# rubenwiersma/gravo_mg

Hardware: AMD Instinct MI355X
Metric: V-cycle wall time (ms per V-cycle incl. residual check) + solve-to-1e-4 iterations, 3M-vertex Poisson (lower is better)
Workload: dtype f64

## Files before the change

### gravo_mg_amd/cabi.py

```python
from __future__ import annotations

import ctypes as C
import os
from typing import List, Optional, Sequence, Tuple

import numpy as np
import scipy.sparse as sp

_HERE = os.path.dirname(os.path.abspath(__file__))
LIB_PATH = os.environ.get("GMG_LIB_PATH") or os.path.join(_HERE, "lib", "libgravomg_hip.so")

GMG_OK, GMG_ERR_INVALID, GMG_ERR_NO_DEVICE, GMG_ERR_HIP, GMG_ERR_STATE, GMG_ERR_NUMERIC, GMG_ERR_UNSUPPORTED = 0, -1, -2, -3, -4, -5, -6
DIVERGED = 1
SMOOTHER_MULTICOLOR_GS, SMOOTHER_JACOBI, SMOOTHER_CHEBYSHEV = 0, 1, 2
COARSE_HOST_LDLT, COARSE_DEVICE_INVERSE, COARSE_AUTO, COARSE_DEVICE_TRIANGLE = 0, 1, 2, 3

_STATUS_NAMES = {
    -1: "GMG_ERR_INVALID", -2: "GMG_ERR_NO_DEVICE", -3: "GMG_ERR_HIP", -4: "GMG_ERR_STATE",
    -5: "GMG_ERR_NUMERIC", -6: "GMG_ERR_UNSUPPORTED",
}


class GmgError(RuntimeError):
    def __init__(self, code: int, msg: str):
        super().__init__(f"{_STATUS_NAMES.get(code, code)}: {msg}")
        self.code = code


class GmgConfig(C.Structure):
    _fields_ = [
        ("device", C.c_int), ("smoother", C.c_int), ("jacobi_omega", C.c_double), ("pre_iters", C.c_int),
        ("post_iters", C.c_int), ("coarse_mode", C.c_int), ("use_graph", C.c_int), ("sigma", C.c_int),
        ("row_align", C.c_int), ("block_rows", C.c_int), ("block_lanes", C.c_int), ("block_from_level", C.c_int),
        ("device_setup", C.c_int), ("device_rap", C.c_int), ("reorder_fine", C.c_int), ("inner_precision", C.c_int), ("block_csr", C.c_int), ("host_threads", C.c_int),
        ("verbose", C.c_int), ("gs_omega", C.c_double), ("restrict_sigma", C.c_int), ("block_ep", C.c_int), ("dist_shard_levels", C.c_int), ("block_fine", C.c_int), ("fine_col16", C.c_int), ("stream_gate", C.c_int), ("dist_exchange", C.c_int), ("prepare_structure", C.c_int), ("fuse_restrict_sweep", C.c_int), ("speculate_head", C.c_int), ("uniform_slices", C.c_int), ("color_ahead", C.c_int),
        ("accelerate", C.c_int),
    ]


class GmgHierarchyOptions(C.Structure):
    _fields_ = [
        ("ratio", C.c_double), ("lower_bound", C.c_int), ("check_voronoi", C.c_int), ("nested", C.c_int),
        ("sampling", C.c_int), ("weighting", C.c_int), ("debug", C.c_int), ("full_clustering", C.c_int), ("use_device", C.c_int),
    ]


class GmgDeviceVectors(C.Structure):
    _fields_ = [
        ("rhs", C.c_void_p), ("rhs_row_stride", C.c_int64), ("rhs_col_stride", C.c_int64),
        ("x0", C.c_void_p), ("x0_row_stride", C.c_int64), ("x0_col_stride", C.c_int64),
        ("x", C.c_void_p), ("x_row_stride", C.c_int64), ("x_col_stride", C.c_int64),
    ]


_ip = C.POINTER(C.c_int)
_dp = C.POINTER(C.c_double)
_vp = C.c_void_p

SIGNATURES = {
    "gmg_config_default": (C.c_int, [C.POINTER(GmgConfig)]),
    "gmg_config_size": (C.c_int, []),
    "gmg_create": (C.c_int, [C.POINTER(GmgConfig), C.POINTER(_vp)]),
    "gmg_destroy": (None, [_vp]),
    "gmg_last_error": (C.c_char_p, [_vp]),
    "gmg_device_count": (C.c_int, []),
    "gmg_set_num_levels": (C.c_int, [_vp, C.c_int]),
    "gmg_set_prolongation": (C.c_int, [_vp, C.c_int, C.c_int, C.c_int, _ip, _ip, _dp]),
    "gmg_set_mass": (C.c_int, [_vp, C.c_int, _dp]),
    "gmg_set_system": (C.c_int, [_vp, C.c_int, _ip, _ip, _dp]),
    "gmg_num_levels": (C.c_int, [_vp]),
    "gmg_level_info": (C.c_int, [_vp, C.c_int, _ip, C.POINTER(C.c_int64), _ip, _ip]),
    "gmg_get_level_operator": (C.c_int, [_vp, C.c_int, _ip, _ip, _dp]),
    "gmg_get_level_ordering": (C.c_int, [_vp, C.c_int, _ip, _ip]),
    "gmg_get_level_blocks": (C.c_int, [_vp, C.c_int, _ip, _ip, C.POINTER(C.c_ubyte)]),
    "gmg_get_timing": (C.c_int, [_vp, C.c_char_p, _dp]),
    "gmg_smooth": (C.c_int, [_vp, C.c_int, _dp, _dp, C.c_int, C.c_int]),
    "gmg_residual": (C.c_int, [_vp, C.c_int, _dp, _dp, C.c_int, _dp]),
    "gmg_spmv": (C.c_int, [_vp, C.c_int, _dp, C.c_int, _dp]),
    "gmg_restrict": (C.c_int, [_vp, C.c_int, _dp, C.c_int, _dp]),
    "gmg_prolong_add": (C.c_int, [_vp, C.c_int, _dp, C.c_int, _dp]),
    "gmg_coarse_solve": (C.c_int, [_vp, _dp, C.c_int, _dp]),
    "gmg_residual_norm": (C.c_int, [_vp, _dp, _dp, C.c_int, C.c_int, _dp]),
    "gmg_vcycle": (C.c_int, [_vp, _dp, _dp, C.c_int]),
    "gmg_smooth_residual": (C.c_int, [_vp, C.c_int, _dp, _dp, C.c_int, C.c_int, C.c_int, _dp]),
    "gmg_solve": (C.c_int, [_vp, _dp, _dp, C.c_int, C.c_double, C.c_int, C.c_int, _ip, _dp, _dp]),
    "gmg_solve_x0_rhs": (C.c_int, [_vp, _dp, _dp, C.c_int, C.c_double, C.c_int, C.c_int, _ip, _dp, _dp]),
    "gmg_solve_device": (C.c_int, [_vp, C.POINTER(GmgDeviceVectors), C.c_int, C.c_double, C.c_int, C.c_int, _ip, _dp, _dp]),
    "gmg_set_system_values_device": (C.c_int, [_vp, C.c_void_p, C.c_int64]),
    "gmg_load_problem": (C.c_int, [_vp, _dp, _dp, C.c_int]),
    "gmg_run_cycles": (C.c_int, [_vp, C.c_int, C.c_int, _dp]),
    "gmg_fetch_solution": (C.c_int, [_vp, _dp]),
    "gmg_set_stream": (C.c_int, [_vp, _vp]),
    "gmg_dist_setup": (C.c_int, [_vp, C.c_int, C.c_int]),
    "gmg_dist_partition": (C.c_int, [_vp, C.c_int, C.c_int]),
    "gmg_dist_bind": (C.c_int, [_vp, _vp, _vp, _vp, C.c_int]),
    "gmg_dist_smooth_color": (C.c_int, [_vp, C.c_int]),
    "gmg_dist_residual_own": (C.c_int, [_vp]),
    "gmg_dist_coarse_cycle": (C.c_int, [_vp]),
    "gmg_dist_prolong_own": (C.c_int, [_vp]),
    "gmg_dist_norm_partial": (C.c_int, [_vp, C.c_int, _dp]),
    "gmg_dist_all_rows": (C.c_int, [_vp, C.c_int]),
    "gmg_dist_gather": (C.c_int, [_vp, C.c_void_p, C.c_void_p, C.c_int64, C.c_void_p]),
    "gmg_dist_scatter": (C.c_int, [_vp, C.c_void_p, C.c_void_p, C.c_void_p, C.c_int64, C.c_void_p]),
    "gmg_p2p_blob_bytes": (C.c_int, []),
    "gmg_p2p_prepare": (C.c_int, [_vp, C.c_int, C.c_int, C.c_int]),
    "gmg_p2p_export": (C.c_int, [_vp, C.c_void_p]),
    "gmg_p2p_connect": (C.c_int, [_vp, C.c_void_p]),
    "gmg_p2p_rccl_unique_id": (C.c_int, [C.c_void_p]),
    "gmg_p2p_connect_rccl": (C.c_int, [_vp, C.c_void_p]),
    "gmg_p2p_load": (C.c_int, [_vp, _dp, _dp]),
    "gmg_p2p_cycles": (C.c_int, [_vp, C.c_int, C.c_int, _dp]),
    "gmg_p2p_fetch": (C.c_int, [_vp, _dp]),
    "gmg_p2p_solve": (C.c_int, [_vp, _dp, _dp, C.c_double, C.c_int, C.c_int, C.POINTER(C.c_int), C.POINTER(C.c_double)]),
    "gmg_p2p_stat": (C.c_int, [_vp, C.c_char_p, _dp]),
    "gmg_p2p_set_smoother": (C.c_int, [_vp, C.c_int]),
    "gmg_p2p_set_fences": (C.c_int, [_vp, C.c_int]),
    "gmg_hierarchy_options_default": (C.c_int, [C.POINTER(GmgHierarchyOptions)]),
    "gmg_hierarchy_build": (C.c_int, [_dp, C.c_int, _ip, C.c_int, C.POINTER(GmgHierarchyOptions), C.POINTER(_vp)]),
    "gmg_hierarchy_destroy": (None, [_vp]),
    "gmg_hierarchy_num_levels": (C.c_int, [_vp]),
    "gmg_hierarchy_level_shape": (C.c_int, [_vp, C.c_int, _ip, _ip, _ip]),
    "gmg_hierarchy_get_prolongation": (C.c_int, [_vp, C.c_int, _ip, _ip, _dp]),
    "gmg_hierarchy_get_timing": (C.c_int, [_vp, C.c_char_p, _dp]),
    "gmg_hierarchy_get_samples": (C.c_int, [_vp, C.c_int, _ip]),
    "gmg_hierarchy_get_nearest": (C.c_int, [_vp, C.c_int, _ip]),
    "gmg_hierarchy_get_points": (C.c_int, [_vp, C.c_int, _dp]),
    "gmg_host_threads": (C.c_int, []),
    "gmg_hierarchy_get_triangles": (C.c_int, [_vp, C.c_int, _ip, _ip]),
    "gmg_hierarchy_get_fine_order": (C.c_int, [_vp, _ip, _ip]),
    "gmg_set_fine_order": (C.c_int, [_vp, C.c_int, _ip]),
    "gmg_set_fine_graph": (C.c_int, [_vp, C.c_int, C.c_int, _ip]),
    "gmg_use_hierarchy": (C.c_int, [_vp, _vp]),
    "gmg_finalize_hierarchy": (C.c_int, [_vp]),
    "gmg_host_ldlt_solve": (C.c_int, [C.c_int, _ip, _ip, _dp, _dp, C.c_int, _dp, C.POINTER(C.c_int64)]),
}

INTERNAL_SIGNATURES = {
    "gmg_debug_sell_info": (C.c_int, [_vp, C.c_int, C.c_int, C.POINTER(C.c_int64)]),
    "gmg_debug_sell_copy": (C.c_int, [_vp, C.c_int, C.c_int, C.POINTER(C.c_int64), _ip, _dp, _ip, _dp]),
    "gmg_debug_col16_copy": (C.c_int, [_vp, C.c_int, C.POINTER(C.c_int64), C.POINTER(C.c_uint), _ip]),
    "gmg_debug_select_parents": (C.c_int, [C.c_int, C.c_int, C.c_int, C.c_int, C.c_int, C.c_int, _dp, _dp, _ip, _ip, _ip, _ip, _ip, _ip, _ip, _ip, C.c_int,
                                           C.POINTER(C.c_ubyte), C.POINTER(C.c_ubyte), _ip, _dp]),
    "gmg_hierarchy_debug_row_kinds": (C.c_int, [_vp, C.c_int, _ip]),
    "gmg_host_galerkin": (C.c_int, [C.c_int, _ip, _ip, _dp, C.c_int, _ip, _ip, _dp, _ip, _ip, _dp]),
    "gmg_debug_device_galerkin": (C.c_int, [_vp, C.c_int, _ip, _ip, _dp, _dp, C.c_int, _ip, _ip, _dp, C.c_int64, _ip, _ip, _dp, _dp, _ip]),
    "gmg_host_plan_level": (C.c_int, [C.c_int, _ip, _ip, _dp, C.c_int, C.c_int, C.c_int, C.POINTER(C.c_int64), _ip, _ip, _ip,
                                      C.POINTER(C.c_ubyte)]),
    "gmg_host_fine_block_rule": (C.c_int, [C.c_int, _ip, _ip, _dp, _ip, _ip]),
    "gmg_debug_set": (C.c_int, [_vp, C.c_char_p, C.c_double]),
    "gmg_bench_kernel": (C.c_int, [_vp, C.c_int, C.c_int, C.c_int, C.c_int, _dp, _ip]),
    "gmg_profile_cycle": (C.c_int, [_vp, C.c_int, C.c_int, _dp, C.c_int]),
    "gmg_algorithmic_bytes": (C.c_int, [_vp, C.c_int, C.c_int, C.c_int, _dp]),
    "gmg_p2p_bench_kind": (C.c_int, [_vp, C.c_char_p, C.c_int, _dp]),
    "gmg_p2p_debug_collective_roundtrip": (C.c_int, [_vp, _dp, C.POINTER(C.c_longlong)]),
    "gmg_host_ldlt_probe": (C.c_int, [C.c_int, _ip, _ip, _dp, _dp, C.c_int, C.c_char_p, C.c_int]),
}

_lib = None


def _preload_torch_hip_runtime():
    import importlib.util
    try:
        spec = importlib.util.find_spec("torch")
    except (ImportError, ValueError):
        spec = None
    if spec is None or not spec.submodule_search_locations:
        return
    libdir = os.path.join(list(spec.submodule_search_locations)[0], "lib")
    for name in ("libhsa-runtime64.so", "libamdhip64.so"):
        path = os.path.join(libdir, name)
        if os.path.exists(path):
            try:
                C.CDLL(path, mode=C.RTLD_GLOBAL)
            except OSError:
                pass


def lib() -> C.CDLL:
    global _lib
    if _lib is None:
        if not os.path.exists(LIB_PATH):
            raise ImportError(
                f"{LIB_PATH} is missing: build it with gravo_mg_amd/csrc/build.sh (or __graft_entry__.build()). "
                "gravo_mg_amd has no CPU fallback for the device path.")
        _preload_torch_hip_runtime()
        l = C.CDLL(LIB_PATH)
        for name, (res, args) in list(SIGNATURES.items()) + list(INTERNAL_SIGNATURES.items()):
            fn = getattr(l, name)
            fn.restype = res
            fn.argtypes = args
        if l.gmg_config_size() != C.sizeof(GmgConfig):
            raise ImportError(f"{LIB_PATH} was built with a gmg_config of {l.gmg_config_size()} bytes, gravo_mg_amd/cabi.py mirrors one of {C.sizeof(GmgConfig)}: "
                              "rebuild the library (gravo_mg_amd/csrc/build.sh) or update the mirror")
        _lib = l
    return _lib


def device_count() -> int:
    return int(lib().gmg_device_count())


def _f64(a, shape2d: bool = True) -> np.ndarray:
    a = np.asarray(a, dtype=np.float64)
    if a.ndim == 1:
        a = a[:, None]
    return np.asfortranarray(a)


def _csc_layout(m) -> sp.csc_matrix:
    m = m if sp.isspmatrix_csc(m) else sp.csc_matrix(m)
    if m.indptr.dtype != np.int32 or m.indices.dtype != np.int32:
        if m.nnz >= 2**31:
            raise ValueError("matrix too large for int32 indices")
        m = sp.csc_matrix((m.data, m.indices.astype(np.int32), m.indptr.astype(np.int32)), shape=m.shape)
    if m.data.dtype != np.float64:
        m = m.astype(np.float64)
    return m


def _csc(m) -> sp.csc_matrix:
    m = sp.csc_matrix(m)
    if not m.has_sorted_indices:
        m = m.copy()
        m.sort_indices()
    m.sum_duplicates()
    if m.indptr.dtype != np.int32 or m.indices.dtype != np.int32:
        if m.nnz >= 2**31:
            raise ValueError("matrix too large for int32 indices")
        m = sp.csc_matrix((m.data, m.indices.astype(np.int32), m.indptr.astype(np.int32)), shape=m.shape)
# ... 7 lines not shown


def _pd(a: np.ndarray):
    return a.ctypes.data_as(_dp)


class Hierarchy:

    def __init__(self, pos, neigh, ratio=8.0, lower_bound=1000, check_voronoi=True, nested=False, sampling=0, weighting=0, debug=False, full_clustering=False, use_device=True):
        l = lib()
        pos = np.ascontiguousarray(pos, dtype=np.float64)
        neigh = np.ascontiguousarray(neigh, dtype=np.int32)
        if pos.ndim != 2 or pos.shape[1] != 3 or neigh.ndim != 2 or neigh.shape[0] != pos.shape[0]:
            raise ValueError("pos must be n x 3 and neigh n x K")
        opt = GmgHierarchyOptions()
        l.gmg_hierarchy_options_default(C.byref(opt))
        opt.ratio, opt.lower_bound, opt.check_voronoi, opt.nested = float(ratio), int(lower_bound), int(bool(check_voronoi)), int(bool(nested))
        opt.sampling, opt.weighting, opt.debug, opt.full_clustering = int(sampling), int(weighting), int(bool(debug)), int(bool(full_clustering))
        opt.use_device = int(use_device)
        self._h = _vp()
        rc = l.gmg_hierarchy_build(_pd(pos), pos.shape[0], _pi(neigh), neigh.shape[1], C.byref(opt), C.byref(self._h))
        if rc:
            raise GmgError(rc, "gmg_hierarchy_build failed (only Sampling.FASTDISK is supported)" if rc == GMG_ERR_UNSUPPORTED else "gmg_hierarchy_build failed")
        self.U: List[sp.csc_matrix] = []
        for k in range(l.gmg_hierarchy_num_levels(self._h)):
            nf, nc, nnz = C.c_int(), C.c_int(), C.c_int()
            l.gmg_hierarchy_level_shape(self._h, k, C.byref(nf), C.byref(nc), C.byref(nnz))
            colptr = np.empty(nc.value + 1, np.int32); rowidx = np.empty(nnz.value, np.int32); val = np.empty(nnz.value, np.float64)
            l.gmg_hierarchy_get_prolongation(self._h, k, _pi(colptr), _pi(rowidx), _pd(val))
            self.U.append(sp.csc_matrix((val, rowidx, colptr), shape=(nf.value, nc.value)))
        self.samples, self.nearest, self.points = [], [], []
        for k, u in enumerate(self.U):
            s_ = np.empty(u.shape[1], np.int32); n_ = np.empty(u.shape[0], np.int32); p_ = np.empty((u.shape[1], 3), np.float64)
            if l.gmg_hierarchy_get_samples(self._h, k, _pi(s_)) or l.gmg_hierarchy_get_nearest(self._h, k, _pi(n_)) or l.gmg_hierarchy_get_points(self._h, k, _pd(p_)):
                raise GmgError(GMG_ERR_INVALID, "hierarchy getters failed")
            self.samples.append(s_); self.nearest.append(n_); self.points.append(p_)
        self.triangles = []
        for k in range(len(self.U)):
            cnt = C.c_int()
            l.gmg_hierarchy_get_triangles(self._h, k, None, C.byref(cnt))
            t = np.empty((cnt.value, 3), np.int32)
            if cnt.value:
                l.gmg_hierarchy_get_triangles(self._h, k, _pi(t), C.byref(cnt))
            self.triangles.append(t)
        cnt = C.c_int()
        l.gmg_hierarchy_get_fine_order(self._h, None, C.byref(cnt))
        self.fine_order = None
        if cnt.value:
            self.fine_order = np.empty(cnt.value, np.int32)
            l.gmg_hierarchy_get_fine_order(self._h, _pi(self.fine_order), C.byref(cnt))

    def row_kinds(self, k: int) -> np.ndarray:
        out = np.zeros(4, np.int32)
        if lib().gmg_hierarchy_debug_row_kinds(self._h, int(k), _pi(out)):
            raise GmgError(GMG_ERR_INVALID, "gmg_hierarchy_debug_row_kinds failed")
        return out

    def timing(self, key: str) -> float:
        out = C.c_double()
        rc = lib().gmg_hierarchy_get_timing(self._h, key.encode(), C.byref(out))
        if rc:
            raise KeyError(key)
        return out.value

    TIMING_KEYS = ("n_vertices", "hierarchy", "sampling", "cluster", "next_neighborhood", "next_positions",
                   "triangle_finding", "triangle_selection", "PDS", "levels")

    def timings(self) -> dict:
        return {k: self.timing(k) for k in self.TIMING_KEYS}

    def __del__(self):
        try:
            if getattr(self, "_h", None):
                lib().gmg_hierarchy_destroy(self._h)
                self._h = None
        except Exception:
            pass


class Engine:

    def __init__(self, smoother=SMOOTHER_MULTICOLOR_GS, pre_iters=2, post_iters=2, jacobi_omega=0.67,
                 coarse_mode=COARSE_AUTO, use_graph=False, sigma=0, row_align=64, block_rows=64, block_from_level=1, block_lanes=0,
                 device_setup=True, device_rap=True, reorder_fine=2, inner_precision=0, block_csr=True, device=0, verbose=False, gs_omega=None, block_ep=None, restrict_sigma=None, dist_shard_levels=None, block_fine=None, fine_col16=None, stream_gate=None, prepare_structure=None, dist_exchange=None, fuse_restrict_sweep=None, speculate_head=None, uniform_slices=None, color_ahead=None, accelerate=0):
        l = lib()
        cfg = GmgConfig()
        l.gmg_config_default(C.byref(cfg))
        cfg.device, cfg.smoother, cfg.jacobi_omega = int(device), int(smoother), float(jacobi_omega)
        cfg.pre_iters, cfg.post_iters, cfg.coarse_mode = int(pre_iters), int(post_iters), int(coarse_mode)
        cfg.use_graph, cfg.sigma, cfg.row_align, cfg.verbose = int(bool(use_graph)), int(sigma), int(row_align), int(bool(verbose))
        cfg.block_rows, cfg.block_from_level, cfg.block_lanes = int(block_rows), int(block_from_level), int(block_lanes)
        cfg.device_setup, cfg.device_rap, cfg.reorder_fine = int(bool(device_setup)), int(bool(device_rap)), int(reorder_fine)
        cfg.inner_precision, cfg.block_csr = int(inner_precision), int(bool(block_csr))
        if gs_omega is not None:
            cfg.gs_omega = float(gs_omega)
        if block_ep is not None:
            cfg.block_ep = int(bool(block_ep))
        if restrict_sigma is not None:
            cfg.restrict_sigma = int(restrict_sigma)
        if dist_shard_levels is not None:
            cfg.dist_shard_levels = int(dist_shard_levels)
        if block_fine is not None:
            cfg.block_fine = int(bool(block_fine))
        if fine_col16 is not None:
            cfg.fine_col16 = int(bool(fine_col16))
        if stream_gate is not None:
            cfg.stream_gate = int(bool(stream_gate))
        if prepare_structure is not None:
            cfg.prepare_structure = int(bool(prepare_structure))
        if fuse_restrict_sweep is not None:
            cfg.fuse_restrict_sweep = int(bool(fuse_restrict_sweep))
        if speculate_head is not None:
            cfg.speculate_head = int(bool(speculate_head))
        if uniform_slices is not None:
            cfg.uniform_slices = int(bool(uniform_slices))
        if color_ahead is not None:
            cfg.color_ahead = int(bool(color_ahead))
        if dist_exchange is not None:
            cfg.dist_exchange = int(dist_exchange)
        cfg.accelerate = int(accelerate)
        self._h = _vp()
        rc = l.gmg_create(C.byref(cfg), C.byref(self._h))
        if rc:
            raise GmgError(rc, "gmg_create failed (invalid configuration)")
        self._n0 = None
        self._sizes: List[int] = []
        self.pre_iters, self.post_iters = int(pre_iters), int(post_iters)
        self.gs_omega = float(cfg.gs_omega)

    @classmethod
    def borrow(cls, handle: int) -> "Engine":
        self = cls.__new__(cls)
        self._h = _vp(int(handle))
        self._borrowed = True
        self._n0 = None
        self._sizes = []
        self.pre_iters = self.post_iters = None
        self.gs_omega = None
        return self

    def _chk(self, rc: int):
        if rc:
            raise GmgError(rc, lib().gmg_last_error(self._h).decode())

    def close(self):
        if getattr(self, "_h", None):
            if not getattr(self, "_borrowed", False):
                lib().gmg_destroy(self._h)
            self._h = None

    def __del__(self):
        try:
            self.close()
        except Exception:
            pass

    def set_prolongations(self, U: Sequence, finalize: bool = True, fine_order=None, fine_graph=None):
        l = lib()
        self._chk(l.gmg_set_num_levels(self._h, len(U)))
        self._sizes = []
        for k, u in enumerate(U):
            u = _csc(u)
            self._chk(l.gmg_set_prolongation(self._h, k, u.shape[0], u.shape[1], _pi(u.indptr), _pi(u.indices), _pd(u.data)))
            if k == 0:
                self._sizes.append(u.shape[0])
            self._sizes.append(u.shape[1])
        if fine_order is not None and len(U):
            fo = np.ascontiguousarray(fine_order, dtype=np.int32)
            self._chk(l.gmg_set_fine_order(self._h, fo.shape[0], _pi(fo)))
        if fine_graph is not None and len(U):
            fg = np.ascontiguousarray(fine_graph, dtype=np.int32)
            self._chk(l.gmg_set_fine_graph(self._h, fg.shape[0], fg.shape[1], _pi(fg)))
        if finalize and len(U):
            self._chk(l.gmg_finalize_hierarchy(self._h))

    def use_hierarchy(self, hier: Hierarchy):
        self._chk(lib().gmg_use_hierarchy(self._h, hier._h))
        self._sizes = [hier.U[0].shape[0]] + [u.shape[1] for u in hier.U] if hier.U else []

    def set_mass(self, mass_diag):
        m = np.ascontiguousarray(mass_diag, dtype=np.float64).ravel()
        self._chk(lib().gmg_set_mass(self._h, m.shape[0], _pd(m)))

    def set_system(self, lhs):
        a = _csc_layout(lhs)
        if a.shape[0] != a.shape[1]:
            raise ValueError("lhs must be square")
        self._chk(lib().gmg_set_system(self._h, a.shape[0], _pi(a.indptr), _pi(a.indices), _pd(a.data)))
        self._n0 = a.shape[0]

    @property
    def num_levels(self) -> int:
        return int(lib().gmg_num_levels(self._h))

    def level_info(self, k: int) -> dict:
        n, nnz, nc, npad = C.c_int(), C.c_int64(), C.c_int(), C.c_int()
        self._chk(lib().gmg_level_info(self._h, k, C.byref(n), C.byref(nnz), C.byref(nc), C.byref(npad)))
        return {"n": n.value, "nnz": nnz.value, "n_colors": nc.value, "n_pad": npad.value}

    def level_operator(self, k: int) -> sp.csc_matrix:
        info = self.level_info(k)
        colptr = np.empty(info["n"] + 1, np.int32); rowidx = np.empty(info["nnz"], np.int32); val = np.empty(info["nnz"], np.float64)
        self._chk(lib().gmg_get_level_operator(self._h, k, _pi(colptr), _pi(rowidx), _pd(val)))
# ... 317 lines not shown
    a, u = _csc_layout(A), _csc_layout(U)
    nc = u.shape[1]
    v2 = None if val2 is None else np.ascontiguousarray(val2, dtype=np.float64)
    if v2 is not None and v2.shape != a.data.shape:
        raise ValueError("val2 must have one value per stored entry of A")
    colptr, status = np.zeros(nc + 1, np.int32), C.c_int(-1)
    cap = a.nnz + nc
    for attempt in range(2):
        rowidx, val = np.empty(max(cap, 1), np.int32), np.empty(max(cap, 1), np.float64)
        out2 = np.empty(max(cap, 1), np.float64) if v2 is not None else None
        rc = lib().gmg_debug_device_galerkin(eng._h, a.shape[0], _pi(a.indptr), _pi(a.indices), _pd(a.data), _pd(v2) if v2 is not None else None, nc,
                                             _pi(u.indptr), _pi(u.indices), _pd(u.data), cap, _pi(colptr), _pi(rowidx), _pd(val),
                                             _pd(out2) if out2 is not None else None, C.byref(status))
        if rc == GMG_ERR_INVALID and attempt == 0 and int(colptr[nc]) > cap:
            cap = int(colptr[nc])
            continue
        eng._chk(rc)
        break
    if status.value != 0:
        return status.value, None, None
    nnz = int(colptr[nc])
    return 0, sp.csc_matrix((val[:nnz].copy(), rowidx[:nnz].copy(), colptr), shape=(nc, nc)), (out2[:nnz].copy() if out2 is not None else None)


def host_galerkin(A, U, as_stored: bool = False) -> sp.csc_matrix:
    a, u = (_csc_layout(A), _csc_layout(U)) if as_stored else (_csc(A), _csc(U))
    nc = u.shape[1]
    colptr = np.zeros(nc + 1, np.int32)
    rc = lib().gmg_host_galerkin(a.shape[0], _pi(a.indptr), _pi(a.indices), _pd(a.data), nc, _pi(u.indptr), _pi(u.indices), _pd(u.data),
                                 _pi(colptr), None, None)
    if rc:
        raise GmgError(rc, "gmg_host_galerkin")
    nnz = int(colptr[nc])
    rowidx = np.empty(nnz, np.int32); val = np.empty(nnz, np.float64)
    lib().gmg_host_galerkin(a.shape[0], _pi(a.indptr), _pi(a.indices), _pd(a.data), nc, _pi(u.indptr), _pi(u.indices), _pd(u.data),
                            _pi(colptr), _pi(rowidx), _pd(val))
    return sp.csc_matrix((val, rowidx, colptr), shape=(nc, nc))


def default_host_threads() -> int:
    return int(lib().gmg_host_threads())


def host_plan_level(A, mode: int = 0, block_rows: int = 256, sigma: int = 1024, row_align: int = 64) -> dict:
    a = _csc(A)
    n = a.shape[0]
    if mode != 1:
        block_rows = row_align
    info = (C.c_int64 * 6)()
    rc = lib().gmg_host_plan_level(n, _pi(a.indptr), _pi(a.indices), _pd(a.data), int(mode), int(block_rows), int(sigma), info, None, None, None, None)
    if rc:
        raise GmgError(rc, "gmg_host_plan_level")
    new2old = np.empty(int(info[0]), np.int32); color_begin = np.zeros(int(info[1]) + 1, np.int32)
    blk_begin = np.zeros(int(info[2]) + 1, np.int32); row_color = np.zeros(int(info[0]), np.uint8)
    rc = lib().gmg_host_plan_level(n, _pi(a.indptr), _pi(a.indices), _pd(a.data), int(mode), int(block_rows), int(sigma), info,
                                   _pi(new2old), _pi(color_begin), _pi(blk_begin), row_color.ctypes.data_as(C.POINTER(C.c_ubyte)))
    if rc:
        raise GmgError(rc, "gmg_host_plan_level")
    n_pad, n_colors, n_blocks = int(info[0]), int(info[1]), int(info[2])
    out = {"n_pad": n_pad, "n_colors": n_colors, "n_blocks": n_blocks, "sell_stored": int(info[3]), "offdiag_nnz": int(info[4]),
           "new2old": new2old[:n_pad].copy()}
    if mode == 1:
        out["blk_begin"] = blk_begin[: n_blocks + 1].copy()
        out["row_color"] = row_color[:n_pad].copy()
    else:
        out["color_begin"] = color_begin[: n_colors + 1].copy()
    return out


def host_plan_ahead(n, indptr, indices, row_align: int = 64, sigma: int = 1024) -> dict:
    indptr = np.ascontiguousarray(indptr, np.int32); indices = np.ascontiguousarray(indices, np.int32)
    vals = np.ones(max(len(indices), 1))
    info = (C.c_int64 * 6)()
    rc = lib().gmg_host_plan_level(int(n), _pi(indptr), _pi(indices), _pd(vals), 4, int(row_align), int(sigma), info, None, None, None, None)
    if rc:
        raise GmgError(rc, "gmg_host_plan_level")
    new2old = np.empty(int(info[0]), np.int32); color_begin = np.zeros(int(info[1]) + 1, np.int32)
    rc = lib().gmg_host_plan_level(int(n), _pi(indptr), _pi(indices), _pd(vals), 4, int(row_align), int(sigma), info, _pi(new2old), _pi(color_begin), None, None)
    if rc:
        raise GmgError(rc, "gmg_host_plan_level")
    return {"n_pad": int(info[0]), "n_colors": int(info[1]), "colored_ahead": bool(info[5]), "new2old": new2old, "color_begin": color_begin}


def host_fine_block_rule(A):
    a = _csc(A)
    blocked, reason = C.c_int(0), C.c_int(0)
    rc = lib().gmg_host_fine_block_rule(a.shape[0], _pi(a.indptr), _pi(a.indices), _pd(a.data), C.byref(blocked), C.byref(reason))
    if rc:
        raise GmgError(rc, "gmg_host_fine_block_rule")
    return bool(blocked.value), int(reason.value)


def host_ldlt_solve(A, b):
    a = _csc(A)
    B = _f64(b)
    X = np.empty_like(B, order="F")
    nnz = C.c_int64()
    rc = lib().gmg_host_ldlt_solve(a.shape[0], _pi(a.indptr), _pi(a.indices), _pd(a.data), _pd(B), B.shape[1], _pd(X), C.byref(nnz))
    if rc:
        raise GmgError(rc, "gmg_host_ldlt_solve (zero pivot?)")
    return (X[:, 0].copy() if np.asarray(b).ndim == 1 else X), nnz.value


def host_ldlt_probe(A, b, reps: int = 3) -> str:
    a = _csc(A)
    B = _f64(b)
    buf = C.create_string_buffer(1 << 16)
    rc = lib().gmg_host_ldlt_probe(a.shape[0], _pi(a.indptr), _pi(a.indices), _pd(a.data), _pd(B), int(reps), buf, len(buf))
    if rc:
        raise GmgError(rc, "gmg_host_ldlt_probe")
    return buf.value.decode()
```

### gravo_mg_amd/csrc/bindings.cpp

```cpp
#include <chrono>
#include <cstdio>
#include <cstdlib>
#include <pybind11/numpy.h>
#include <pybind11/pybind11.h>
#include <pybind11/stl.h>

#include <algorithm>
#include <atomic>
#include <cmath>
#include <cstdint>
#include <memory>
#include <stdexcept>
#include <string>
#include <thread>
#include <vector>

#include "multigrid_solver.h"

namespace py = pybind11;
using DenseIn = py::array_t<double, py::array::f_style | py::array::forcecast>;
using IntIn = py::array_t<int, py::array::c_style | py::array::forcecast>;

namespace {

// ... 202 lines not shown
        MGBS::MatrixXd x = b;
        solver->clearError();
        if (pardiso) throw std::runtime_error("direct_solve(pardiso=True): Pardiso (MKL) is not part of this build; use pardiso=False (sparse LDL^T)");
        solver->solve(A, b, x, 0);
        check();
        return from_dense(x);
    }

    py::list prolongation_matrices() {
        py::list out;
        for (const auto& u : solver->U) out.append(from_sparse(u));
        return out;
    }

    void set_prolongation_matrices(py::list U) {
        std::vector<MGBS::SparseMatrix> v;
        for (auto item : U) v.push_back(to_sparse(py::reinterpret_borrow<py::object>(item)));
        solver->U = v;
    }

    std::vector<std::vector<int>> sampling_indices() { return solver->samples; }
    std::vector<std::vector<size_t>> nearest_source() { return solver->nearestSource; }
    py::list level_points() {
        py::list out;
        for (const auto& P : solver->levelV) out.append(from_dense(P));
        return out;
    }
    py::list level_edges() { return py::list(); }
    std::vector<std::vector<int>> notrimap() { return solver->noTriFoundMap; }
    std::vector<std::vector<std::vector<int>>> all_triangles() { return solver->allTriangles; }
    py::list coarse_normals() { return py::list(); }

    void write_hierarchy_timing(std::string experiment, std::string file, bool write_headers) { MGBS::writeTiming(solver->hierarchyTiming, experiment, file, write_headers); }
    void write_solver_timing(std::string experiment, std::string file, bool write_headers) { MGBS::writeTiming(solver->solverTiming, experiment, file, write_headers); }
    void write_convergence(std::string file) { MGBS::writeConvergence(solver->convergence, file); }

    double residual(py::object lhs, DenseIn rhs, DenseIn solution, int type = 2) {
        MappedSparse mapped = map_system_matrix(lhs, symCache);
        MGBS::SparseMatrix& A = mapped.m;
        solver->clearError();
        double r = solver->residualCheck(A, to_dense(rhs), to_dense(solution), type);
        check();
        return r;
    }

    std::map<std::string, double> solver_timing() { return solver->solverTiming; }
    std::map<std::string, double> hierarchy_timing() { return solver->hierarchyTiming; }
    std::vector<std::tuple<double, double>> convergence() { return solver->convergence; }
    std::tuple<uintptr_t, long> prepare_system(py::object lhs) {
        MappedSparse mapped = map_system_matrix(lhs, symCache);
        gmg_handle h = nullptr;
        long gen = 0;
        solver->clearError();
        if (solver->prepareSystem(mapped.m, &h, &gen) != GMG_OK) { check(); throw std::runtime_error("prepare_system failed"); }
        return std::make_tuple((uintptr_t)h, gen);
    }
    uintptr_t engine_handle() { return (uintptr_t)solver->engineHandle(); }
    void invalidate_system() { solver->systemChangedExternally(); }
    void set_engine_option(const std::string& key, double value) {
        gmg_config& c = solver->engineConfig;
        if (key == "smoother") c.smoother = (int)value;
        else if (key == "jacobi_omega") c.jacobi_omega = value;
        else if (key == "gs_omega") c.gs_omega = value;
        else if (key == "coarse_mode") c.coarse_mode = (int)value;
        else if (key == "use_graph") c.use_graph = (int)value;
        else if (key == "block_rows") c.block_rows = (int)value;
        else if (key == "block_from_level") c.block_from_level = (int)value;
        else if (key == "device") c.device = (int)value;
        else if (key == "row_align") c.row_align = (int)value;
        else if (key == "block_lanes") c.block_lanes = (int)value;
        else if (key == "dist_shard_levels") c.dist_shard_levels = (int)value;
        else if (key == "block_fine") c.block_fine = (int)value;
        else if (key == "dist_rank") solver->distRank = (int)value;
        else if (key == "dist_world") solver->distWorld = (int)value;
        else if (key == "fine_col16") c.fine_col16 = (int)value;
        else if (key == "stream_gate") c.stream_gate = (int)value;
        else if (key == "fuse_restrict_sweep") c.fuse_restrict_sweep = (int)value;
        else if (key == "speculate_head") c.speculate_head = (int)value;
        else if (key == "uniform_slices") c.uniform_slices = (int)value;
        else if (key == "color_ahead") c.color_ahead = (int)value;
        else if (key == "dist_exchange") c.dist_exchange = (int)value;
        else if (key == "inner_precision") c.inner_precision = (int)value;
        else if (key == "accelerate") c.accelerate = (int)value;
        else throw std::invalid_argument("unknown engine option: " + key);
    }

#ifdef GMG_TESTING
    void test_report_diverged(int n) { solver->testReportDiverged = n; }
#endif

private:
    void check() {
        std::string now = solver->lastError();
        if (!now.empty()) throw std::runtime_error(now);
    }
    std::unique_ptr<MGBS::MultigridSolver> solver;
    SymmetryCache symCache;
};

PYBIND11_MODULE(gravomg_bindings, m) {
    m.doc() = "Multigrid solver bindings (MI355X-native V-cycle hot path)";

    py::enum_<Hierarchy>(m, "Hierarchy").value("OURS", OURS).value("SIG21", SIG21);
    py::enum_<Sampling>(m, "Sampling").value("FASTDISK", FASTDISK).value("POISSONDISK", POISSONDISK).value("FPS", FPS).value("RANDOM", RANDOM).value("MIS", MIS);
    py::enum_<Weighting>(m, "Weighting").value("BARYCENTRIC", BARYCENTRIC).value("UNIFORM", UNIFORM).value("INVDIST", INVDIST);

    py::class_<MultigridSolver>(m, "MultigridSolver")
        .def(py::init<DenseIn, IntIn, py::object, double, int, int, double, int, int, int, int, bool, bool, Sampling, Weighting, bool, DenseIn, bool, bool, bool, int, bool>())
        .def("construct_sig21_hierarchy", &MultigridSolver::construct_sig21_hierarchy, py::arg("F"))
        .def("toggle_hierarchy", &MultigridSolver::toggle_hierarchy, py::arg("hierarchy"))
        .def("solve", &MultigridSolver::solve, py::arg("lhs"), py::arg("rhs"))
        .def("direct_solve", &MultigridSolver::direct_solve, py::arg("lhs"), py::arg("rhs"), py::arg("pardiso"))
        .def("prolongation_matrices", &MultigridSolver::prolongation_matrices)
        .def("set_prolongation_matrices", &MultigridSolver::set_prolongation_matrices, py::arg("U"))
        .def("sampling_indices", &MultigridSolver::sampling_indices)
        .def("level_points", &MultigridSolver::level_points)
        .def("level_edges", &MultigridSolver::level_edges)
        .def("notrimap", &MultigridSolver::notrimap)
        .def("all_triangles", &MultigridSolver::all_triangles)
        .def("coarse_normals", &MultigridSolver::coarse_normals)
        .def("nearest_source", &MultigridSolver::nearest_source)
        .def("write_hierarchy_timing", &MultigridSolver::write_hierarchy_timing, py::arg("experiment"), py::arg("file"), py::arg("write_headers"))
        .def("write_solver_timing", &MultigridSolver::write_solver_timing, py::arg("experiment"), py::arg("file"), py::arg("write_headers"))
        .def("write_convergence", &MultigridSolver::write_convergence, py::arg("file"))
        .def("residual", &MultigridSolver::residual, py::arg("lhs"), py::arg("rhs"), py::arg("solution"), py::arg("type") = 2)
        .def("solver_timing", &MultigridSolver::solver_timing)
        .def("hierarchy_timing", &MultigridSolver::hierarchy_timing)
        .def("convergence", &MultigridSolver::convergence)
        .def("prepare_system", &MultigridSolver::prepare_system, py::arg("lhs"))
        .def("engine_handle", &MultigridSolver::engine_handle)
        .def("invalidate_system", &MultigridSolver::invalidate_system)
        .def("set_engine_option", &MultigridSolver::set_engine_option, py::arg("key"), py::arg("value"))
#ifdef GMG_TESTING
        .def("_test_report_diverged", &MultigridSolver::test_report_diverged, py::arg("n"))
#endif
        ;
}
```

### gravo_mg_amd/csrc/engine.hip

```cpp
#include <hip/hip_runtime.h>
#include <dlfcn.h>

#include <array>
#include <atomic>
#include <chrono>
#include <cmath>
#include <functional>
#include <future>
#include <cstdio>
#include <cstdlib>
#include <cstring>
#include <map>
#include <mutex>
#include <shared_mutex>
#include <string>
#include <vector>

#if !defined(__HIP_DEVICE_COMPILE__)
#include <execinfo.h>
#include <signal.h>
#include <unistd.h>
#endif

#include "../../include/gravomg_hip.h"
// ... 15 lines not shown

#if !defined(__HIP_DEVICE_COMPILE__)
namespace {
struct sigaction gmg_prev_action[32];
void gmg_fatal_signal(int sig) {
    void* frames[48];
    const int nf = backtrace(frames, 48);
    const char msg[] = "[gmg] fatal signal, native stack of the faulting thread:\n";
    (void)!write(2, msg, sizeof(msg) - 1);
    backtrace_symbols_fd(frames, nf, 2);
    if (sig > 0 && sig < 32) sigaction(sig, &gmg_prev_action[sig], nullptr); else signal(sig, SIG_DFL);
    raise(sig);
}
struct GmgSignalAid {
    GmgSignalAid() {
        if (!EnvSwitches::get().segv_backtrace) return;
        void* warm[4];
        (void)backtrace(warm, 4);
        struct sigaction sa;
        std::memset(&sa, 0, sizeof(sa));
        sa.sa_handler = gmg_fatal_signal;
        for (int sig : {SIGSEGV, SIGBUS, SIGABRT, SIGFPE}) sigaction(sig, &sa, &gmg_prev_action[sig]);
    }
} gmg_signal_aid;
}
#endif

#include "engine_state.hip.hpp"
#include "engine_setup.hip.hpp"
#include "engine_cycle.hip.hpp"
#include "engine_part.hip.hpp"
#include "engine_system.hip.hpp"

int gate_unwound(gmg_handle h);
#define GMG_CATCH_H                                                                                             \
    catch (const std::exception& e_) { if (h) (void)gate_unwound(h); return h ? fail(h, GMG_ERR_STATE, std::string("exception: ") + e_.what()) : GMG_ERR_STATE; } \
    catch (...) { if (h) (void)gate_unwound(h); return h ? fail(h, GMG_ERR_STATE, "unknown exception") : GMG_ERR_STATE; }
#define GMG_CATCH_0                                              \
    catch (...) { return GMG_ERR_STATE; }

void p2p_release_handle(gmg_handle h);


extern "C" {

int gmg_config_size(void) { return (int)sizeof(gmg_config); }

int gmg_config_default(gmg_config* cfg) try {
    if (!cfg) return GMG_ERR_INVALID;
    std::memset(cfg, 0, sizeof(*cfg));
    cfg->device = 0;
    cfg->smoother = GMG_SMOOTHER_MULTICOLOR_GS;
    cfg->jacobi_omega = 0.67;
    cfg->pre_iters = 2;
    cfg->post_iters = 2;
    cfg->coarse_mode = GMG_COARSE_AUTO;
    cfg->use_graph = 0;
    cfg->sigma = 0;
    cfg->row_align = 64;
    cfg->block_rows = 64;
    cfg->block_from_level = 1;
    cfg->block_lanes = 0;
    cfg->device_setup = 1;
    cfg->device_rap = 1;
    cfg->reorder_fine = 2;
    cfg->inner_precision = 0;
    cfg->block_csr = 1;
    cfg->host_threads = 0;
    cfg->verbose = 0;
    cfg->block_ep = 1;
    cfg->dist_shard_levels = 2;
    cfg->fine_col16 = 1;
    cfg->stream_gate = 1;
    cfg->prepare_structure = 1;
    cfg->fuse_restrict_sweep = 1;
    cfg->speculate_head = 1;
    cfg->uniform_slices = 1;
    cfg->color_ahead = 1;
    cfg->dist_exchange = 0;
    cfg->block_fine = 1;
    cfg->restrict_sigma = 64;
    cfg->gs_omega = 1.35;
    cfg->accelerate = 0;
    return GMG_OK;
} GMG_CATCH_0

int gmg_host_threads(void) try { return hw_threads(); } GMG_CATCH_0

int gmg_device_count(void) try {
    int n = 0;
    if (hipGetDeviceCount(&n) != hipSuccess) return 0;
    return n;
} GMG_CATCH_0

int gmg_create(const gmg_config* cfg, gmg_handle* out) try {
    if (!out) return GMG_ERR_INVALID;
    gmg_config c;
    if (cfg) c = *cfg; else gmg_config_default(&c);
    if (c.sigma < 0 || c.sigma % 64 || c.restrict_sigma < 0 || c.restrict_sigma % 64 || c.row_align <= 0 || c.row_align % 64 || c.pre_iters < 0 || c.post_iters < 0 ||
        c.reorder_fine < 0 || c.reorder_fine > 2 || c.inner_precision < 0 || c.inner_precision > 1 || c.block_rows < 0 || c.block_rows > gmgk::kBlockRows || c.block_rows % 64 || c.block_from_level < 0 || !(c.gs_omega > 0.0 && c.gs_omega < 2.0) || c.dist_shard_levels < 1 || c.dist_shard_levels > 2 || c.block_fine < 0 || c.block_fine > 1 || c.dist_exchange < 0 || c.dist_exchange > 2 ||
        (c.block_lanes != 0 && c.block_lanes != 1 && c.block_lanes != 4) || (c.block_lanes != 1 && c.block_rows > gmgk::kQuadBlockRows)) return GMG_ERR_INVALID;
    if (c.accelerate < 0 || c.accelerate > gmg::kAccelMaxDepth) return GMG_ERR_INVALID;
    if (c.smoother < GMG_SMOOTHER_MULTICOLOR_GS || c.smoother > GMG_SMOOTHER_CHEBYSHEV) return GMG_ERR_INVALID;
    if (c.accelerate > 0 && c.inner_precision) return GMG_ERR_UNSUPPORTED;
    gmg_handle h = new gmg_solver_s();
    h->cfg = c;
    if (h->cfg.host_threads <= 0) h->cfg.host_threads = hw_threads();
    int ndev = gmg_device_count();
    if (ndev > 0 && c.device >= 0 && c.device < ndev && hipSetDevice(c.device) == hipSuccess &&
        hipStreamCreateWithFlags(&h->stream, hipStreamNonBlocking) == hipSuccess) {
        h->has_device = true;
        h->own_stream = h->stream;
        { int cus = 0; if (hipDeviceGetAttribute(&cus, hipDeviceAttributeMultiprocessorCount, c.device) == hipSuccess && cus > 0) h->n_cus = cus; else (void)hipGetLastError(); }
        (void)hipEventCreate(&h->ev0);
        (void)hipEventCreate(&h->ev1);
        if (hipStreamCreateWithFlags(&h->aux_stream, hipStreamNonBlocking) != hipSuccess) { h->aux_stream = nullptr; (void)hipGetLastError(); }
        if (hipEventCreateWithFlags(&h->aux_ev, hipEventDisableTiming) != hipSuccess) { h->aux_ev = nullptr; (void)hipGetLastError(); }
        if (hipMalloc((void**)&h->d_aux_err, sizeof(int)) != hipSuccess) { h->d_aux_err = nullptr; (void)hipGetLastError(); }
        h->poll = EnvSwitches::get().poll;
        (void)ensure_bounce(h);
    }
    *out = h;
    return GMG_OK;
} GMG_CATCH_0

void gmg_destroy(gmg_handle h) {
    if (!h) return;
    PoolScope pool_scope_(&h->pool);
    if (h->has_device) {
        (void)hipSetDevice(h->cfg.device);
        (void)hipStreamSynchronize(h->stream);
        p2p_release_handle(h);
        drop_system(h);
        drop_device_transfers(h);
        h->d_stage = {}; h->d_partials = {}; h->d_norm = {}; h->d_watch = {};
        if (h->h_pinned) (void)sync_hipHostFree(h->h_pinned);
        for (int i = 0; i < 2; ++i) { if (h->h_stage[i]) (void)sync_hipHostFree(h->h_stage[i]); if (h->h_stage_ev[i]) (void)hipEventDestroy(h->h_stage_ev[i]); }
        for (hipEvent_t& e : h->h_chunk_ev) if (e) (void)hipEventDestroy(e);
        if (h->h_norm) (void)sync_hipHostFree(h->h_norm);
        if (h->h_flag) (void)sync_hipHostFree(h->h_flag);
        if (h->ev0) (void)hipEventDestroy(h->ev0);
        if (h->ev1) (void)hipEventDestroy(h->ev1);
        if (h->aux_ev) (void)hipEventDestroy(h->aux_ev);
        if (h->aux_stream) { (void)hipStreamSynchronize(h->aux_stream); (void)sync_hipStreamDestroy(h->aux_stream); }
        if (h->d_aux_err) (void)sync_hipFree(h->d_aux_err);
        drop_rap_order(h);
        for (int i = 0; i < 2; ++i) { if (h->bounce[i]) (void)sync_hipHostFree(h->bounce[i]); if (h->bounce_ev[i]) (void)hipEventDestroy(h->bounce_ev[i]); }
        for (hipEvent_t e : h->prof_ev) (void)hipEventDestroy(e);
        (void)sync_hipStreamDestroy(h->own_stream);
        h->pool.trim();
    }
    delete h;
}

const char* gmg_last_error(gmg_handle h) { return h ? h->err.c_str() : "null handle"; }

int gmg_set_num_levels(gmg_handle h, int L) try {
    if (!h || L < 0 || L > 64) return h ? fail(h, GMG_ERR_INVALID, "invalid level count") : GMG_ERR_INVALID;
    PoolScope pool_scope_(&h->pool);
    if (h->has_device) { drop_system(h); drop_device_transfers(h); }
    h->patches.clear(); h->patches_ready = false;
    h->bfs_order.clear();
    h->fine_graph.reset();
    drop_rap_order(h);
    h->L = L;
    h->ord_cache_valid = false;
// ... 1148 lines not shown
    std::memcpy(c_colptr, C.ptr.data(), sizeof(int) * (n_coarse + 1));
    if (c_rowidx) std::memcpy(c_rowidx, C.idx.data(), sizeof(int) * C.nnz());
    if (c_val) std::memcpy(c_val, C.val.data(), sizeof(double) * C.nnz());
    return GMG_OK;
} GMG_CATCH_0

int gmg_debug_device_galerkin(gmg_handle h, int n, const int* a_colptr, const int* a_rowidx, const double* a_val, const double* a_val2, int n_coarse,
                              const int* u_colptr, const int* u_rowidx, const double* u_val, int64_t cap, int* c_colptr, int* c_rowidx, double* c_val,
                              double* c_val2, int* status) try {
    NEED_DEVICE();
    if (n <= 0 || n_coarse <= 0 || cap < 0 || !a_colptr || !a_rowidx || !a_val || !u_colptr || !u_rowidx || !u_val || !c_colptr || !c_rowidx || !c_val || !status ||
        (a_val2 && !c_val2)) return fail(h, GMG_ERR_INVALID, "bad arguments");
    if (a_colptr[0] != 0 || u_colptr[0] != 0) return fail(h, GMG_ERR_INVALID, "column pointers must start at 0");
    for (int i = 0; i < n; ++i) if (a_colptr[i + 1] < a_colptr[i]) return fail(h, GMG_ERR_INVALID, "column pointers of A decrease");
    for (int c = 0; c < n_coarse; ++c) if (u_colptr[c + 1] < u_colptr[c]) return fail(h, GMG_ERR_INVALID, "column pointers of U decrease");
    for (int q = 0; q < a_colptr[n]; ++q) if (a_rowidx[q] < 0 || a_rowidx[q] >= n) return fail(h, GMG_ERR_INVALID, "row index of A out of range");
    for (int q = 0; q < u_colptr[n_coarse]; ++q) if (u_rowidx[q] < 0 || u_rowidx[q] >= n) return fail(h, GMG_ERR_INVALID, "row index of U out of range");
    if (hipSetDevice(h->cfg.device) != hipSuccess) return fail(h, GMG_ERR_HIP, "hipSetDevice failed");
    DevCsr dA, dU, dC;
    DevEll3 e3;
    DevBuf<int> d_err;
    Compressed C;
    int rc, herr = 0;
    if ((rc = dev_alloc(h, d_err, 1))) return rc;
    HIPCHK(hipMemsetAsync(d_err, 0, sizeof(int), h->stream));
    if ((rc = upload_csr_raw(h, dA, n, a_colptr, a_rowidx, a_val)) || (rc = upload_csr_raw(h, dU, n_coarse, u_colptr, u_rowidx, u_val)) ||
        (rc = build_ell3(h, e3, dU, n, d_err))) { (void)hipStreamSynchronize(h->stream); return rc; }
    HIPCHK(hipMemcpyAsync(&herr, d_err, sizeof(int), hipMemcpyDeviceToHost, h->stream));
    HIPCHK(hipStreamSynchronize(h->stream));
    *status = 0;
    if (herr) { *status = 1; return GMG_OK; }
    int64_t nnz = 0;
    rc = device_rap(h, dA, dU, e3, dC, C, true, true, &nnz, d_err);
    if (rc == 1) { *status = 1; return GMG_OK; }
    if (rc) return rc;
    std::memcpy(c_colptr, C.ptr.data(), sizeof(int) * ((size_t)n_coarse + 1));
    if (nnz > cap) return fail(h, GMG_ERR_INVALID, "the product has " + std::to_string(nnz) + " entries: more than the caller's capacity (c_colptr is filled)");
    if (nnz) { std::memcpy(c_rowidx, C.idx.data(), sizeof(int) * (size_t)nnz); std::memcpy(c_val, C.val.data(), sizeof(double) * (size_t)nnz); }
    if (a_val2) {
        Compressed C2;
        if ((rc = h2d(h, dA.val, a_val2, sizeof(double) * (size_t)a_colptr[n]))) { (void)hipStreamSynchronize(h->stream); return rc; }
        rc = device_rap(h, dA, dU, e3, dC, C2, false, true, &nnz, d_err, true);
        HIPCHK(hipStreamSynchronize(h->stream));
        if (rc) return rc < 0 ? rc : fail(h, GMG_ERR_STATE, "the numeric pass declined a pattern the product was made on");
        if ((int64_t)C2.val.size() != nnz) return fail(h, GMG_ERR_STATE, "the numeric pass returned another number of entries");
        if (nnz) std::memcpy(c_val2, C2.val.data(), sizeof(double) * (size_t)nnz);
    }
    return GMG_OK;
} GMG_CATCH_H

int gmg_host_plan_level(int n, const int* colptr, const int* rowidx, const double* val, int mode, int block_rows, int sigma, int64_t* info,
                        int* new2old, int* color_begin, int* blk_begin, unsigned char* row_color) try {
    if (n <= 0 || !colptr || !rowidx || !val || mode < 0 || mode > 4) return GMG_ERR_INVALID;
    if (mode == 1 && (block_rows <= 0 || block_rows > gmgk::kBlockRows || block_rows % 64)) return GMG_ERR_INVALID;
    if (sigma < 0 || sigma % 64) return GMG_ERR_INVALID;
    if (mode == 4) {
        PreColoring pre;
        std::atomic<int> stop{0};
        pre.n_colors = greedy_coloring_ahead(n, colptr, rowidx, (int64_t)colptr[n], pre.c8, stop);
        if (pre.n_colors == -2) return GMG_ERR_INVALID;
        if (info) info[5] = pre.n_colors >= 0 ? 1 : 0;
        LevelOrdering o = make_ordering(PatternView{n, colptr, rowidx}, true, (block_rows > 0 && block_rows % 64 == 0) ? block_rows : 64, sigma, 0, nullptr, true, &pre);
        if (o.n_colors > kMaxColors) return GMG_ERR_UNSUPPORTED;
        if (info) { info[0] = o.n_pad; info[1] = o.n_colors; info[2] = 0; info[3] = 0; info[4] = 0; }
        if (new2old) std::memcpy(new2old, o.new2old.data(), sizeof(int) * o.n_pad);
        if (color_begin) std::memcpy(color_begin, o.color_begin.data(), sizeof(int) * (o.n_colors + 1));
        return GMG_OK;
    }
    Compressed A;
    A.assign(n, n, colptr, rowidx, val);
    LevelOrdering o = mode == 1 ? make_block_ordering(A, block_rows)
                                : make_ordering(A, true, (block_rows > 0 && block_rows % 64 == 0) ? block_rows : 64, sigma, mode == 2 ? 1 : 0, nullptr, mode == 3);
    if (o.n_colors > kMaxColors) return GMG_ERR_UNSUPPORTED;
    SellHost sa; std::vector<double> dg; std::string e;
    if (!build_operator_sell(A, o, 0, sa, dg, e)) return GMG_ERR_NUMERIC;
    if (info) { info[0] = o.n_pad; info[1] = o.n_colors; info[2] = o.n_blocks(); info[3] = sa.stored(); info[4] = sa.nnz_real; info[5] = 0; }
    if (new2old) std::memcpy(new2old, o.new2old.data(), sizeof(int) * o.n_pad);
    if (color_begin && !o.blocked) std::memcpy(color_begin, o.color_begin.data(), sizeof(int) * (o.n_colors + 1));
    if (blk_begin && o.blocked) std::memcpy(blk_begin, o.blk_begin.data(), sizeof(int) * o.blk_begin.size());
    if (row_color && o.blocked) std::memcpy(row_color, o.row_color.data(), o.row_color.size());
    return GMG_OK;
} GMG_CATCH_0

int gmg_debug_set(gmg_handle h, const char* key, double value) try {
    if (!h || !key) return GMG_ERR_INVALID;
    if (std::string(key) == "col16_uncovered") { h->dbg_col16_uncovered = (int)value; return GMG_OK; }
    if (std::string(key) == "cheby_ratio") {
        if (value != 0.0 && !cheby_ratio_usable(value)) return fail(h, GMG_ERR_INVALID, "cheby_ratio must be > 1 (0: the process-wide ratio)");
        h->dbg_cheby_ratio = value;
        if (h->has_device) drop_graphs(h);
        if (h->timing.count("cheby_ratio")) h->timing["cheby_ratio"] = cheby_ratio(h);
        return GMG_OK;
    }
    return fail(h, GMG_ERR_INVALID, std::string("unknown debug key: ") + key);
} GMG_CATCH_H

int gmg_host_fine_block_rule(int n, const int* colptr, const int* rowidx, const double* val, int* blocked, int* reason) try {
    if (n <= 0 || !colptr || !rowidx || !val || !blocked) return GMG_ERR_INVALID;
    int why = 0;
    if ((double)colptr[n] < kFineBlockMinRow * (double)n) why = 1;
    else if (!stieltjes_signs(n, colptr, rowidx, val, hw_threads())) why = 2;
    *blocked = why == 0 ? 1 : 0;
    if (reason) *reason = why;
    return GMG_OK;
} GMG_CATCH_0

int gmg_host_ldlt_solve(int n, const int* colptr, const int* rowidx, const double* val, const double* b, int d, double* x, int64_t* factor_nnz) try {
    if (n <= 0 || !colptr || !rowidx || !val || !b || !x || d <= 0) return GMG_ERR_INVALID;
    Compressed A;
    A.assign(n, n, colptr, rowidx, val);
    SupernodalLDLT f;
    if (!f.factor(A)) return GMG_ERR_NUMERIC;
    std::vector<double> w((size_t)n * d);
    f.solve_multi(b, (size_t)n, x, (size_t)n, d, w.data());
    if (factor_nnz) *factor_nnz = f.factor_nnz();
    return GMG_OK;
} GMG_CATCH_0

int gmg_host_ldlt_probe(int n, const int* colptr, const int* rowidx, const double* val, const double* b, int reps, char* report, int cap) try {
    if (n <= 0 || !colptr || !rowidx || !val || !b || !report || cap <= 0) return GMG_ERR_INVALID;
    reps = std::max(1, reps);
    Compressed A;
    A.assign(n, n, colptr, rowidx, val);
    SupernodalLDLT f;
    if (!f.factor(A)) return GMG_ERR_NUMERIC;
    std::vector<double> w((size_t)n * 3), x((size_t)n);
    f.solve_multi(b, (size_t)n, x.data(), (size_t)n, 1, w.data());
    std::string text;
    auto say = [&](const char* fmt, auto... args) { char line[1024]; std::snprintf(line, sizeof(line), fmt, args...); text += line; };
    {
        std::vector<double> xb((size_t)n);
        double best = 1e30;
        for (int batch = 0; batch < 20; ++batch) {
            auto t0 = clk::now();
            for (int i = 0; i < reps; ++i) f.solve_multi(b, (size_t)n, xb.data(), (size_t)n, 1, w.data());
            best = std::min(best, 1e3 * ms_since(t0) / reps);
        }
        say("factorisation: ordering %.2f ms, symbolic %.2f ms, numeric %.2f ms\n", f.phase_ms[0], f.phase_ms[1], f.phase_ms[2]);
        {
            std::vector<double> ts;
            for (int i = 0; i < 15; ++i) { if (!f.factor(A, true)) return GMG_ERR_NUMERIC; ts.push_back(f.phase_ms[2]); }
            std::sort(ts.begin(), ts.end());
            say("numeric re-factorisation on %d thread(s): best %.2f ms, median %.2f ms\n", SupernodalLDLT::numeric_threads(), ts.front(), ts[ts.size() / 2]);
        }
        {
            SupernodalLDLT::DeviceFactor E;
            f.export_device_factor(E);
            std::vector<double> col((size_t)n), e((size_t)n, 0.0), ref((size_t)n), wk((size_t)n);
            double worst = 0.0, scale = 0.0;
            const int picks = std::min(n, 24);
            for (int t = 0; t < picks; ++t) {
                const int c = (int)((long)t * (n - 1) / std::max(picks - 1, 1));
                SupernodalLDLT::emulate_device_column(E, c, col.data());
                e[(size_t)f.perm[(size_t)c]] = 1.0;
                f.solve(e.data(), ref.data(), wk.data());
                e[(size_t)f.perm[(size_t)c]] = 0.0;
                for (int j = c; j < n; ++j) { worst = std::max(worst, std::fabs(col[(size_t)j] - ref[(size_t)f.perm[(size_t)j]])); scale = std::max(scale, std::fabs(ref[(size_t)f.perm[(size_t)j]])); }
            }
            say("device factor layout: %d chunks of <= %d columns in %d levels; %d columns of the inverse by the chunk algorithm vs back-substitution: max |difference| %.3e of max |entry| %.3e\n",
                E.nq, SupernodalLDLT::kChunk, E.nlev, picks, worst, scale);
        }
        long part[3];
        f.split_report(part);
        say("n=%d nnz(L)=%ld: %.2f us per single-column solve on one thread (best of 20 batches of %d); %d parts of the elimination "
                     "tree, panel entries in the lightest / heaviest part / above them: %ld / %ld / %ld\n", n, f.factor_nnz(), best, reps, f.parts(), part[0], part[1], part[2]);
        for (int threads = 2; threads <= std::min(8, f.parts()); threads += threads < 4 ? 1 : 2) {
            double best2 = 1e30, diff = 0.0;
            SpinTeam team(threads - 1);
            team.arm();
            std::vector<double> x2((size_t)n);
            for (int batch = 0; batch < 20; ++batch) {
                auto t0 = clk::now();
                for (int i = 0; i < reps; ++i) f.solve_multi(b, (size_t)n, x2.data(), (size_t)n, 1, w.data(), &team);
                best2 = std::min(best2, 1e3 * ms_since(t0) / reps);
// ... 52 lines not shown
```

### gravo_mg_amd/csrc/engine_cycle.hip.hpp

```cpp
#pragma once

namespace {


#define DISPATCH_D(dc, ...)              \
    switch (dc) {                        \
        case 1: { constexpr int D = 1; __VA_ARGS__; } break; \
        case 2: { constexpr int D = 2; __VA_ARGS__; } break; \
        case 3: { constexpr int D = 3; __VA_ARGS__; } break; \
        default: { constexpr int D = 4; __VA_ARGS__; } break; \
    }

#define DISPATCH_C16(mode, ...)          \
    switch (mode) {                      \
        case 1: { constexpr int C16 = 1; __VA_ARGS__; } break; \
        case 2: { constexpr int C16 = 2; __VA_ARGS__; } break; \
        case 3: { constexpr int C16 = 3; __VA_ARGS__; } break; \
        case 4: { constexpr int C16 = 4; __VA_ARGS__; } break; \
        default: { constexpr int C16 = 0; __VA_ARGS__; } break; \
    }

#define DISPATCH_FLAG(NAME, cond, ...)   \
    { if (cond) { constexpr bool NAME = true; __VA_ARGS__; } else { constexpr bool NAME = false; __VA_ARGS__; } }

#define DISPATCH_ONE_OF(NAME, v, A, B, C, ...)   \
    { if ((v) == (A)) { constexpr int NAME = A; __VA_ARGS__; } else if ((v) == (B)) { constexpr int NAME = B; __VA_ARGS__; } else { constexpr int NAME = C; __VA_ARGS__; } }

template <class F>
inline void for_col_chunks(int d, F&& f) {
    for (int c0 = 0; c0 < d; c0 += 4) f(c0, std::min(4, d - c0));
}

template <class T> struct Prec;
template <> struct Prec<double> {
    static const double* val(const DevSell& s) { return s.val; }
    static const double* diag(const Level& l) { return l.diag; }
    static const double* bcval(const Level& l) { return l.bc_val; }
    static const double* epval(const Level& l) { return l.ep_val; }
    static const double* eeval(const Level& l) { return l.ee_val; }
    static double* x(Level& l) { return l.x; }
    static double* b(Level& l) { return l.b; }
    static double* r(Level& l) { return l.r; }
    static double* tmp(Level& l) { return l.tmp; }
};
template <> struct Prec<float> {
    static const float* val(const DevSell& s) { return s.val32; }
    static const float* diag(const Level& l) { return l.diag32; }
    static const float* bcval(const Level& l) { return l.bc_val32; }
    static const float* epval(const Level& l) { return l.ep_val32; }
    static const float* eeval(const Level& l) { return l.ee_val32; }
    static float* x(Level& l) { return l.x32; }
    static float* b(Level& l) { return l.b32; }
    static float* r(Level& l) { return l.r32; }
    static float* tmp(Level& l) { return l.tmp32; }
};

template <class T>
struct SmoothAsk {
    bool from_zero = false;
    bool first_done = false;
    bool head_done = false;
    T* res_out = nullptr;
    bool res_il = false;
    int norm_type = -1;
    T* il_out = nullptr;
};
template <class T>
struct SmoothDone {
    int res_from = 0;
    int norm_blocks = 0;
    const T* prev = nullptr;
    bool prev_valid = false;
    bool il_written = false;
};

template <class T>
int fold_norm(gmg_handle, Level&, int, bool, int, int, int) { return 0; }
template <>
int fold_norm<double>(gmg_handle h, Level& l, int d, bool last_launch, int sb, int se, int type) {
    if (!last_launch || type < 0 || &l != &h->lv[0] || d > 4 || l.ord.n_colors < 2 || se != l.Aoff.n_slices) return 0;
    const double* w = type == 1 ? h->d_minv : (type == 2 ? h->d_mass : nullptr);
    const int nblk = grid_for(se - sb), first = norm_grid(sb);
    if ((size_t)(first + nblk) > (size_t)h->partial_blocks) return 0;
    DISPATCH_D(d, DISPATCH_C16(l.Aoff.c16_sel(), hipLaunchKernelGGL((gmgk::gs_color_norm<D, C16>), dim3(nblk), dim3(gmgk::kBlock), 0, h->stream, l.Aoff.slice_ptr,
                                     l.Aoff.col, l.Aoff.val, l.diag, l.b, l.x, l.n_pad, sb, se, h->cfg.gs_omega, w, h->d_partials + (size_t)first * 2 * d,
                                     l.Aoff.col16, l.Aoff.win_base, l.Aoff.c16_arg())));
    return nblk;
}

template <class T>
int fold_residual(gmg_handle, Level&, int, bool, int, int, T*, bool) { return 0; }
template <>
int fold_residual<double>(gmg_handle h, Level& l, int d, bool last_launch, int sb, int se, double* out, bool il) {
    if (!last_launch || !out || &l != &h->lv[0] || d > 4 || l.ord.n_colors < 2 || se != l.Aoff.n_slices || sb <= 0) return 0;
    DISPATCH_D(d, DISPATCH_C16(l.Aoff.c16_sel(), DISPATCH_FLAG(YI, il, hipLaunchKernelGGL((gmgk::gs_color_residual<D, C16, (YI && D > 1)>), dim3(grid_for(se - sb)),
                                     dim3(gmgk::kBlock), 0, h->stream, l.Aoff.slice_ptr, l.Aoff.col, l.Aoff.val, l.diag, l.b, l.x, out, l.n_pad, sb, se,
                                     h->cfg.gs_omega, l.Aoff.col16, l.Aoff.win_base, l.Aoff.c16_arg()))));
    return sb;
}

inline bool polled(gmg_handle h);

template <class T>
T level_omega(gmg_handle h, const Level& l) { return &l == &h->lv[0] ? (T)h->cfg.gs_omega : (T)1.0; }

template <class T>
void launch_gs_color(gmg_handle h, Level& l, int c0, int dc, int sb, int se, T omega, const unsigned long long* plain_rows = nullptr, const int* go = nullptr) {
    const int ld = l.n_pad;
    T* x = Prec<T>::x(l);
    const T* b = Prec<T>::b(l);
    if (&l == &h->lv[0]) {
        DISPATCH_D(dc, DISPATCH_C16(l.Aoff.c16_sel(), DISPATCH_FLAG(OM, plain_rows != nullptr, hipLaunchKernelGGL((gmgk::gs_color<T, D, C16 + 1, (OM && sizeof(T) == 8)>),
                                          dim3(grid_for(se - sb)), dim3(gmgk::kBlock), 0, h->stream, l.Aoff.slice_ptr, l.Aoff.col, Prec<T>::val(l.Aoff), Prec<T>::diag(l),
                                          b + (size_t)c0 * ld, x + (size_t)c0 * ld, ld, sb, se, 1, omega, l.Aoff.col16, l.Aoff.win_base, l.Aoff.c16_arg(), plain_rows, go))));
    } else {
        DISPATCH_D(dc, hipLaunchKernelGGL((gmgk::gs_color<T, D, 0>), dim3(grid_for(se - sb)), dim3(gmgk::kBlock), 0, h->stream,
                                          l.Aoff.slice_ptr, l.Aoff.col, Prec<T>::val(l.Aoff), Prec<T>::diag(l), b + (size_t)c0 * ld,
                                          x + (size_t)c0 * ld, ld, sb, se, 1, omega));
    }
}

inline int first_color(const Level& l) {
    for (int c = 0; c < l.ord.n_colors; ++c)
        if (l.ord.color_begin[c + 1] / 64 > l.ord.color_begin[c] / 64) return c;
    return -1;
}

inline bool head_eligible(gmg_handle h, int d) {
    return h->cfg.speculate_head && polled(h) && !h->cfg.inner_precision && h->cfg.smoother == GMG_SMOOTHER_MULTICOLOR_GS && h->cfg.pre_iters > 0 && h->L >= 1 &&
           !h->lv[0].ord.blocked && h->lv[0].ord.n_colors >= 2 && first_color(h->lv[0]) >= 0 && first_color(h->lv[0]) < h->lv[0].ord.n_colors - 1 && d >= 1 && d <= 4 &&
           !h->partitioned && h->part_world <= 1 && h->d_watch && !h->prof_on;
}
inline bool enqueue_head(gmg_handle h, int d) {
    Level& l = h->lv[0];
    const int c = first_color(l);
    launch_gs_color<double>(h, l, 0, d, l.ord.color_begin[c] / 64, l.ord.color_begin[c + 1] / 64, level_omega<double>(h, l), nullptr, reinterpret_cast<const int*>(h->d_watch + 1));
    h->timing["heads_enqueued"] += 1.0;
    return true;
}

template <class T>
SmoothDone<T> launch_gs_sweeps(gmg_handle h, Level& l, int d, int iters, const SmoothAsk<T>& ask) {
    SmoothDone<T> done;
    const int c_head = ask.head_done ? first_color(l) : -1;
    for (int it = 0; it < iters; ++it)
        for_col_chunks(d, [&](int c0, int dc) {
            for (int c = 0; c < l.ord.n_colors; ++c) {
                int sb = l.ord.color_begin[c] / 64, se = l.ord.color_begin[c + 1] / 64;
                if (se <= sb) continue;
                if (it == 0 && c0 == 0 && c == c_head) continue;
                const bool last_launch = it == iters - 1 && c == l.ord.n_colors - 1;
                if (const int nblk = fold_norm<T>(h, l, d, last_launch, sb, se, ask.norm_type)) { done.norm_blocks = nblk; continue; }
                if (const int from = fold_residual<T>(h, l, d, last_launch, sb, se, ask.res_out, ask.res_il)) { done.res_from = from; continue; }
                launch_gs_color<T>(h, l, c0, dc, sb, se, level_omega<T>(h, l));
            }
        });
    return done;
}

template <class T>
void launch_jacobi_sweeps(gmg_handle h, Level& l, int d, int iters) {
    const int ld = l.n_pad;
    T* in = Prec<T>::x(l); T* out = Prec<T>::tmp(l);
    const T* b = Prec<T>::b(l);
    for (int it = 0; it < iters; ++it) {
        for_col_chunks(d, [&](int c0, int dc) {
            DISPATCH_D(dc, hipLaunchKernelGGL((gmgk::jacobi_sweep<T, D>), dim3(grid_for(l.Aoff.n_slices)), dim3(gmgk::kBlock), 0, h->stream,
                                              l.Aoff.slice_ptr, l.Aoff.col, Prec<T>::val(l.Aoff), Prec<T>::diag(l), b + (size_t)c0 * ld,
                                              (in ? in + (size_t)c0 * ld : nullptr), out + (size_t)c0 * ld, ld, l.Aoff.n_slices, (T)h->cfg.jacobi_omega, 1));
        });
        std::swap(in, out);
    }
    if (in != Prec<T>::x(l)) (void)hipMemcpyAsync(Prec<T>::x(l), in, sizeof(T) * (size_t)ld * d, hipMemcpyDeviceToDevice, h->stream);
}

template <class T>
void launch_cheby_steps(gmg_handle h, Level& l, int d, int iters) {
    const int ld = l.n_pad;
    T* in = Prec<T>::x(l); T* out = Prec<T>::tmp(l);
    const T* b = Prec<T>::b(l);
    T* p = Prec<T>::r(l);
    const int c16 = &l == &h->lv[0] ? l.Aoff.c16_sel() : 0;
    const double ratio = cheby_ratio(h);
    for (int it = 0; it < iters; ++it) {
        const ChebyStep st = cheby_step_coeffs(l.cheby_lambda, ratio, it);
// ... 28 lines not shown
                                              (in ? in + (size_t)c0 * ld : nullptr), out + (size_t)c0 * ld, ld, l.ep_cap_e, l.ep_cap_l, nb, b0, vgrid, out_il)));
        } else if (l.use_bcsr && d > 1) {
            DISPATCH_D(dc, hipLaunchKernelGGL((gmgk::gs_block_csrout<T, D, (D == 1 ? 32 : 24)>), dim3(nb), dim3(64),
                                              (size_t)l.bc_cap * (sizeof(T) + sizeof(int)) + (size_t)D * 64 * sizeof(T), h->stream, blk_begin,
                                              blk_ncolors, l.d_row_color, l.Ain.slice_ptr, l.ain_col16, Prec<T>::val(l.Ain), l.bc_ptr, l.bc_col,
                                              Prec<T>::bcval(l), Prec<T>::diag(l), b + (size_t)c0 * ld, (in ? in + (size_t)c0 * ld : nullptr), out + (size_t)c0 * ld,
                                              ld, l.bc_cap));
        } else if (l.Ain.lpr == 4) {
            DISPATCH_D(dc, hipLaunchKernelGGL((gmgk::gs_block4<T, D, 8>), dim3(nb), dim3(4 * h->cfg.block_rows), 0, h->stream, blk_begin,
                                              blk_ncolors, l.d_row_color, l.Ain.slice_ptr, l.ain_col16, Prec<T>::val(l.Ain), l.Aout.slice_ptr,
                                              l.Aout.col, Prec<T>::val(l.Aout), Prec<T>::diag(l), b + (size_t)c0 * ld, (in ? in + (size_t)c0 * ld : nullptr),
                                              out + (size_t)c0 * ld, ld));
        } else {
            DISPATCH_D(dc, hipLaunchKernelGGL((gmgk::gs_block<T, D, (D == 1 ? 32 : 24)>), dim3(nb), dim3(h->cfg.block_rows), 0, h->stream, blk_begin,
                                              blk_ncolors, l.d_row_color, l.Ain.slice_ptr, l.ain_col16, Prec<T>::val(l.Ain), l.Aout.slice_ptr,
                                              l.Aout.col, Prec<T>::val(l.Aout), Prec<T>::diag(l), b + (size_t)c0 * ld, (in ? in + (size_t)c0 * ld : nullptr),
                                              out + (size_t)c0 * ld, ld));
        }
    });
}

template <class T>
SmoothDone<T> launch_block_sweeps(gmg_handle h, Level& l, int d, int iters, const SmoothAsk<T>& ask) {
    SmoothDone<T> done;
    const int ld = l.n_pad;
    const int nb = l.ord.n_blocks();
    T* in = ask.from_zero ? nullptr : Prec<T>::x(l); T* out = Prec<T>::tmp(l);
    const T* before_last = nullptr;
    bool last_known = false;
    int it0 = 0;
    if (ask.from_zero && ask.first_done) {
        before_last = nullptr; last_known = true;
        in = out; out = Prec<T>::x(l);
        it0 = 1;
    }
    for (int it = it0; it < iters; ++it) {
        const bool with_il = ask.il_out && it == iters - 1 && l.use_ep && d > 1 && d <= 4;
        launch_block_sweep_range<T>(h, l, d, in, out, 0, nb, nullptr, nullptr, with_il ? ask.il_out : nullptr);
        if (with_il) done.il_written = true;
        before_last = in; last_known = true;
        if (it == 0 && ask.from_zero) { in = out; out = Prec<T>::x(l); }
        else std::swap(in, out);
    }
    if (in != Prec<T>::x(l)) (void)hipMemcpyAsync(Prec<T>::x(l), in, sizeof(T) * (size_t)ld * d, hipMemcpyDeviceToDevice, h->stream);
    done.prev_valid = last_known && before_last != (const T*)Prec<T>::x(l);
    done.prev = before_last;
    return done;
}

template <class T>
bool launch_residual_delta(gmg_handle h, Level& l, int d, T* r, const SmoothDone<T>& swept, const int* begin_table = nullptr, int nb_list = 0) {
    if (!l.use_ep || !swept.prev_valid || pointwise_smoother(h->cfg)) return false;
    const int ld = l.n_pad, nb = begin_table ? nb_list : l.ord.n_blocks();
    if (nb <= 0) return true;
    const int grid = (nb + 7) / 8 * 8;
    const T* x_old = swept.prev;
    const T* x_new = Prec<T>::x(l);
    for_col_chunks(d, [&](int c0, int dc) {
        DISPATCH_D(dc, DISPATCH_FLAG(STREAM, ep_streams(l), hipLaunchKernelGGL((gmgk::residual_delta_ep<T, D, STREAM>), dim3(grid), dim3(64),
                                          gmgk::ep_lds_bytes<T>(0, l.ep_cap_e, 0), h->stream, begin_table, l.ee_ptr, l.ee_col, Prec<T>::eeval(l),
                                          (x_old ? x_old + (size_t)c0 * ld : nullptr), x_new + (size_t)c0 * ld, r + (size_t)c0 * ld, ld, nb)));
    });
    return true;
}

inline bool smooth_from_zero_ok(gmg_handle h, const Level& l, int iters) {
    return iters > 0 && !pointwise_smoother(h->cfg) && l.ord.blocked;
}

template <class T = double>
SmoothDone<T> launch_smooth(gmg_handle h, Level& l, int d, int iters, const SmoothAsk<T>& ask = {}) {
    if (iters <= 0) return {};
    if (h->cfg.smoother == GMG_SMOOTHER_JACOBI) launch_jacobi_sweeps<T>(h, l, d, iters);
    else if (h->cfg.smoother == GMG_SMOOTHER_CHEBYSHEV) launch_cheby_steps<T>(h, l, d, iters);
    else if (l.ord.blocked) return launch_block_sweeps<T>(h, l, d, iters, ask);
    else return launch_gs_sweeps<T>(h, l, d, iters, ask);
    return {};
}

template <class T, int LPR>
void launch_spmv_lpr(gmg_handle h, Level& l, int d, int mode, const T* b, const T* x, T* y, int sb, int se, bool y_il = false) {
    const int ld = l.n_pad;
    const bool il = y_il && mode == 1 && LPR == 1 && d > 1 && d <= 4;
    for_col_chunks(d, [&](int c0, int dc) {
        DISPATCH_D(dc, DISPATCH_C16(l.Aoff.c16_sel(), DISPATCH_FLAG(RES, mode == 1, DISPATCH_FLAG(YI, il,
                       hipLaunchKernelGGL((gmgk::spmv_full<T, D, (RES ? 1 : 0), LPR, (LPR == 1 ? C16 : 0), (YI && RES && LPR == 1 && D > 1)>), dim3(grid_for(se - sb)),
                                          dim3(gmgk::kBlock), 0, h->stream, l.Aoff.slice_ptr, l.Aoff.col, Prec<T>::val(l.Aoff), Prec<T>::diag(l),
                                          (RES ? b + (size_t)c0 * ld : nullptr), x + (size_t)c0 * ld, y + (size_t)c0 * ld, ld, sb, se, 1, l.Aoff.col16,
                                          l.Aoff.win_base, l.Aoff.c16_arg())))));
    });
}
template <class T>
void launch_spmv_list(gmg_handle h, Level& l, int d, const T* b, const T* x, T* y, const int* slices, int n_list) {
    const int ld = l.n_pad;
    for_col_chunks(d, [&](int c0, int dc) {
        DISPATCH_D(dc, DISPATCH_FLAG(QUAD, l.Aoff.lpr == 4, hipLaunchKernelGGL((gmgk::spmv_full_list<T, D, 1, (QUAD ? 4 : 1)>), dim3(grid_for(n_list)), dim3(gmgk::kBlock), 0,
                                          h->stream, l.Aoff.slice_ptr, l.Aoff.col, Prec<T>::val(l.Aoff), Prec<T>::diag(l), b + (size_t)c0 * ld, x + (size_t)c0 * ld,
                                          y + (size_t)c0 * ld, ld, slices, n_list)));
    });
}
template <class T>
void launch_spmv(gmg_handle h, Level& l, int d, int mode, const T* b, const T* x, T* y, int n_slices = -1, bool y_il = false) {
    if (n_slices < 0) n_slices = l.Aoff.n_slices;
    if (l.Aoff.lpr == 4) launch_spmv_lpr<T, 4>(h, l, d, mode, b, x, y, 0, n_slices);
    else launch_spmv_lpr<T, 1>(h, l, d, mode, b, x, y, 0, n_slices, y_il);
}

template <class T, int LPR>
void launch_restrict_lpr(gmg_handle h, Level& fine, Level& coarse, int d, const T* src, T* dst, bool src_il = false) {
    const bool il = src_il && d > 1 && d <= 4;
    for_col_chunks(d, [&](int c0, int dc) {
        DISPATCH_D(dc, DISPATCH_C16(fine.R.c16_sel(), DISPATCH_FLAG(XI, il, hipLaunchKernelGGL((gmgk::transfer<T, D, 0, LPR, C16, (XI && D > 1)>), dim3(grid_for(fine.R.n_slices)),
                                          dim3(gmgk::kBlock), 0, h->stream, fine.R.slice_ptr, fine.R.col, Prec<T>::val(fine.R), fine.R.row_of, src + (size_t)c0 * fine.n_pad,
                                          fine.n_pad, dst + (size_t)c0 * coarse.n_pad, coarse.n_pad, 0, fine.R.n_slices, 1, fine.R.col16, fine.R.win_base, fine.R.c16_arg()))));
    });
}
template <class T>
void launch_restrict_list(gmg_handle h, Level& fine, Level& coarse, int d, const T* src, T* dst, const int* slices, int n_list) {
    for_col_chunks(d, [&](int c0, int dc) {
        DISPATCH_D(dc, DISPATCH_FLAG(QUAD, fine.R.lpr == 4, hipLaunchKernelGGL((gmgk::transfer_list<T, D, 0, (QUAD ? 4 : 1)>), dim3(grid_for(n_list)), dim3(gmgk::kBlock), 0,
                                          h->stream, fine.R.slice_ptr, fine.R.col, Prec<T>::val(fine.R), fine.R.row_of, src + (size_t)c0 * fine.n_pad, fine.n_pad,
                                          dst + (size_t)c0 * coarse.n_pad, coarse.n_pad, slices, n_list)));
    });
}
template <class T>
void launch_restrict(gmg_handle h, Level& fine, Level& coarse, int d, const T* src, T* dst, bool src_il = false) {
    if (fine.R.lpr == 4) launch_restrict_lpr<T, 4>(h, fine, coarse, d, src, dst, src_il);
    else launch_restrict_lpr<T, 1>(h, fine, coarse, d, src, dst, src_il);
}

template <class T>
int restrict_sweep0_kind(gmg_handle h, const Level& fine, const Level& coarse, int d, bool src_il) {
    if (!h->cfg.fuse_restrict_sweep || pointwise_smoother(h->cfg) || h->cfg.pre_iters <= 0 || d > 4) return 0;
    if (!coarse.ord.blocked || fine.R.lpr != 4 || !(h->cfg.restrict_sigma == 0 || h->cfg.restrict_sigma == 64)) return 0;
    if (coarse.use_ep) return (coarse.n_pad == 64 * coarse.ord.n_blocks() && fine.R.n_slices == 4 * coarse.ord.n_blocks()) ? 1 : 0;
    if (!(coarse.use_bcsr && d > 1) && coarse.Ain.lpr == 4 && fine.R.c16_mode == 0 && !src_il && fine.R.n_slices * 16 == coarse.n_pad) return 2;
    return 0;
}
template <class T>
void launch_restrict_sweep0(gmg_handle h, Level& fine, Level& coarse, int d, const T* src, bool src_il, int kind, const int* blk_list = nullptr, int nb_list = 0) {
    const int nb = blk_list ? nb_list : coarse.ord.n_blocks();
    if (kind == 2) {
        DISPATCH_D(d, hipLaunchKernelGGL((gmgk::gs_block4<T, D, 8, true>), dim3(nb), dim3(4 * h->cfg.block_rows), 0, h->stream, coarse.d_blk_begin, coarse.d_blk_ncolors,
                                         coarse.d_row_color, coarse.Ain.slice_ptr, coarse.ain_col16, Prec<T>::val(coarse.Ain), coarse.Aout.slice_ptr, coarse.Aout.col,
                                         Prec<T>::val(coarse.Aout), Prec<T>::diag(coarse), (const T*)nullptr, (const T*)nullptr, Prec<T>::tmp(coarse), coarse.n_pad,
                                         fine.R.slice_ptr, fine.R.col, Prec<T>::val(fine.R), fine.R.row_of, src, fine.n_pad, Prec<T>::b(coarse)));
        return;
    }
    const int vgrid = (nb + 7) / 8 * 8;
    const size_t lds_sweep = gmgk::ep_lds_bytes<T>(d, 0, coarse.ep_cap_l);
    const size_t lds = lds_sweep + (size_t)d * 64 * sizeof(T);
    DISPATCH_D(d, DISPATCH_C16(fine.R.c16_sel(), DISPATCH_FLAG(STREAM, ep_streams(coarse), DISPATCH_FLAG(XI, src_il,
                  hipLaunchKernelGGL((gmgk::restrict_sweep0<T, D, STREAM, C16, (XI && D > 1)>), dim3(vgrid), dim3(256), lds, h->stream, fine.R.slice_ptr, fine.R.col,
                                     Prec<T>::val(fine.R), fine.R.row_of, src, fine.n_pad, fine.R.col16, fine.R.win_base, fine.R.c16_arg(), Prec<T>::b(coarse),
                                     coarse.d_blk_ncolors, coarse.d_row_color, coarse.ep_ptr, coarse.ep_col, Prec<T>::epval(coarse), Prec<T>::diag(coarse),
                                     Prec<T>::tmp(coarse), coarse.n_pad, nb, vgrid, (int)lds_sweep, blk_list)))));
}

template <class T>
void launch_prolong_add(gmg_handle h, Level& fine, Level& coarse, int d, const T* src, T* dst, bool src_il = false, int sb = 0, int se = -1, int c16 = -1) {
    const bool il = src_il && d > 1 && d <= 4;
    if (se < 0) se = fine.P.n_slices;
    if (c16 < 0) c16 = fine.P.c16_sel();
    for_col_chunks(d, [&](int c0, int dc) {
        DISPATCH_D(dc, DISPATCH_C16(c16, DISPATCH_FLAG(XI, il, hipLaunchKernelGGL((gmgk::transfer<T, D, 1, 1, C16, (XI && D > 1)>), dim3(grid_for(se - sb)), dim3(gmgk::kBlock), 0,
                                          h->stream, fine.P.slice_ptr, fine.P.col, Prec<T>::val(fine.P), (const int*)nullptr, src + (size_t)c0 * coarse.n_pad, coarse.n_pad,
                                          dst + (size_t)c0 * fine.n_pad, fine.n_pad, sb, se, 1, fine.P.col16, fine.P.win_base, fine.P.c16_arg()))));
    });
}
template <class T>
void launch_prolong_add_list(gmg_handle h, Level& fine, Level& coarse, int d, const T* src, T* dst, const int* slices, int n_list) {
    for_col_chunks(d, [&](int c0, int dc) {
        DISPATCH_D(dc, hipLaunchKernelGGL((gmgk::transfer_list<T, D, 1, 1>), dim3(grid_for(n_list)), dim3(gmgk::kBlock), 0, h->stream, fine.P.slice_ptr, fine.P.col,
                                          Prec<T>::val(fine.P), (const int*)nullptr, src + (size_t)c0 * coarse.n_pad, coarse.n_pad, dst + (size_t)c0 * fine.n_pad,
                                          fine.n_pad, slices, n_list));
    });
}

constexpr unsigned kPolledHostFlags = hipHostMallocCoherent | hipHostMallocMapped;
inline bool polled(gmg_handle h) { return !h->cfg.use_graph && h->poll && h->h_flag; }

int wait_flag(gmg_handle h, int slot) {
    const unsigned long long want = h->flag_seq[slot];
    auto t0 = clk::now();
    double next_query_ms = 20.0;
    for (unsigned spin = 1;; ++spin) {
        if (__atomic_load_n(h->h_flag + 8 * slot, __ATOMIC_ACQUIRE) == want) return GMG_OK;
        if ((spin & 4095u) == 0 && ms_since(t0) > next_query_ms) {
            hipError_t q = hipStreamQuery(h->stream);
            if (q == hipSuccess) {
                if (__atomic_load_n(h->h_flag + 8 * slot, __ATOMIC_ACQUIRE) != want) { h->poll = false; h->timing["poll_disabled"] = 1.0; }
                return GMG_OK;
            }
            if (q != hipErrorNotReady) HIPCHK(q);
            next_query_ms += 20.0;
        }
        __builtin_ia32_pause();
    }
}

int wait_norm(gmg_handle h) {
    if (polled(h)) return wait_flag(h, 0);
    HIPCHK(hipStreamSynchronize(h->stream));
    return GMG_OK;
}

struct CycleWatch { int mode; double tol; int type; int cycles_done; };

void launch_reduce(gmg_handle h, int nblk, int dc, int c0, bool last, const double* partials = nullptr, const CycleWatch* decide = nullptr) {
    if (!partials) partials = h->d_partials;
    if (polled(h)) {
        gmgk::SolveWatch watch{nullptr, nullptr, nullptr, 0.0, 0, 0, 0, 0};
        if (decide && last && c0 == 0 && h->d_watch)
            watch = gmgk::SolveWatch{reinterpret_cast<int*>(h->d_watch + 1), h->h_flag + 1, h->d_watch, decide->tol, decide->mode, decide->type, dc, decide->cycles_done};
        hipLaunchKernelGGL(gmgk::reduce_partials, dim3(1), dim3(gmgk::kReduceBlock), 0, h->stream, partials, nblk, 2 * dc, h->h_norm + 2 * c0,
                           last ? h->h_flag : nullptr, last ? ++h->flag_seq[0] : 0ull, (int)EnvSwitches::get().publish_fenced, watch);
    }
    else
        hipLaunchKernelGGL(gmgk::reduce_partials, dim3(1), dim3(gmgk::kReduceBlock), 0, h->stream, partials, nblk, 2 * dc, h->d_norm + 2 * c0,
                           (unsigned long long*)nullptr, 0ull, 0);
}

int launch_norm(gmg_handle h, int d, int type, int folded = 0, const CycleWatch* decide = nullptr) {
    Level& l = h->lv[0];
    const double* w = type == 1 ? h->d_minv : (type == 2 ? h->d_mass : nullptr);
    const int n_slices = folded ? l.ord.color_begin[l.ord.n_colors - 1] / 64 : l.Aoff.n_slices;
    const int nblk = norm_grid(n_slices);
    const bool poll = polled(h);
    for_col_chunks(d, [&](int c0, int dc) {
        DISPATCH_D(dc, DISPATCH_C16(l.Aoff.c16_sel(), hipLaunchKernelGGL((gmgk::residual_norm_slices<D, 0, C16>), dim3(nblk), dim3(gmgk::kNormWaves * 64), 0, h->stream,
                                          l.Aoff.slice_ptr, l.Aoff.col, l.Aoff.val, l.diag, l.b + (size_t)c0 * l.n_pad, l.x + (size_t)c0 * l.n_pad, w,
                                          l.n_pad, n_slices, (float*)nullptr, h->d_partials, l.Aoff.col16, l.Aoff.win_base, l.Aoff.c16_arg())));
        launch_reduce(h, nblk + folded, dc, c0, c0 + 4 >= d, nullptr, decide);
    });
    if (!poll) HIPCHK(hipMemcpyAsync(h->h_norm, h->d_norm, sizeof(double) * 2 * d, hipMemcpyDeviceToHost, h->stream));
    return GMG_OK;
}

int ensure_vectors(gmg_handle h, int d) {
    if (d <= h->dcap) return GMG_OK;
    drop_graphs(h);
    unbind_level0(h);
    h->accel = {};
    auto vec = [&](auto& v, const Level& l, bool wanted) -> int {
        v.reset();
        if (!wanted) return GMG_OK;
        const size_t count = (size_t)l.n_pad * d;
        int rc = dev_alloc(h, v, count);
        if (rc == GMG_OK) HIPCHK(hipMemsetAsync(v, 0, sizeof(*v.get()) * count, h->stream));
        return rc;
    };
    for (auto& l : h->lv) {
        const bool tmp = pointwise_smoother(h->cfg) || l.ord.blocked, f32 = h->cfg.inner_precision != 0;
        int rc;
        if ((rc = vec(l.x, l, true)) || (rc = vec(l.b, l, true)) || (rc = vec(l.r, l, true)) || (rc = vec(l.tmp, l, tmp)) ||
            (rc = vec(l.x32, l, f32)) || (rc = vec(l.b32, l, f32)) || (rc = vec(l.r32, l, f32)) || (rc = vec(l.tmp32, l, f32 && tmp))) return rc;
    }
    Level& c = h->lv[h->L];
    size_t need = (size_t)c.n_pad * d * 2;
    if (need > h->pinned_cap) {
        if (h->h_pinned) (void)sync_hipHostFree(h->h_pinned);
        HIPCHK(hipHostMalloc((void**)&h->h_pinned, sizeof(double) * need, kPolledHostFlags));
        h->pinned_cap = need;
    }
    if (h->h_norm) (void)sync_hipHostFree(h->h_norm);
    HIPCHK(hipHostMalloc((void**)&h->h_norm, sizeof(double) * 2 * d, kPolledHostFlags));
    if (!h->h_flag) {
        HIPCHK(hipHostMalloc((void**)&h->h_flag, 256, kPolledHostFlags));
        std::memset(h->h_flag, 0, 256);
    }

    int rc;
    if ((rc = dev_alloc(h, h->d_norm, (size_t)2 * d))) return rc;
    if (!h->d_watch) {
        if ((rc = dev_alloc(h, h->d_watch, 2))) return rc;
        HIPCHK(hipMemsetAsync(h->d_watch, 0, 16, h->stream));
    }
    h->dcap = d;
    h->loaded_d = 0;
    return GMG_OK;
}

int ensure_stage(gmg_handle h, size_t n_doubles) {
    if (n_doubles <= h->stage_cap) return GMG_OK;
    int rc;
    if ((rc = dev_alloc(h, h->d_stage, n_doubles))) return rc;
    h->stage_cap = n_doubles;
    return GMG_OK;
}

int ensure_host_stage(gmg_handle h, size_t n_doubles) {
    if (n_doubles <= h->h_stage_cap) return GMG_OK;
    for (int i = 0; i < 2; ++i) {
        if (h->h_stage[i]) (void)sync_hipHostFree(h->h_stage[i]);
        h->h_stage[i] = nullptr;
        HIPCHK(hipHostMalloc((void**)&h->h_stage[i], sizeof(double) * n_doubles, hipHostMallocDefault));
        if (!h->h_stage_ev[i]) HIPCHK(hipEventCreateWithFlags(&h->h_stage_ev[i], hipEventDisableTiming));
    }
    h->h_stage_cap = n_doubles;
    return GMG_OK;
}

inline void threaded_copy(double* dst, const double* src, size_t n, int threads) {
    const int T = (int)std::min<size_t>(std::max(1, std::min(threads, 16)), n / 65536 + 1);
    if (T <= 1) { std::memcpy(dst, src, sizeof(double) * n); return; }
    parallel_ranges(T, T, [&](int t0, int t1, int) {
        for (int t = t0; t < t1; ++t) {
            size_t lo = n * t / T, hi = n * (t + 1) / T;
            std::memcpy(dst + lo, src + lo, sizeof(double) * (hi - lo));
        }
    }, 1);
}

constexpr int kXferChunks = 6;
inline size_t xfer_chunk(size_t cnt) { return std::max<size_t>((cnt + kXferChunks - 1) / kXferChunks, (size_t)1 << 17); }
// ... 247 lines not shown
        const int ranks = (h->dist_ready && EnvSwitches::get().local_world <= 1) ? std::max(1, h->world) : 1;
        const int share = cpu_budget() / ranks;
        int threads = std::min(std::min(h->coarse.parts() * std::max(1, std::min(cols, 4)), 8), share - 1);
        if (env_threads > 0) threads = std::min(threads, env_threads);
        if (h->coarse_device || threads < 2) { h = nullptr; return; }
        if (!h->coarse_helper || h->coarse_helper->helpers() != threads - 1) h->coarse_helper.reset(new SpinTeam(threads - 1));
        h->coarse_helper->stay_near_caller();
        h->coarse_helper->arm();
    }
    ~HelperScope() { if (h) h->coarse_helper->disarm(); }
    HelperScope(const HelperScope&) = delete;
    HelperScope& operator=(const HelperScope&) = delete;
};

int coarse_host_serve(gmg_handle h) {
    if (!h->coarse_pending) return GMG_OK;
    h->coarse_pending = false;
    if (!h->coarse_warm) { h->coarse_warm_sink += h->coarse.warm(); h->coarse_warm = true; }
    const int w = wait_flag(h, 1);
    if (w == GMG_OK) coarse_host_solve(h, h->coarse_pending_d);
    __atomic_store_n(h->h_flag + 16, h->flag_seq[2], __ATOMIC_RELEASE);
    if (h->gate_shared) { h->gate_shared = false; --tl_gates_held; gate_mutex().unlock_shared(); }
    return w;
}

}
int gate_unwound(gmg_handle h) {
    if (h->coarse_pending) {
        h->coarse_pending = false;
        if (h->h_flag) __atomic_store_n(h->h_flag + 16, h->flag_seq[2], __ATOMIC_RELEASE);
    }
    if (h->gate_shared) { h->gate_shared = false; --tl_gates_held; gate_mutex().unlock_shared(); }
    return GMG_OK;
}
namespace {

template <class T = double>
int coarse_host_begin(gmg_handle h, int d) {
    Level& c = h->lv[h->L];
    const size_t cnt = (size_t)c.n_pad * d;
    double* rc = h->h_pinned;
    double* e = h->h_pinned + cnt;
    if (sizeof(T) == 4) launch_cvt(h, c.b32, c.b, cnt);
    if (polled(h)) {
        hipLaunchKernelGGL(gmgk::publish_to_host, dim3(1), dim3(gmgk::kBlock), 0, h->stream, c.b, rc, (int)cnt, h->h_flag + 8, ++h->flag_seq[1], (int)EnvSwitches::get().publish_fenced);
        const bool gate_off = h->cfg.stream_gate == 0;
        if (h->gate_ok && h->gate_proven && !gate_off) {
            if (!h->gate_shared) { gate_mutex().lock_shared(); h->gate_shared = true; ++tl_gates_held; }
            if (hipStreamWaitValue64(h->stream, h->h_flag + 16, ++h->flag_seq[2], hipStreamWaitValueGte, ~0ull) == hipSuccess) {
                hipLaunchKernelGGL(gmgk::fetch_from_host, dim3((unsigned)std::min<size_t>(8, (cnt + gmgk::kBlock - 1) / gmgk::kBlock)), dim3(gmgk::kBlock), 0, h->stream,
                                   (const double*)e, c.x, (int)cnt);
                if (sizeof(T) == 4) launch_cvt(h, c.x, c.x32, cnt);
                h->coarse_pending = true; h->coarse_pending_d = d;
                return GMG_OK;
            }
            (void)hipGetLastError();
            if (h->gate_shared) { h->gate_shared = false; --tl_gates_held; gate_mutex().unlock_shared(); }
            h->gate_ok = false; --h->flag_seq[2]; h->timing["gate_disabled"] = 1.0;
        }
        int w = wait_flag(h, 1);
        if (w) return w;
        if (h->poll) h->gate_proven = true;
        if (!polled(h)) HIPCHK(hipStreamSynchronize(h->stream));
    } else {
        HIPCHK(hipMemcpyAsync(rc, c.b, sizeof(double) * cnt, hipMemcpyDeviceToHost, h->stream));
        HIPCHK(hipStreamSynchronize(h->stream));
    }
    coarse_host_solve(h, d);
    HIPCHK(hipMemcpyAsync(c.x, e, sizeof(double) * cnt, hipMemcpyHostToDevice, h->stream));
    if (sizeof(T) == 4) launch_cvt(h, c.x, c.x32, cnt);
    return GMG_OK;
}

template <class T = double>
int coarse_host_roundtrip(gmg_handle h, int d) {
    int rc = coarse_host_begin<T>(h, d);
    return rc ? rc : coarse_host_serve(h);
}

int launch_residual_to_f32(gmg_handle h, int d, int type) {
    Level& l = h->lv[0];
    const double* w = type == 1 ? h->d_minv : (type == 2 ? h->d_mass : nullptr);
    const int nblk = norm_grid(l.Aoff.n_slices);
    for_col_chunks(d, [&](int c0, int dc) {
        DISPATCH_D(dc, DISPATCH_C16(l.Aoff.c16_sel(), hipLaunchKernelGGL((gmgk::residual_norm_slices<D, 1, C16>), dim3(nblk), dim3(gmgk::kNormWaves * 64), 0, h->stream,
                                          l.Aoff.slice_ptr, l.Aoff.col, l.Aoff.val, l.diag, l.b + (size_t)c0 * l.n_pad, l.x + (size_t)c0 * l.n_pad, w, l.n_pad,
                                          l.Aoff.n_slices, l.b32 + (size_t)c0 * l.n_pad, h->d_partials, l.Aoff.col16, l.Aoff.win_base, l.Aoff.c16_arg())));
        launch_reduce(h, nblk, dc, c0, c0 + 4 >= d);
    });
    if (!polled(h)) HIPCHK(hipMemcpyAsync(h->h_norm, h->d_norm, sizeof(double) * 2 * d, hipMemcpyDeviceToHost, h->stream));
    return GMG_OK;
}

enum { G_DOWN = 1, G_UP = 2, G_FULL = 3 };

template <class F>
int run_graph(gmg_handle h, int key, F&& enqueue) {
    if (!h->cfg.use_graph) { enqueue(); return GMG_OK; }
    auto it = h->graphs.find(key);
    if (it == h->graphs.end()) {
        hipGraph_t g = nullptr;
        hipGraphExec_t ge = nullptr;
        auto tc = clk::now();
        HIPCHK(hipStreamBeginCapture(h->stream, hipStreamCaptureModeThreadLocal));
        enqueue();
        HIPCHK(hipStreamEndCapture(h->stream, &g));
        h->timing["graph_capture_ms"] += ms_since(tc);
        tc = clk::now();
        HIPCHK(hipGraphInstantiate(&ge, g, nullptr, nullptr, 0));
        h->timing["graph_instantiate_ms"] += ms_since(tc);
        (void)hipGraphDestroy(g);
        it = h->graphs.emplace(key, ge).first;
    }
    HIPCHK(hipGraphLaunch(it->second, h->stream));
    return GMG_OK;
}

template <class T>
int vcycle_legs(gmg_handle h, int d, int norm_type, int key_salt, bool head_done, const CycleWatch* decide) {
    int rc;
    const int nt = norm_type < 0 ? 9 : norm_type;
    constexpr bool mixed = sizeof(T) == 4;
    const bool foldable = !mixed && norm_type >= 0 && h->cfg.post_iters > 0 && h->cfg.smoother == GMG_SMOOTHER_MULTICOLOR_GS && !h->lv[0].ord.blocked;
    const int fold_type = foldable ? norm_type : -1;
    auto head = [&] { if (mixed) (void)hipMemsetAsync(h->lv[0].x32, 0, sizeof(float) * (size_t)h->lv[0].n_pad * d, h->stream); };
    auto tail = [&](int& err, int folded) {
        if (mixed) {
            const size_t cnt = (size_t)h->lv[0].n_pad * d;
            hipLaunchKernelGGL(gmgk::add_correction, dim3((unsigned)((cnt + 255) / 256)), dim3(256), 0, h->stream, h->lv[0].x32, h->lv[0].x, (int64_t)cnt);
            err = launch_residual_to_f32(h, d, norm_type);
        } else if (norm_type >= 0) err = launch_norm(h, d, norm_type, folded, decide);
        prof_mark(h);
    };
    if (h->coarse_device) {
        int err = GMG_OK;
        rc = run_graph(h, key_salt + G_FULL * 10000 + d * 10 + nt, [&] {
            head();
            enqueue_down<T>(h, d,  0,  false, head_done);
            enqueue_coarse_device<T>(h, d);
            tail(err, enqueue_up<T>(h, d, 0, fold_type));
        });
        return rc ? rc : err;
    }
    if ((rc = run_graph(h, key_salt + G_DOWN * 10000 + d * 10, [&] { head(); enqueue_down<T>(h, d,  0,  false, head_done); }))) return rc;
    if ((rc = coarse_host_begin<T>(h, d))) return rc;
    int err = GMG_OK;
    rc = run_graph(h, key_salt + G_UP * 10000 + d * 10 + nt, [&] { tail(err, enqueue_up<T>(h, d, 0, fold_type)); });
    const int served = coarse_host_serve(h);
    return rc ? rc : (served ? served : err);
}

int vcycle_resident(gmg_handle h, int d, int norm_type, bool head_done = false, const CycleWatch* decide = nullptr) {
    if (h->cfg.inner_precision) return vcycle_legs<float>(h, d, norm_type, 100000, head_done, decide);
    return vcycle_legs<double>(h, d, norm_type, 0, head_done, decide);
}


int ensure_accel(gmg_handle h) {
    auto& a = h->accel;
    const int m = h->cfg.accelerate, n_pad = h->lv[0].n_pad, D = h->dcap;
    if (a.xk && a.depth == m && a.d == D && a.n_pad == n_pad) return GMG_OK;
    a = {};
    const size_t count = (size_t)n_pad * D;
    auto vec = [&](DevBuf<double>* p) -> int {
        int rc = dev_alloc(h, *p, count);
        if (rc == GMG_OK) HIPCHK(hipMemsetAsync(*p, 0, sizeof(double) * count, h->stream));
        return rc;
    };
    int rc;
    for (DevBuf<double>* p : {&a.xk, &a.r, &a.z0}) if ((rc = vec(p))) return rc;
// ... 85 lines not shown
```

### gravo_mg_amd/csrc/engine_state.hip.hpp

```cpp
#pragma once

inline std::shared_mutex& gate_mutex() { static std::shared_mutex* m = new std::shared_mutex(); return *m; }
static thread_local int tl_gates_held = 0;
struct DeviceSyncGuard {
    bool locked = false;
    DeviceSyncGuard() { if (tl_gates_held == 0) { gate_mutex().lock(); locked = true; } }
    ~DeviceSyncGuard() { if (locked) gate_mutex().unlock(); }
    DeviceSyncGuard(const DeviceSyncGuard&) = delete;
    DeviceSyncGuard& operator=(const DeviceSyncGuard&) = delete;
};
static inline hipError_t sync_hipFree(void* p) { DeviceSyncGuard g; return hipFree(p); }
static inline hipError_t sync_hipHostFree(void* p) { DeviceSyncGuard g; return hipHostFree(p); }
static inline hipError_t sync_hipStreamDestroy(hipStream_t s) { DeviceSyncGuard g; return hipStreamDestroy(s); }

struct DevPool {
    std::multimap<size_t, void*> parked;
    std::map<void*, size_t> size_of;
    size_t parked_bytes = 0, live_bytes = 0;
    size_t peak_live_bytes = 0;
    void reset_peak() { peak_live_bytes = live_bytes; }
    static size_t round_up(size_t b) { return (std::max<size_t>(b, 1) + 511) & ~(size_t)511; }
    hipError_t alloc(void** p, size_t bytes) {
        const size_t need = round_up(bytes);
        auto it = parked.lower_bound(need);
// ... 20 lines not shown
    void trim() {
        { DeviceSyncGuard g; for (auto& kv : parked) { (void)hipFree(kv.second); size_of.erase(kv.second); } }
        parked.clear(); parked_bytes = 0;
    }
};
static thread_local DevPool* tl_pool = nullptr;
struct PoolScope {
    DevPool* prev;
    explicit PoolScope(DevPool* p) : prev(tl_pool) { tl_pool = p; }
    ~PoolScope() { tl_pool = prev; }
};
static inline hipError_t dev_malloc(void** p, size_t bytes) { return tl_pool ? tl_pool->alloc(p, bytes) : hipMalloc(p, bytes); }
static inline hipError_t dev_free(void* p) { if (!p) return hipSuccess; if (tl_pool) { tl_pool->release(p); return hipSuccess; } return sync_hipFree(p); }

#include "dev_buf.hpp"
inline void dev_buf_release(void* p) { (void)dev_free(p); }

namespace {

struct DevSell {
    int n_slices = 0;
    int lpr = 1;
    int64_t stored = 0, nnz_real = 0;
    DevBuf<int64_t> slice_ptr;
    DevBuf<int> col;
    DevBuf<double> val;
    DevBuf<float> val32;
    DevBuf<int> row_of;
    DevBuf<unsigned> col16;
    DevBuf<int> win_base;
    int c16_dbits = 13;
    int c16_mode = 0;
    int c16_from = 0;
    bool resident = false;
    int uniform_w = 0;
    int c16_arg() const { return (c16_mode == 1 ? c16_from : 0) | uniform_w << 24 | (c16_dbits == 11 ? 1 << 30 : 0); }
    int c16_sel() const { return c16_mode ? c16_mode + (resident ? 2 : 0) : 0; }
};

struct DevCsr {
    int n_outer = 0;
    DevBuf<int> ptr, idx;
    DevBuf<double> val;
};

struct DevEll3 {
    int n = 0;
    DevBuf<int> cnt, col;
    DevBuf<double> val;
};

struct Level {
    int n = 0, n_pad = 0;
    int64_t nnz = 0;
    LevelOrdering ord;
    Compressed A;
    bool hostA_pattern = false, hostA_values = false;
    DevCsr dA;
    DevSell Aoff;
    DevBuf<double> diag;
    double cheby_lambda = 0.0;
    DevSell P, R;
    DevSell Ain, Aout;
    DevBuf<unsigned short> ain_col16;
    bool use_bcsr = false;
    DevBuf<int> bc_ptr, bc_mid, bc_col;
    DevBuf<double> bc_val;
    DevBuf<float> bc_val32;
    int bc_cap = 0;
    int64_t bc_nnz = 0;
    bool use_ep = false;
    DevBuf<int> ee_ptr, ee_col, ep_ptr;
    DevBuf<unsigned short> ep_col;
    DevBuf<double> ee_val, ep_val;
    DevBuf<float> ee_val32, ep_val32;
    int64_t ee_nnz = 0, ep_nnz = 0;
    int ep_cap_e = 0, ep_cap_l = 0;
    DevBuf<int> d_blk_begin, d_blk_ncolors;
    DevBuf<unsigned char> d_row_color;
    DevBuf<int> src_A, src_diag, src_ee, src_ep;
    DevBuf<int> d_new2old;
    DevBuf<int> d_old2new;
    DevBuf<int> d_blk_of_row;
    DevBuf<double> x, b, r, tmp;
    DevBuf<float> diag32, x32, b32, r32, tmp32;
};

}

struct FineGraph {
    int n = 0;
    RawVec<int> ptr, idx;
};

struct gmg_hierarchy_s {
    HierarchyResult res;
    std::shared_ptr<const FineGraph> graph;
    std::vector<int> fine_order;
};

struct DistP2P;

struct DistPlan {
    int rank = 0, world = 1, n_colors = 0;
    bool shard1 = false;
    uint64_t key[2] = {0, 0};
    std::vector<int> blk_owner;
    std::vector<std::vector<int>> own_blocks;
    std::vector<std::vector<int>> halo;
    std::vector<std::vector<int>> halo1, halo0r;
};

enum class LiveSystem { none, placeholder, system };

struct gmg_solver_s {
    DevPool pool;
    DistP2P* p2p = nullptr;
    double dbg_cheby_ratio = 0.0;
    int dbg_col16_uncovered = 0;
    gmg_config cfg;
    std::string err;
    bool has_device = false;
    int n_cus = 256;
    hipStream_t stream = nullptr;
    int L = -1;
    std::vector<Compressed> U;
    std::vector<char> U_set;
    std::vector<DevCsr> dU;
    std::vector<DevEll3> dE3;
    bool dU_ready = false;
    std::vector<PatchSet> patches;
    std::vector<int> cluster_order;
    DevBuf<int> d_cluster_order, d_cluster_inv;
    std::vector<int> bfs_order;
    std::shared_ptr<const FineGraph> fine_graph;
    bool mass_dirty = false;
    DevBuf<int> d_bfs_order, d_bfs_inv;
    int base_order_choice = 0;
    RawVec<int> reo_ptr, reo_idx;
    bool patches_ready = false;
    bool dU_flagged = false;
    std::vector<double> mass;
    std::vector<Level> lv;
    SupernodalLDLT coarse;
    LiveSystem live = LiveSystem::none;
    int dcap = 0;
    DevBuf<double> d_mass, d_minv;
    DevBuf<double> d_stage; size_t stage_cap = 0;
    double* h_stage[2] = {nullptr, nullptr}; size_t h_stage_cap = 0;
    void* bounce[2] = {nullptr, nullptr};
    hipEvent_t bounce_ev[2] = {nullptr, nullptr}; int bounce_flip = 0;
    hipEvent_t h_stage_ev[2] = {nullptr, nullptr}; int h_stage_flip = 0;
    hipEvent_t h_chunk_ev[16] = {};
    DevBuf<double> d_partials; int partial_blocks = 0;
    DevBuf<double> d_norm;
    struct AccelState {
        DevBuf<double> xk, r, z0;
        DevBuf<double> zs[gmg::kAccelMaxStored];
        DevBuf<double> qs[gmg::kAccelMaxStored];
        DevBuf<double> scal;
        DevBuf<double> partials;
        int depth = 0, d = 0, n_pad = 0;
    } accel;
    DevBuf<double> d_watch;
    double* h_pinned = nullptr; size_t pinned_cap = 0;
    double* h_norm = nullptr;
    unsigned long long* h_flag = nullptr; unsigned long long flag_seq[3] = {0, 0, 0};
    bool gate_ok = true;
    bool gate_proven = false;
    bool coarse_pending = false;
    bool gate_shared = false;
    bool coarse_warm = false;
    double coarse_warm_sink = 0.0;
    int coarse_pending_d = 0;
    bool poll = true;
    DevBuf<double> d_ainv;
    int ainv_n = 0, ainv_ld = 0;
    DevBuf<double> d_tri, d_tri_row, d_tri_col;
    DevBuf<int> d_tri_perm;
    int tri_n = -1;
    bool coarse_triangle = false;
    int64_t fused_restrictions = 0;
    bool coarse_device = false;
    std::vector<double> coarse_work;
    std::unique_ptr<SpinTeam> coarse_helper;
    std::map<std::string, double> timing;
    std::map<int, hipGraphExec_t> graphs;
    int loaded_d = 0;
    hipEvent_t ev0 = nullptr, ev1 = nullptr;
    hipStream_t aux_stream = nullptr;
    hipEvent_t aux_ev = nullptr;
    int* d_aux_err = nullptr;
    std::vector<int> rap_need;
    int* d_rap_order = nullptr;
    std::vector<int> rap_need2;
    int* d_rap_order2 = nullptr;
    std::vector<hipEvent_t> prof_ev;
    bool prof_on = false; int prof_n = 0;
    hipStream_t own_stream = nullptr;
    int rank = 0, world = 1;
    bool dist_ready = false;
// ... 253 lines not shown
```

### gravo_mg_amd/csrc/engine_system.hip.hpp

```cpp
namespace {

void drop_rap_order(gmg_handle h) {
    h->rap_need.clear(); h->rap_need2.clear();
    if (h->d_rap_order) { (void)sync_hipFree(h->d_rap_order); h->d_rap_order = nullptr; }
    if (h->d_rap_order2) { (void)sync_hipFree(h->d_rap_order2); h->d_rap_order2 = nullptr; }
}
bool ensure_rap_order(gmg_handle h) {
    if (!h->rap_need.empty() && h->d_rap_order) return true;
    drop_rap_order(h);
    const Compressed& U0 = h->U[0];
    const int nc = U0.n_outer, nf = U0.n_inner;
    if (nc <= 0 || nf <= 0) return false;
    const int nb = (nf + 63) / 64 + 1;
    std::vector<int> start((size_t)nb + 1, 0), order((size_t)nc), bucket((size_t)nc);
    for (int p = 0; p < nc; ++p) {
        int big = -1;
        for (int e = U0.ptr[p]; e < U0.ptr[p + 1]; ++e) big = std::max(big, U0.idx[e]);
        bucket[p] = big >= 0 ? (big >> 6) + 1 : 0;
        ++start[(size_t)bucket[p] + 1];
    }
    for (int b = 0; b < nb; ++b) start[b + 1] += start[b];
    h->rap_need.resize((size_t)nc);
    for (int p = 0; p < nc; ++p) { const int at = start[bucket[p]]++; order[at] = p; h->rap_need[at] = bucket[p] > 0 ? (bucket[p] - 1) * 64 + 63 : -1; }
    if (hipMalloc((void**)&h->d_rap_order, sizeof(int) * (size_t)nc) != hipSuccess) { (void)hipGetLastError(); h->d_rap_order = nullptr; h->rap_need.clear(); return false; }
// ... 321 lines not shown
    std::function<void(size_t, hipEvent_t)> after_chunk = [&](size_t bytes_done, hipEvent_t arrived) {
        const int64_t entries = (int64_t)(bytes_done / sizeof(double));
        const int rows = (int)(std::upper_bound(colptr, colptr + n + 1, (int)std::min<int64_t>(entries, colptr[n])) - colptr) - 1;
        const bool last = bytes_done >= val_bytes;
        auto ready = [&](const std::vector<int>& need) { return last ? (int)need.size() : (int)(std::upper_bound(need.begin(), need.end(), rows - 1) - need.begin()); };
        const int p_hi = ready(h->rap_need);
        if (p_hi - l1_rows_done < 32768 && !last) return;
        if (p_hi > l1_rows_done) {
            (void)hipStreamWaitEvent(h->aux_stream, arrived, 0);
            rap_rows_behind(h, 1, l1_rows_done, p_hi);
            l1_rows_done = p_hi;
        }
        if (pipeline2) {
            const int q_hi = ready(h->rap_need2);
            if (q_hi > l2_rows_done && (last || q_hi - l2_rows_done >= 4096)) { rap_rows_behind(h, 2, l2_rows_done, q_hi); l2_rows_done = q_hi; }
        }
    };
    if (pipeline) (void)hipMemsetAsync(h->d_aux_err, 0, sizeof(int), h->aux_stream);
    const int rc_up = h2d(h, h->lv[0].dA.val, e.val, val_bytes, pipeline ? &after_chunk : nullptr);
    if (pipeline) { (void)hipEventRecord(h->aux_ev, h->aux_stream); (void)hipStreamWaitEvent(h->stream, h->aux_ev, 0); }
    e.speculative = true;
    if (rc_up == GMG_OK) { e.rc_spec = refresh_system_values(h, n, e.val, t_all, true, l1_rows_done, l2_rows_done); e.spec_done = true; }
    keyed.get();
    e.have_key = true;
    return rc_up;
}

int enter_system(gmg_handle h, int n, const int* colptr, const int* rowidx, const double* val, clk::time_point t_all, SystemEntry& e) {
    e.colptr = colptr; e.rowidx = rowidx; e.val = val;
    const bool live = h->live != LiveSystem::none;
    const bool want_ahead = !(live && h->live_key_valid && (int)h->lv.size() == h->L + 1 && h->lv[0].n == n && (int64_t)colptr[n] == h->lv[0].nnz) &&
                            !h->ord_cache_valid && h->cfg.smoother == GMG_SMOOTHER_MULTICOLOR_GS && n >= (1 << 17) && h->cfg.color_ahead &&
                            !(h->cfg.block_rows > 0 && h->cfg.block_from_level <= 0);
    std::shared_future<int> inspected = std::async(std::launch::async, [h, n, colptr, rowidx] { return inspect_pattern(n, n, colptr, rowidx, h->cfg.host_threads); }).share();
    if (want_ahead) {
        const int64_t nnz_claimed = colptr[n];
        AheadColoring& ahead = e.ahead;
        ahead.ptr = colptr;
        ahead.fut = std::async(std::launch::async, [&ahead, inspected, n, colptr, rowidx, nnz_claimed] {
            if (inspected.get() != 0) return -2;
            return greedy_coloring_ahead(n, colptr, rowidx, nnz_claimed, ahead.pre.c8, ahead.stop);
        });
    }
    if (live && h->live_key_valid && h->refill_ready && (int)h->lv.size() == h->L + 1 && h->lv[0].n == n && colptr[0] == 0 && (int64_t)colptr[n] == h->lv[0].nnz &&
        h->lv[0].dA.val) {
        const int rc_up = speculate(h, n, e, t_all);
        if (rc_up != GMG_OK) { (void)inspected.get(); lose_live_system(h); return rc_up; }
    }
    if (!live && h->cfg.device_setup && h->cfg.device_rap && h->cfg.smoother == GMG_SMOOTHER_MULTICOLOR_GS && colptr[0] == 0 && colptr[n] >= n) {
        const int rc_up = upload_csr_raw(h, e.early_A0, n, colptr, rowidx, val);
        if (rc_up != GMG_OK) { (void)inspected.get(); return rc_up; }
    }
    const int what = inspected.get();
    if (what == 2) { if (e.speculative) lose_live_system(h); return fail(h, GMG_ERR_INVALID, "index out of range in LHS"); }
    if (what == 1) {
        e.canon = canonical_copy(n, n, colptr, rowidx, val, h->cfg.host_threads);
        e.colptr = e.canon.ptr.data(); e.rowidx = e.canon.idx.data(); e.val = e.canon.val.data();
        e.have_key = false;
        e.ahead.cancel();
        e.early_A0 = {};
        if (e.speculative) { e.speculative = e.spec_done = false; lose_live_system(h); h->refill_ready = false; }
    }
    return GMG_OK;
}

int values_only(gmg_handle h, int n, SystemEntry& e, clk::time_point t_all) {
    if (h->live == LiveSystem::none || !h->live_key_valid || !h->refill_ready || (int)h->lv.size() != h->L + 1 || h->lv[0].n != n) return 1;
    if (!e.have_key) { pattern_key(n, e.colptr, e.rowidx, h->cfg.host_threads, e.pat_key); e.have_key = true; }
    const bool keeps_fine_blocks = !(h->lv[0].ord.blocked && h->cfg.block_from_level >= 1) || stieltjes_signs(n, e.colptr, e.rowidx, e.val, h->cfg.host_threads);
    if (e.pat_key[0] != h->live_key[0] || e.pat_key[1] != h->live_key[1] || e.colptr[n] != h->lv[0].nnz || !keeps_fine_blocks) return 1;
    const bool from_placeholder = h->live == LiveSystem::placeholder;
    const int rc = e.spec_done ? e.rc_spec : refresh_system_values(h, n, e.val, t_all);
    if (rc == GMG_OK) {
        h->live = LiveSystem::system;
        h->timing["setup_structure_prepared"] = from_placeholder ? 1.0 : 0.0;
        h->timing["t_verdict"] = h->timing["setup_total"] = ms_since(t_all);
        h->timing["upload"] = h->timing["setup_total"] - h->timing["reduction"];
    } else if (rc != 1) {
        lose_live_system(h); h->refill_ready = false;
    }
    return rc;
}

void stash_orderings(gmg_handle h) {
    h->ord_cache.resize(h->L + 1);
    for (int k = 0; k <= h->L; ++k) h->ord_cache[k] = std::move(h->lv[k].ord);
    h->ord_cache_key[0] = h->live_key[0]; h->ord_cache_key[1] = h->live_key[1];
    h->ord_cache_valid = true;
}

struct LevelStage {
    SellHost sa, sin, sout, sp, sr;
    BlockCsrHost bc, bin;
    bool use_bcsr = false, use_ep = false;
    std::vector<unsigned short> ep16;
    std::vector<double> dg;
    std::vector<unsigned short> c16;
    std::string err;
    bool ok = true;
    double ms_order = 0, ms_sell = 0;
};

class FullSetup {
public:
    FullSetup(gmg_handle h, SystemEntry& e, int n, clk::time_point t_all, bool placeholder)
        : h(h), e(e), n(n), L(h->L), colptr(e.colptr), rowidx(e.rowidx), val(e.val), t_all(t_all), placeholder(placeholder),
          mc(h->cfg.smoother == GMG_SMOOTHER_MULTICOLOR_GS), part(h->part_world > 1), device_setup(h->cfg.device_setup != 0),
          stage(L + 1), ord_done(L + 1), op_done(L), tr_done(L) {}
    ~FullSetup() {
        try { join(); } catch (...) {}
        if (factor_done.valid()) factor_done.wait();
    }
    int run() {
        h->timing["setup_wait_ordering"] = 0.0; h->timing["setup_device_layout"] = 0.0;
        if (part && !(device_setup && h->cfg.device_rap && mc)) return fail(h, GMG_ERR_UNSUPPORTED, std::string("a partitioned set-up needs device_setup = 1, device_rap = 1 and the multicolour smoother (this handle runs ") + smoother_name(h->cfg) + ")");
        h->partitioned = false;
        h->pool.reset_peak();
        int rc;
        if (device_setup) {
            if ((rc = ensure_device_transfers(h))) return rc;
            if (h->dU_flagged) device_setup = false;
            if (part && !device_setup) return fail(h, GMG_ERR_UNSUPPORTED, "a partitioned set-up has no host fallback (a prolongation row has more than 3 entries)");
        }
        start_tasks();
        if ((rc = renumber_level0())) return rc;
        spawn_level(0);
        if ((rc = galerkin_chain())) return rc;
        h->timing["reduction"] = ms_since(t0);
        factor_done = spawn_coarse_factor(h, ord_hit, &ms_factor).share();
        auto tl = clk::now();
        if (device_setup) { device_layouts(); ms_h2d = ms_since(tl); }
        if (!device_setup) host_uploads();
        join();
        h->timing["t_lhs_copied"] = ms_lhs_copied;
        h->timing["setup_colored_ahead"] = colored_ahead.load();
        mark("tasks_joined");
        const bool factor_ok = factor_done.get();
        mark("factor_joined");
        (void)hipStreamSynchronize(h->stream);
        if (rc_all != GMG_OK) return err_all.empty() ? rc_all : fail(h, rc_all, err_all);
        if (!factor_ok) return fail(h, GMG_ERR_NUMERIC, "coarsest operator is singular (LDL^T hit a zero pivot)");
        h->coarse_work.assign((size_t)h->lv[L].A.n_outer * 4, 0.0);
        h->timing["setup_ordering"] = 0.0; h->timing["setup_sell"] = 0.0;
        for (int k = 0; k <= L; ++k) h->timing["setup_ordering_l" + std::to_string(k)] = stage[k].ms_order;
        for (int k = 0; k <= L; ++k) { h->timing["setup_ordering"] = std::max(h->timing["setup_ordering"], stage[k].ms_order); h->timing["setup_sell"] = std::max(h->timing["setup_sell"], stage[k].ms_sell); }
        h->timing["setup_h2d"] = ms_h2d;
        const int nblk = std::max(kNormBlocks, grid_for((h->lv[0].n_pad + 63) / 64));
        if (nblk > h->partial_blocks) {
            if ((rc = dev_alloc(h, h->d_partials, (size_t)nblk * 8))) return rc;
            h->partial_blocks = nblk;
        }
        return GMG_OK;
    }
    int commit() {
        HIPCHK(hipStreamSynchronize(h->stream));
        h->timing["device_bytes_peak"] = (double)h->pool.peak_live_bytes;
        if (part) {
            const bool s1 = h->plan && h->plan->shard1;
            h->lv[0].dA = {};
            if (s1) h->lv[1].dA = {};
            if (!h->dU.empty()) { h->dU[0] = {}; h->dE3[0] = {}; }
            for (int k = 0; k <= (s1 ? 1 : 0); ++k) { h->lv[k].d_old2new = {}; h->lv[k].d_blk_of_row = {}; }
            h->pool.trim_large((size_t)4 << 20);
            h->partitioned = true;
        }
        h->timing["device_bytes"] = (double)h->pool.live_bytes;
        h->live_key[0] = e.pat_key[0]; h->live_key[1] = e.pat_key[1];
        h->live_key_valid = true;
        h->ord_cache_valid = false;
        h->live = LiveSystem::system;
        h->refill_ready = device_setup && device_rap_ok && h->cfg.device_setup != 0 && !part;
        return GMG_OK;
    }
    double ms_factor = 0;
    bool inverse_built = false;

private:
    void start_tasks() {
        const bool need_host_A0 = !device_setup || !h->cfg.device_rap;
        h->lv[0].n = n; h->lv[0].nnz = colptr[n];
        if (need_host_A0) {
            lhs_copied = std::async(std::launch::async, [this] { h->lv[0].A.assign(n, n, colptr, rowidx, val); ms_lhs_copied = ms_since(t_all); }).share();
            h->lv[0].hostA_pattern = h->lv[0].hostA_values = true;
        }
        stage_ready = std::async(std::launch::async, [h = h, n = n] { (void)hipSetDevice(h->cfg.device); return ensure_host_stage(h, (size_t)n); });
        if (!e.have_key) pattern_key(n, colptr, rowidx, h->cfg.host_threads, e.pat_key);
        mark("pattern_key");
        blocked0 = fine_level_blocked(h, n, colptr, rowidx, val);
        h->timing["fine_level_blocked"] = blocked0 ? 1.0 : 0.0;
        ord_hit = h->ord_cache_valid && (int)h->ord_cache.size() == L + 1 && e.pat_key[0] == h->ord_cache_key[0] && e.pat_key[1] == h->ord_cache_key[1] &&
                  h->ord_cache[0].blocked == blocked0;
        h->timing["setup_ordering_cached"] = ord_hit ? 1.0 : 0.0;
        if (ord_hit || blocked0 || !mc || e.ahead.ptr != colptr) e.ahead.cancel();
        h->timing["setup_values_only"] = 0.0;
        h->ord_cache_valid = false;
        if (!h->patches_ready && !ord_hit) patches_done = std::async(std::launch::async, [h = h] { build_patches(h); }).share();
    }
    int renumber_level0() {
        t0 = clk::now();
        reorder0 = mc && !ord_hit && !blocked0 && wants_locality_reorder(PatternView{n, colptr, rowidx}, h->cfg.reorder_fine);
        if (reorder0) e.ahead.cancel();
        if (e.early_A0.ptr && device_setup && h->cfg.device_rap) { h->lv[0].dA = std::move(e.early_A0); e.early_A0 = {}; A0_uploaded = true; }
        const bool have_bfs = (int)h->bfs_order.size() == n, have_cluster = h->patches_ready && (int)h->cluster_order.size() == n;
        h->base_order_choice = (reorder0 && h->patches_ready && have_bfs && !have_cluster) ? 1 : 0;
        if (reorder0 && have_bfs && have_cluster && !(device_setup && h->cfg.device_rap)) {
            unsigned long long sc[2], sb[2];
            order_gather_score_host(PatternView{n, colptr, rowidx}, h->cluster_order, 4096, sc);
            order_gather_score_host(PatternView{n, colptr, rowidx}, h->bfs_order, 4096, sb);
            h->base_order_choice = (sc[1] && sb[1] && (double)sb[0] / (double)sb[1] < (double)sc[0] / (double)sc[1]) ? 1 : 0;
            h->timing["base_order_score_cluster"] = sc[1] ? (double)sc[0] / (double)sc[1] : 0.0;
            h->timing["base_order_score_bfs"] = sb[1] ? (double)sb[0] / (double)sb[1] : 0.0;
            h->timing["base_order_choice"] = h->base_order_choice;
        }
        if (reorder0 && device_setup && h->cfg.device_rap && (have_cluster || (h->patches_ready && have_bfs))) {
            int rc = A0_uploaded ? GMG_OK : upload_csr_raw(h, h->lv[0].dA, n, colptr, rowidx, val);
            if (rc == GMG_OK) { A0_uploaded = true; rc = choose_base_order(h, h->lv[0].dA, n); }
            if (rc == GMG_OK) rc = device_permute_pattern(h, h->lv[0].dA, n, colptr[n]);
            if (rc != GMG_OK) return rc;
            permuted0 = true;
            mark("permuted_pattern");
        }
        return GMG_OK;
    }
    int galerkin_chain() {
// ... 358 lines not shown
```

### gravo_mg_amd/csrc/host_plan.hpp

```cpp
#pragma once
#include <chrono>
#include <cstdio>
#include <cstdlib>
#include <algorithm>
#include <atomic>
#include <cmath>
#include <cstdint>
#include <cstdlib>
#include <future>
#include <memory>
#include <numeric>
#include <string>
#include <vector>

#include <stdlib.h>
#include <sys/mman.h>

#include "host_sparse.hpp"

namespace gmg {

constexpr int kSlice = 64;

template <class T>
// ... 599 lines not shown
                }
                key[i] = best >= 0 ? pos[best] : nc;
            }
        });
        std::vector<int> start((size_t)nc + 2, 0);
        for (int i = 0; i < nf; ++i) start[key[i] + 1]++;
        for (int c = 0; c <= nc; ++c) start[c + 1] += start[c];
        order.assign(nf, 0);
        for (int i = 0; i < nf; ++i) order[start[key[i]]++] = i;
        pos.assign(nf, 0);
        parallel_ranges(nf, T, [&](int lo, int hi, int) { for (int r = lo; r < hi; ++r) pos[order[r]] = r; });
    }
    return order;
}

inline std::vector<int> bfs_point_order(const int* neigh, int n, int K) {
    std::vector<int> order;
    order.reserve((size_t)n);
    std::vector<unsigned char> seen((size_t)n, 0);
    for (int s = 0; s < n; ++s) {
        if (seen[s]) continue;
        seen[s] = 1; order.push_back(s);
        for (size_t h = order.size() - 1; h < order.size(); ++h) {
            if (h + 8 < order.size()) __builtin_prefetch(neigh + (size_t)order[h + 8] * K);
            const int* row = neigh + (size_t)order[h] * K;
            for (int j = 0; j < K; ++j) {
                const int w = row[j];
                if (w < 0) break;
                if (!seen[w]) { seen[w] = 1; order.push_back(w); }
            }
        }
    }
    return order;
}

template <class Mat>
inline void order_gather_score_host(const Mat& A, const std::vector<int>& order, int n_win, unsigned long long out[2]) {
    const int n = A.n_outer;
    out[0] = out[1] = 0;
    if (n < 512) return;
    std::vector<int> inv((size_t)n);
    for (int r = 0; r < n; ++r) inv[order[r]] = r;
    constexpr int kMaxRow = 32;
    std::vector<int> p((size_t)64 * kMaxRow), len(64);
    for (int w = 0; w < n_win; ++w) {
        const int start = (int)((long long)w * (n - 256) / n_win);
        int maxlen = 0;
        for (int l = 0; l < 64; ++l) {
            const int v = order[start + 4 * l], b = A.ptr[v];
            len[l] = std::min(A.ptr[v + 1] - b, kMaxRow);
            for (int q = 0; q < len[l]; ++q) p[(size_t)l * kMaxRow + q] = inv[A.idx[b + q]];
            std::sort(p.begin() + (size_t)l * kMaxRow, p.begin() + (size_t)l * kMaxRow + len[l]);
            maxlen = std::max(maxlen, len[l]);
        }
        for (int j = 0; j < maxlen; ++j)
            for (int l = 0; l < 64; ++l) {
                if (j >= len[l]) continue;
                ++out[1];
                const int line = p[(size_t)l * kMaxRow + j] >> 4;
                bool first = true;
                for (int m = 0; m < l && first; ++m) first = !(j < len[m] && (p[(size_t)m * kMaxRow + j] >> 4) == line);
                out[0] += first ? 1 : 0;
            }
    }
}

inline double mean_index_distance_table(const int* neigh, int n, int K) {
    const int step = std::max(1, n / 65536);
    double sum = 0.0; long cnt = 0;
    for (int i = 0; i < n; i += step)
        for (int j = 0; j < K && neigh[(size_t)i * K + j] >= 0; ++j) { sum += std::abs(neigh[(size_t)i * K + j] - i); ++cnt; }
    return cnt ? sum / cnt : 0.0;
}

inline LevelOrdering identity_ordering(int n) {
    LevelOrdering o;
    o.n = n; o.n_pad = round_up(std::max(n, 1), kSlice); o.n_colors = 1;
    o.color_begin = {0, o.n_pad};
    o.new2old.assign(o.n_pad, -1);
    o.old2new.resize(n);
    for (int i = 0; i < n; ++i) { o.new2old[i] = i; o.old2new[i] = i; }
    return o;
}
struct RowStage {
    std::vector<int64_t> ptr;
    RawVec<int> idx;
    RawVec<double> val;
};

template <class LenFn>
inline void stage_lengths(int np, RowStage& st, LenFn&& len_of) {
    st.ptr.assign((size_t)np + 1, 0);
    parallel_ranges(np, hw_threads(), [&](int lo, int hi, int) {
        for (int r = lo; r < hi; ++r) st.ptr[r + 1] = len_of(r);
    });
    for (int r = 0; r < np; ++r) st.ptr[r + 1] += st.ptr[r];
    st.idx.resize((size_t)st.ptr[np]);
    st.val.resize((size_t)st.ptr[np]);
}

inline SellHost csr_to_sell(int n_rows_pad, int n_cols, const RowStage& st, int sort_sigma, int lpr = 1) {
    const std::vector<int64_t>& ptr = st.ptr;
    const int rps = kSlice / lpr;
    SellHost s;
    s.lpr = lpr;
    s.n_rows_pad = n_rows_pad; s.n_cols = n_cols; s.n_slices = n_rows_pad / rps;
    s.nnz_real = ptr[n_rows_pad];
    std::vector<int> order;
    const bool sorted = sort_sigma > 0;
    if (sorted) {
        order.resize(n_rows_pad);
        const int nwin = (n_rows_pad + sort_sigma - 1) / sort_sigma;
        parallel_ranges(nwin, hw_threads(), [&](int lo, int hi, int) {
            for (int wi = lo; wi < hi; ++wi) {
                int w = wi * sort_sigma, we = std::min(n_rows_pad, w + sort_sigma);
                std::iota(order.begin() + w, order.begin() + we, w);
                std::stable_sort(order.begin() + w, order.begin() + we, [&](int a, int b) { return (ptr[a + 1] - ptr[a]) > (ptr[b + 1] - ptr[b]); });
            }
        });
        s.row_of = order;
    }
    auto row_at = [&](int i) { return sorted ? order[i] : i; };
    s.slice_ptr.assign((size_t)s.n_slices + 1, 0);
    parallel_ranges(s.n_slices, hw_threads(), [&](int lo, int hi, int) {
        for (int sl = lo; sl < hi; ++sl) {
            int64_t w = 0;
            for (int l = 0; l < rps; ++l) { int r = row_at(sl * rps + l); w = std::max<int64_t>(w, (ptr[r + 1] - ptr[r] + lpr - 1) / lpr); }
            s.slice_ptr[sl + 1] = w * kSlice;
        }
    });
    for (int sl = 0; sl < s.n_slices; ++sl) s.slice_ptr[sl + 1] += s.slice_ptr[sl];
    s.col.resize((size_t)s.stored());
    s.val.resize((size_t)s.stored());
    parallel_ranges(s.n_slices, hw_threads(), [&](int lo, int hi, int) {
        for (int sl = lo; sl < hi; ++sl) {
            const int64_t base = s.slice_ptr[sl];
            const int64_t w = (s.slice_ptr[sl + 1] - base) / kSlice;
            for (int l = 0; l < rps; ++l) {
                const int r = row_at(sl * rps + l);
                const int64_t len = ptr[r + 1] - ptr[r], p0 = ptr[r];
                for (int64_t e = 0; e < w * lpr; ++e) {
                    const int64_t q = base + (e / lpr) * kSlice + l * lpr + (e % lpr);
                    if (e < len) { s.col[q] = st.idx[p0 + e]; s.val[q] = st.val[p0 + e]; }
                    else { s.col[q] = 0; s.val[q] = 0.0; }
                }
            }
        }
    });
    return s;
}

inline void sort_row(std::vector<std::pair<int, double>>& row) {
    std::sort(row.begin(), row.end(), [](const std::pair<int, double>& a, const std::pair<int, double>& b) { return a.first < b.first; });
}

inline bool build_operator_sell(const Compressed& A, const LevelOrdering& o, int lpr, SellHost& out,
                                std::vector<double>& diag, std::string& err) {
    if (lpr != 4) lpr = 1;
    const int np = o.n_pad;
    diag.assign(np, 1.0);
    std::atomic<int> bad_row{-1};
    RowStage st;
    stage_lengths(np, st, [&](int r) -> int64_t {
        int old = o.new2old[r];
        if (old < 0) return 0;
        int64_t len = 0;
// ... 165 lines not shown
```

### gravo_mg_amd/csrc/host_sparse.hpp

```cpp
#pragma once
#include <algorithm>
#include <cstdint>
#include <cstdio>
#include <cstdlib>
#include <cstring>
#include <atomic>
#include <condition_variable>
#include <deque>
#include <functional>
#include <memory>
#include <mutex>
#include <pthread.h>
#include <sched.h>
#include <stdlib.h>
#include <sys/mman.h>
#include <new>
#include <string>
#include <thread>
#include <type_traits>
#include <utility>
#include <vector>

namespace gmg {

template <class T>
struct default_init_allocator : std::allocator<T> {
    template <class U> struct rebind { using other = default_init_allocator<U>; };
    using std::allocator<T>::allocator;
    static constexpr size_t kHuge = (size_t)2 << 20;
    T* allocate(size_t n) {
        const size_t bytes = n * sizeof(T);
        if (bytes >= 2 * kHuge) {
            void* q = nullptr;
            const size_t rounded = (bytes + kHuge - 1) & ~(kHuge - 1);
            if (posix_memalign(&q, kHuge, rounded) == 0) {
                (void)madvise(q, rounded, MADV_HUGEPAGE);
                return static_cast<T*>(q);
            }
            throw std::bad_alloc();
        }
        void* q = std::malloc(std::max<size_t>(bytes, 1));
        if (!q) throw std::bad_alloc();
        return static_cast<T*>(q);
    }
    void deallocate(T* p, size_t) noexcept { std::free(p); }
    template <class U> void construct(U* p) noexcept(std::is_nothrow_default_constructible<U>::value) { ::new (static_cast<void*>(p)) U; }
    template <class U, class... Args> void construct(U* p, Args&&... args) { ::new (static_cast<void*>(p)) U(std::forward<Args>(args)...); }
};
using IndexVec = std::vector<int, default_init_allocator<int>>;
using ValueVec = std::vector<double, default_init_allocator<double>>;

struct Compressed {
    int n_outer = 0;
    int n_inner = 0;
    std::vector<int> ptr;
    IndexVec idx;
    ValueVec val;
    int nnz() const { return ptr.empty() ? 0 : ptr[n_outer]; }
    void assign(int nouter, int ninner, const int* p, const int* i, const double* v) {
        n_outer = nouter; n_inner = ninner;
        ptr.assign(p, p + nouter + 1);
        idx.assign(i, i + ptr[nouter]);
        val.assign(v, v + ptr[nouter]);
    }
};

struct EnvSwitches {
    int host_threads = 0, local_world = 0, ldlt_threads = 0;
    bool trace_setup = false, trace_ldlt = false, trace_ctor = false, poll = true, segv_backtrace = false;
    bool block_smallest_last = true;
    double p2p_timeout_s = 0.0;
    bool p2p_fence_free = false, publish_fenced = false, p2p_shared_device = false;
    int symv_rows = 0, symv_strides = 0;
    bool symv_v2 = true;
    bool tri_nt = false;
    double cheby_ratio = 0.0;
    static const EnvSwitches& get() {
        static const EnvSwitches v = [] {
            EnvSwitches e;
            auto num = [](const char* name) { const char* s = std::getenv(name); return s ? std::atof(s) : -1.0; };
            if (num("GMG_HOST_THREADS") > 0) e.host_threads = (int)num("GMG_HOST_THREADS");
            if (num("LOCAL_WORLD_SIZE") > 1) e.local_world = (int)num("LOCAL_WORLD_SIZE");
            if (num("GMG_LDLT_THREADS") > 0) e.ldlt_threads = (int)num("GMG_LDLT_THREADS");
            if (const char* t = std::getenv("GMG_BLOCK_COLOURING")) e.block_smallest_last = std::string(t) != "bfs";
            if (const char* t = std::getenv("GMG_TRACE")) { const std::string s(t); e.trace_setup = s.find("setup") != std::string::npos; e.trace_ldlt = s.find("ldlt") != std::string::npos; e.trace_ctor = s.find("ctor") != std::string::npos; }
            e.poll = num("GMG_POLL") != 0.0;
            if (num("GMG_P2P_TIMEOUT_S") > 0) e.p2p_timeout_s = num("GMG_P2P_TIMEOUT_S");
            e.segv_backtrace = num("GMG_SEGV_BACKTRACE") > 0;
            e.p2p_fence_free = num("GMG_P2P_FENCE_FREE") > 0;
            e.publish_fenced = num("GMG_PUBLISH_FENCED") > 0;
            e.p2p_shared_device = num("GMG_P2P_SHARED_DEVICE") > 0;
            e.symv_rows = std::max(0, (int)num("GMG_SYMV_ROWS"));
            e.symv_strides = std::max(0, (int)num("GMG_SYMV_STRIDES"));
            e.symv_v2 = (int)num("GMG_SYMV_V2") != 0;
            e.tri_nt = (int)num("GMG_TRI_NT") > 0;
            if (const char* t = std::getenv("GMG_CHEBY_RATIO")) {
                const double r = std::atof(t);
                if (r > 1.0 && r <= 1e6) e.cheby_ratio = r;
                else std::fprintf(stderr, "[gmg] GMG_CHEBY_RATIO=%s ignored: the ratio must be > 1 and <= 1e6 (the compiled default is used)\n", t);
            }
            return e;
        }();
        return v;
    }
};

inline int cpu_budget() {
    static const int v = [] {
        long t = (long)std::thread::hardware_concurrency();
        if (t <= 0) t = 1;
        cpu_set_t set;
        if (sched_getaffinity(0, sizeof(set), &set) == 0) { const int c = CPU_COUNT(&set); if (c > 0) t = std::min<long>(t, c); }
        auto apply_v2 = [&](const std::string& file) {
            if (FILE* f = std::fopen(file.c_str(), "r")) {
                char q[64]; long long period = 0;
                if (std::fscanf(f, "%63s %lld", q, &period) == 2 && std::strcmp(q, "max") != 0 && period > 0) {
                    const long long quota = std::atoll(q);
                    if (quota > 0) t = std::min<long>(t, (long)std::max<long long>(1, (quota + period - 1) / period));
                }
                std::fclose(f);
            }
        };
        auto read_ll = [](const char* file, long long& out) {
            FILE* f = std::fopen(file, "r");
            if (!f) return false;
            const bool ok = std::fscanf(f, "%lld", &out) == 1;
            std::fclose(f);
            return ok;
        };
        apply_v2("/sys/fs/cgroup/cpu.max");
        if (FILE* f = std::fopen("/proc/self/cgroup", "r")) {
            char line[1024];
            while (std::fgets(line, sizeof(line), f)) {
                if (std::strncmp(line, "0::", 3) != 0) continue;
                std::string path(line + 3);
                while (!path.empty() && (path.back() == '\n' || path.back() == '/')) path.pop_back();
                while (!path.empty()) {
                    apply_v2("/sys/fs/cgroup" + path + "/cpu.max");
                    const size_t cut = path.find_last_of('/');
                    path = cut == std::string::npos ? std::string() : path.substr(0, cut);
                }
            }
            std::fclose(f);
        }
        long long quota = 0, period = 0;
        if (read_ll("/sys/fs/cgroup/cpu/cpu.cfs_quota_us", quota) && read_ll("/sys/fs/cgroup/cpu/cpu.cfs_period_us", period) && quota > 0 && period > 0)
            t = std::min<long>(t, (long)std::max<long long>(1, (quota + period - 1) / period));
        const EnvSwitches& env = EnvSwitches::get();
        if (env.local_world > 1) t = std::max<long>(1, t / env.local_world);
        if (env.host_threads > 0) t = env.host_threads;
        return (int)std::max<long>(1, t);
    }();
    return v;
}

inline int hw_threads() { return std::min(cpu_budget(), 128); }

class WorkerPool {
public:
    static WorkerPool& instance() {
        static WorkerPool* p = new WorkerPool();
        return *p;
    }
    struct Batch {
        std::atomic<int> pending{0};
    };
    void submit(Batch& b, std::function<void()> fn) {
        b.pending.fetch_add(1, std::memory_order_relaxed);
        {
            std::lock_guard<std::mutex> g(m_);
            ensure_workers();
            q_.emplace_back(&b, std::move(fn));
        }
        cv_.notify_one();
    }
    void wait(Batch& b) {
        while (b.pending.load(std::memory_order_acquire) > 0) {
            std::pair<Batch*, std::function<void()>> job;
// ... 141 lines not shown
```

### gravo_mg_amd/csrc/kernels.hip.hpp

```cpp
#pragma once
#include <hip/hip_runtime.h>
#include <stdint.h>
#include "solve_rule.hpp"
#include "coarse_triangle.hpp"

namespace gmgk {

constexpr int kBlock = 256;
constexpr int kWavesPerBlock = kBlock / 64;

__device__ __forceinline__ int wave_slice(int n_slices_total, int xcd_swizzle) {
    int nblk = gridDim.x;
    int b = blockIdx.x;
    if (xcd_swizzle && (nblk & 7) == 0) b = (b & 7) * (nblk >> 3) + (b >> 3);
    int w = b * kWavesPerBlock + (threadIdx.x >> 6);
    (void)n_slices_total;
    return __builtin_amdgcn_readfirstlane(w);
}

template <int D, int XI> __device__ __forceinline__ int64_t x_at(int c, int d, int ld) { return XI ? (int64_t)c * D + d : c + (int64_t)d * ld; }

__device__ __forceinline__ float fma_of(float a, float b, float c) { return __builtin_fmaf(a, b, c); }
__device__ __forceinline__ double fma_of(double a, double b, double c) { return __builtin_fma(a, b, c); }

template <class T, int D, int W, int XI = 0>
__device__ __forceinline__ void row_dot_group(const int* __restrict__ cp, const T* __restrict__ vp, const T* x, int ld,
                                              T (&acc)[D]) {
    int c[W];
    T v[W];
#pragma unroll
    for (int j = 0; j < W; ++j) { c[j] = __builtin_nontemporal_load(cp + j * 64); v[j] = __builtin_nontemporal_load(vp + j * 64); }
    T xv[W][D];
#pragma unroll
    for (int j = 0; j < W; ++j)
#pragma unroll
        for (int d = 0; d < D; ++d) xv[j][d] = x[x_at<D, XI>(c[j], d, ld)];
#pragma unroll
    for (int j = 0; j < W; ++j)
#pragma unroll
        for (int d = 0; d < D; ++d) acc[d] = fma_of(v[j], xv[j][d], acc[d]);
}

template <int D> struct DotGroup { static constexpr int value = D >= 4 ? 4 : (D == 3 ? 6 : 8); };
template <class T, int D, int G = DotGroup<D>::value, int XI = 0>
__device__ __forceinline__ void row_dot(const int64_t* __restrict__ slice_ptr, const int* __restrict__ col,
                                        const T* __restrict__ val, const T* x, int ld, int s, int lane,
                                        T (&acc)[D], int uw = 0) {
    const int64_t p0 = uw ? (int64_t)s * (uw << 6) : slice_ptr[s];
    int w = uw ? uw : (int)((slice_ptr[s + 1] - p0) >> 6);
    const int* cp = col + p0 + lane;
    const T* vp = val + p0 + lane;
#pragma unroll
    for (int c = 0; c < D; ++c) acc[c] = 0.0;
    for (; w >= G; w -= G, cp += G * 64, vp += G * 64) row_dot_group<T, D, G, XI>(cp, vp, x, ld, acc);
    switch (w) {
        case 1: row_dot_group<T, D, 1, XI>(cp, vp, x, ld, acc); break;
        case 2: row_dot_group<T, D, 2, XI>(cp, vp, x, ld, acc); break;
        case 3: row_dot_group<T, D, 3, XI>(cp, vp, x, ld, acc); break;
        case 4: if (G > 4) row_dot_group<T, D, 4, XI>(cp, vp, x, ld, acc); break;
        case 5: if (G > 4) row_dot_group<T, D, 5, XI>(cp, vp, x, ld, acc); break;
        case 6: if (G > 4) row_dot_group<T, D, 6, XI>(cp, vp, x, ld, acc); break;
        case 7: if (G > 4) row_dot_group<T, D, 7, XI>(cp, vp, x, ld, acc); break;
        default: break;
    }
}

template <class T, int D, int W, bool FLAGS, int XI = 0, bool KEEP = false>
__device__ __forceinline__ void row_dot_group16(const unsigned* __restrict__ cp, const int* __restrict__ cp32, const T* __restrict__ vp, const T* x, int ld,
                                                int basev, int dbits, int& fallback, T (&acc)[D]) {
    unsigned pk[(W + 1) / 2];
    T v[W];
#pragma unroll
    for (int q = 0; q < (W + 1) / 2; ++q) pk[q] = KEEP ? cp[q * 64] : __builtin_nontemporal_load(cp + q * 64);
#pragma unroll
    for (int j = 0; j < W; ++j) v[j] = KEEP ? vp[j * 64] : __builtin_nontemporal_load(vp + j * 64);
    if constexpr (FLAGS) { if (fallback < 0) fallback = __builtin_amdgcn_readfirstlane(basev) < 0 ? 1 : 0; }
    int c[W];
    if (FLAGS && fallback) {
#pragma unroll
        for (int j = 0; j < W; ++j) c[j] = __builtin_nontemporal_load(cp32 + j * 64);
    } else {
        const unsigned mask = (1u << dbits) - 1u;
#pragma unroll
        for (int j = 0; j < W; ++j) {
            const unsigned u = (j & 1) ? pk[j >> 1] >> 16 : pk[j >> 1] & 0xffffu;
            c[j] = __builtin_amdgcn_ds_bpermute((int)((u >> dbits) << 2), basev) + (int)(u & mask);
        }
    }
    T xv[W][D];
#pragma unroll
    for (int j = 0; j < W; ++j)
#pragma unroll
        for (int d = 0; d < D; ++d) xv[j][d] = x[x_at<D, XI>(c[j], d, ld)];
#pragma unroll
    for (int j = 0; j < W; ++j)
#pragma unroll
        for (int d = 0; d < D; ++d) acc[d] = fma_of(v[j], xv[j][d], acc[d]);
}

template <class T, int D, bool FLAGS, int G = DotGroup<D>::value, int XI = 0, bool KEEP = false>
// ... 792 lines not shown
                for (int c = 0; c < D; ++c) s_[c] += vj * xs[c][cj];
            }
            quad_reduce<T, D>(s_);
            if (writer) {
#pragma unroll
                for (int c = 0; c < D; ++c) xs[c][lrow] = (rhs[c] - s_[c]) * dg;
            }
        }
        __syncthreads();
    }
    if (active && writer) {
#pragma unroll
        for (int c = 0; c < D; ++c) x_out[row + (int64_t)c * ld] = xs[c][lrow];
    }
}

template <class T, int D>
__global__ __launch_bounds__(kBlock) void jacobi_sweep(const int64_t* __restrict__ slice_ptr, const int* __restrict__ col,
                                                       const T* __restrict__ val, const T* __restrict__ diag,
                                                       const T* __restrict__ b, const T* __restrict__ x_in,
                                                       T* __restrict__ x_out, int ld, int n_slices, T omega,
                                                       int xcd_swizzle) {
    const int s = wave_slice(n_slices, xcd_swizzle);
    if (s >= n_slices) return;
    const int lane = threadIdx.x & 63;
    const int row = s * 64 + lane;
    T acc[D];
    row_dot<T, D>(slice_ptr, col, val, x_in, ld, s, lane, acc);
    const T dg = diag[row];
#pragma unroll
    for (int c = 0; c < D; ++c) {
        const T xi = x_in[row + (int64_t)c * ld];
        x_out[row + (int64_t)c * ld] = gs_row(b[row + (int64_t)c * ld], acc[c], dg, omega, xi);
    }
}

template <class T, int D, bool FIRST, int C16 = 0>
__global__ __launch_bounds__(kBlock) void cheby_step(const int64_t* __restrict__ slice_ptr, const int* __restrict__ col,
                                                     const T* __restrict__ val, const T* __restrict__ diag,
                                                     const T* __restrict__ b, const T* __restrict__ x_in,
                                                     T* __restrict__ x_out, T* __restrict__ p, int ld, int n_slices, T c1, T c2,
                                                     int xcd_swizzle, const unsigned* __restrict__ col16 = nullptr,
                                                     const int* __restrict__ win_base = nullptr, int c16_arg = 0) {
    const int s = wave_slice(n_slices, xcd_swizzle);
    if (s >= n_slices) return;
    const int lane = threadIdx.x & 63;
    const int row = s * 64 + lane;
    T acc[D];
    row_dot_sel<T, D, C16>(slice_ptr, col, col16, win_base, c16_arg, val, x_in, ld, s, lane, acc);
    const T dg = diag[row];
#pragma unroll
    for (int c = 0; c < D; ++c) {
        const int64_t i = row + (int64_t)c * ld;
        const T xi = x_in[i];
        const T z = (b[i] - row_ax(acc[c], dg, xi)) / dg;
        T pn = c2 * z;
        if constexpr (!FIRST) pn = c1 * p[i] + pn;
        p[i] = pn;
        x_out[i] = xi + pn;
    }
}

template <class T, int D, int MODE, int LPR, int C16 = 0, int YI = 0>
__device__ __forceinline__ void spmv_full_slice(const int64_t* __restrict__ slice_ptr, const int* __restrict__ col, const T* __restrict__ val,
                                                const T* __restrict__ diag, const T* __restrict__ b, const T* __restrict__ x, T* __restrict__ y,
                                                int ld, int s, const unsigned* __restrict__ col16 = nullptr, const int* __restrict__ win_base = nullptr, int c16_arg = 0) {
    const int lane = threadIdx.x & 63;
    const int row = s * (64 / LPR) + lane / LPR;
    T acc[D];
    row_dot_sel<T, D, C16>(slice_ptr, col, col16, win_base, c16_arg, val, x, ld, s, lane, acc);
    if (LPR == 4) { quad_reduce<T, D>(acc); if (lane & 3) return; }
    const T dg = diag[row];
#pragma unroll
    for (int c = 0; c < D; ++c) {
        const T ax = row_ax(acc[c], dg, x[row + (int64_t)c * ld]);
        y[YI ? (int64_t)row * D + c : row + (int64_t)c * ld] = MODE == 1 ? b[row + (int64_t)c * ld] - ax : ax;
    }
}
template <class T, int D, int MODE, int LPR, int C16 = 0, int YI = 0>
__global__ __launch_bounds__(kBlock) void spmv_full(const int64_t* __restrict__ slice_ptr, const int* __restrict__ col,
                                                    const T* __restrict__ val, const T* __restrict__ diag,
                                                    const T* __restrict__ b, const T* __restrict__ x,
                                                    T* __restrict__ y, int ld, int slice_begin, int slice_end,
                                                    int xcd_swizzle, const unsigned* __restrict__ col16 = nullptr, const int* __restrict__ win_base = nullptr, int c16_arg = 0) {
    const int s = slice_begin + wave_slice(slice_end - slice_begin, xcd_swizzle);
    if (s >= slice_end) return;
    spmv_full_slice<T, D, MODE, LPR, C16, YI>(slice_ptr, col, val, diag, b, x, y, ld, s, col16, win_base, c16_arg);
}
template <class T, int D, int MODE, int LPR>
__global__ __launch_bounds__(kBlock) void spmv_full_list(const int64_t* __restrict__ slice_ptr, const int* __restrict__ col,
                                                         const T* __restrict__ val, const T* __restrict__ diag,
                                                         const T* __restrict__ b, const T* __restrict__ x,
                                                         T* __restrict__ y, int ld, const int* __restrict__ slices, int n_list) {
    const int i = wave_slice(n_list, 1);
    if (i >= n_list) return;
    spmv_full_slice<T, D, MODE, LPR>(slice_ptr, col, val, diag, b, x, y, ld, __builtin_amdgcn_readfirstlane(slices[i]));
}

template <class T, int D, int ADD, int LPR, int C16 = 0, int XI = 0>
__device__ __forceinline__ void transfer_slice(const int64_t* __restrict__ slice_ptr, const int* __restrict__ col, const T* __restrict__ val,
                                               const int* __restrict__ row_of, const T* __restrict__ x, int ldx, T* __restrict__ y, int ldy, int s,
                                               const unsigned* __restrict__ col16 = nullptr, const int* __restrict__ win_base = nullptr, int c16_arg = 0) {
    const int lane = threadIdx.x & 63;
    const int srow = s * (64 / LPR) + lane / LPR;
    T acc[D];
    row_dot_sel<T, D, C16, (LPR == 4 ? 8 : DotGroup<D>::value), XI>(slice_ptr, col, col16, win_base, c16_arg, val, x, ldx, s, lane, acc);
    if (LPR == 4) { quad_reduce<T, D>(acc); if (lane & 3) return; }
    const int row = (!ADD && row_of) ? row_of[srow] : srow;
    if (row < 0) return;
#pragma unroll
    for (int c = 0; c < D; ++c) {
        if (ADD) y[row + (int64_t)c * ldy] += acc[c];
        else y[row + (int64_t)c * ldy] = acc[c];
    }
}
template <class T, int D, int ADD, int LPR, int C16 = 0, int XI = 0>
__global__ __launch_bounds__(kBlock) void transfer(const int64_t* __restrict__ slice_ptr, const int* __restrict__ col,
                                                   const T* __restrict__ val, const int* __restrict__ row_of,
                                                   const T* __restrict__ x, int ldx, T* __restrict__ y, int ldy,
                                                   int slice_begin, int slice_end, int xcd_swizzle, const unsigned* __restrict__ col16 = nullptr,
                                                   const int* __restrict__ win_base = nullptr, int c16_arg = 0) {
    const int s = slice_begin + wave_slice(slice_end - slice_begin, xcd_swizzle);
    if (s >= slice_end) return;
    transfer_slice<T, D, ADD, LPR, C16, XI>(slice_ptr, col, val, row_of, x, ldx, y, ldy, s, col16, win_base, c16_arg);
}
template <class T, int D, int ADD, int LPR>
__global__ __launch_bounds__(kBlock) void transfer_list(const int64_t* __restrict__ slice_ptr, const int* __restrict__ col,
                                                        const T* __restrict__ val, const int* __restrict__ row_of,
                                                        const T* __restrict__ x, int ldx, T* __restrict__ y, int ldy,
                                                        const int* __restrict__ slices, int n_list) {
    const int i = wave_slice(n_list, 1);
    if (i >= n_list) return;
    transfer_slice<T, D, ADD, LPR>(slice_ptr, col, val, row_of, x, ldx, y, ldy, __builtin_amdgcn_readfirstlane(slices[i]));
}

#if defined(__HIP_DEVICE_COMPILE__) && !defined(__gfx942__) && !defined(__gfx950__)
#error "kernels.hip.hpp: the fence-free publication sequence (publish_order) relies on gfx942 / gfx950 store completion semantics"
#endif
__device__ __forceinline__ void publish_order(int fenced) {
    asm volatile("s_waitcnt vmcnt(0)" ::: "memory");
    if (fenced) __builtin_amdgcn_fence(__ATOMIC_RELEASE, "");
}
__device__ __forceinline__ void consume_order(int fenced) {
    if (fenced) __builtin_amdgcn_fence(__ATOMIC_ACQUIRE, "");
}

constexpr int kReduceBlock = 1024;
constexpr int kReduceMaxComp = 8;
__device__ __forceinline__ void block_reduce_partials(const double* __restrict__ partials, int n_blocks, int ncomp, double* __restrict__ out,
                                                      double (*red)[kReduceMaxComp]) {
    const int wave = threadIdx.x >> 6, lane = threadIdx.x & 63;
    double v[kReduceMaxComp];
#pragma unroll
    for (int c = 0; c < kReduceMaxComp; ++c) v[c] = 0.0;
    for (int i0 = threadIdx.x; i0 < n_blocks; i0 += 4 * kReduceBlock) {
        double t[4][kReduceMaxComp];
#pragma unroll
        for (int u = 0; u < 4; ++u) {
            const int i = i0 + u * kReduceBlock;
#pragma unroll
            for (int c = 0; c < kReduceMaxComp; ++c) t[u][c] = (c < ncomp && i < n_blocks) ? partials[(int64_t)i * ncomp + c] : 0.0;
        }
#pragma unroll
        for (int u = 0; u < 4; ++u)
#pragma unroll
            for (int c = 0; c < kReduceMaxComp; ++c) v[c] += t[u][c];
    }
#pragma unroll
    for (int c = 0; c < kReduceMaxComp; ++c) {
        if (c >= ncomp) break;
        double t = v[c];
#pragma unroll
        for (int off = 32; off > 0; off >>= 1) t += __shfl_down(t, off, 64);
        if (lane == 0) red[wave][c] = t;
    }
    __syncthreads();
    if ((int)threadIdx.x < ncomp) {
        double t = 0.0;
#pragma unroll
        for (int w = 0; w < kReduceBlock / 64; ++w) t += red[w][threadIdx.x];
        __hip_atomic_store(reinterpret_cast<unsigned long long*>(out + threadIdx.x), (unsigned long long)__double_as_longlong(t), __ATOMIC_RELAXED, __HIP_MEMORY_SCOPE_SYSTEM);
    }
}

struct SolveWatch {
    int* go;
    unsigned long long* host_go;
    double* least;
    double tol;
    int mode;
    int norm_type, d, cycles_done;
};
__global__ __launch_bounds__(kReduceBlock) void reduce_partials(const double* __restrict__ partials, int n_blocks, int ncomp,
                                                                double* __restrict__ out, unsigned long long* flag, unsigned long long seq, int fenced,
                                                                SolveWatch watch = SolveWatch{nullptr, nullptr, nullptr, 0.0, 0, 0, 0, 0}) {
    __shared__ double red[kReduceBlock / 64][kReduceMaxComp];
    block_reduce_partials(partials, n_blocks, ncomp, out, red);
    if (watch.go != nullptr && threadIdx.x == 0) {
        int go = 1;
        if (watch.mode == 1) {
            double s[kReduceMaxComp];
            for (int c = 0; c < ncomp; ++c) {
                double t = 0.0;
#pragma unroll
                for (int w = 0; w < kReduceBlock / 64; ++w) t += red[w][c];
// ... 247 lines not shown
        else v = gathered[sg.off + i];
        vec[sg.idx[k] + (int64_t)c * ld] = v;
    }
}

template <bool SYS>
__global__ __launch_bounds__(64) void coll_sum_ranks(const double* __restrict__ gathered, long long chunk, int world, int rank, const double* __restrict__ mine,
                                                     int n, double* __restrict__ out) {
    const int t = threadIdx.x;
    if (t >= n) return;
    double sum = 0.0;
    for (int r = 0; r < world; ++r) {
        if (r == rank) { sum += mine[t]; continue; }
        if (SYS) sum += __longlong_as_double((long long)__hip_atomic_load(reinterpret_cast<const unsigned long long*>(gathered) + (long long)r * chunk + t, __ATOMIC_RELAXED, __HIP_MEMORY_SCOPE_SYSTEM));
        else sum += gathered[(long long)r * chunk + t];
    }
    out[t] = sum;
}

__global__ __launch_bounds__(kBlock) void publish_to_host(const double* __restrict__ src, double* __restrict__ dst, int n,
                                                          unsigned long long* flag, unsigned long long seq, int fenced) {
    for (int i = threadIdx.x; i < n; i += kBlock)
        __hip_atomic_store(reinterpret_cast<unsigned long long*>(dst + i), (unsigned long long)__double_as_longlong(src[i]), __ATOMIC_RELAXED, __HIP_MEMORY_SCOPE_SYSTEM);
    publish_order(fenced);
    __syncthreads();
    if (threadIdx.x == 0) __hip_atomic_store(flag, seq, __ATOMIC_RELAXED, __HIP_MEMORY_SCOPE_SYSTEM);
}

__global__ __launch_bounds__(kBlock) void fetch_from_host(const double* src, double* __restrict__ dst, int n) {
    const unsigned long long* s = reinterpret_cast<const unsigned long long*>(src);
    for (int i = blockIdx.x * kBlock + threadIdx.x; i < n; i += gridDim.x * kBlock)
        dst[i] = __longlong_as_double((long long)__hip_atomic_load(s + i, __ATOMIC_RELAXED, __HIP_MEMORY_SCOPE_SYSTEM));
}

template <int D>
__global__ __launch_bounds__(kBlock) void residual_norm_partials(const int64_t* __restrict__ slice_ptr, const int* __restrict__ col,
                                                                 const double* __restrict__ val, const double* __restrict__ diag,
                                                                 const double* __restrict__ b, const double* __restrict__ x,
                                                                 const double* __restrict__ weight, int ld, int slice_begin,
                                                                 int slice_end, double* __restrict__ partials) {
    __shared__ double red[kWavesPerBlock][2 * D];
    const int wave = threadIdx.x >> 6, lane = threadIdx.x & 63;
    double sums[2 * D];
#pragma unroll
    for (int c = 0; c < 2 * D; ++c) sums[c] = 0.0;
    for (int s = slice_begin + __builtin_amdgcn_readfirstlane(blockIdx.x * kWavesPerBlock + wave); s < slice_end;
         s += gridDim.x * kWavesPerBlock) {
        const int row = s * 64 + lane;
        double acc[D];
        row_dot<double, D>(slice_ptr, col, val, x, ld, s, lane, acc);
        const double dg = diag[row];
        const double w = weight ? weight[row] : 1.0;
#pragma unroll
        for (int c = 0; c < D; ++c) {
            const double bi = b[row + (int64_t)c * ld];
            const double r = row_ax(acc[c], dg, x[row + (int64_t)c * ld]) - bi;
            sums[2 * c] += norm_term(r, w);
            sums[2 * c + 1] += norm_term(bi, w);
        }
    }
#pragma unroll
    for (int c = 0; c < 2 * D; ++c) {
        double v = sums[c];
#pragma unroll
        for (int off = 32; off > 0; off >>= 1) v += __shfl_down(v, off, 64);
        if (lane == 0) red[wave][c] = v;
    }
    __syncthreads();
    if (threadIdx.x < 2 * D) {
        double v = 0.0;
#pragma unroll
        for (int w2 = 0; w2 < kWavesPerBlock; ++w2) v += red[w2][threadIdx.x];
        partials[(int64_t)blockIdx.x * (2 * D) + threadIdx.x] = v;
    }
}

constexpr int kNormWaves = 16;
template <int D, int MODE, int C16 = 0>
__global__ __launch_bounds__(kNormWaves * 64, 8) void residual_norm_slices(const int64_t* __restrict__ slice_ptr, const int* __restrict__ col,
                                                               const double* __restrict__ val, const double* __restrict__ diag,
                                                               const double* __restrict__ b, const double* __restrict__ x,
                                                               const double* __restrict__ weight, int ld, int n_slices,
                                                               float* __restrict__ r32, double* __restrict__ partials,
                                                               const unsigned* __restrict__ col16 = nullptr, const int* __restrict__ win_base = nullptr, int c16_arg = 0) {
    __shared__ double red[kNormWaves][2 * D];
    const int wave = threadIdx.x >> 6, lane = threadIdx.x & 63;
    int nblk = gridDim.x, bb = blockIdx.x;
    if ((nblk & 7) == 0) bb = (bb & 7) * (nblk >> 3) + (bb >> 3);
    const int s = __builtin_amdgcn_readfirstlane(bb * kNormWaves + wave);
    double sums[2 * D];
#pragma unroll
    for (int c = 0; c < 2 * D; ++c) sums[c] = 0.0;
    if (s < n_slices) {
        const int row = s * 64 + lane;
        double acc[D];
        row_dot_sel<double, D, C16>(slice_ptr, col, col16, win_base, c16_arg, val, x, ld, s, lane, acc);
        const double dg = diag[row];
        const double w = weight ? weight[row] : 1.0;
#pragma unroll
        for (int c = 0; c < D; ++c) {
            const double bi = b[row + (int64_t)c * ld];
            double r;
            if (MODE == 1) { r = bi - row_ax(acc[c], dg, x[row + (int64_t)c * ld]); r32[row + (int64_t)c * ld] = (float)r; }
            else r = row_ax(acc[c], dg, x[row + (int64_t)c * ld]) - bi;
            sums[2 * c] = norm_term(r, w);
            sums[2 * c + 1] = norm_term(bi, w);
        }
    }
    block_sums_store<kNormWaves, D>(sums, red, wave, lane, bb, partials);
}

__global__ void add_correction(const float* __restrict__ e, double* __restrict__ x, int64_t n) {
    const int64_t i = (int64_t)blockIdx.x * blockDim.x + threadIdx.x;
    if (i < n) x[i] += (double)e[i];
}

__global__ void cvt_f64_to_f32(const double* __restrict__ src, float* __restrict__ dst, int64_t n) {
    const int64_t i = (int64_t)blockIdx.x * blockDim.x + threadIdx.x;
    if (i < n) dst[i] = (float)src[i];
}

__global__ void cvt_f32_to_f64(const float* __restrict__ src, double* __restrict__ dst, int64_t n) {
    const int64_t i = (int64_t)blockIdx.x * blockDim.x + threadIdx.x;
    if (i < n) dst[i] = (double)src[i];
}

__global__ void permute_in(const double* __restrict__ src, int n, const int* __restrict__ new2old, double* __restrict__ dst,
                           int ld, int n_pad, int D) {
    const int r = blockIdx.x * blockDim.x + threadIdx.x;
    if (r >= n_pad) return;
    const int old = new2old[r];
    for (int c = 0; c < D; ++c) dst[r + (int64_t)c * ld] = old >= 0 ? src[old + (int64_t)c * n] : 0.0;
}

__global__ void permute_out(const double* __restrict__ src, int ld, int n_pad, const int* __restrict__ new2old,
                            double* __restrict__ dst, int n, int D) {
    const int r = blockIdx.x * blockDim.x + threadIdx.x;
    if (r >= n_pad) return;
    const int old = new2old[r];
    if (old < 0) return;
    for (int c = 0; c < D; ++c) dst[old + (int64_t)c * n] = src[r + (int64_t)c * ld];
}

template <int D, bool X0>
__global__ __launch_bounds__(256) void permute_in2_strided(const double* rhs, int64_t rhs_rs, int64_t rhs_cs, const double* x0, int64_t x0_rs, int64_t x0_cs,
                                                           const int* __restrict__ new2old, double* __restrict__ b, double* __restrict__ x, int ld,
                                                           int n_pad, int d) {
    const int r = blockIdx.x * blockDim.x + threadIdx.x;
    if (r >= n_pad) return;
    const int old = new2old[r];
    const double* pb = rhs + (int64_t)(old >= 0 ? old : 0) * rhs_rs;
    const double* px = X0 ? x0 + (int64_t)(old >= 0 ? old : 0) * x0_rs : nullptr;
    if (D > 0) {
        double vb[D > 0 ? D : 1], vx[D > 0 ? D : 1];
#pragma unroll
        for (int c = 0; c < D; ++c) {
            vb[c] = old >= 0 ? pb[(int64_t)c * rhs_cs] : 0.0;
            vx[c] = X0 ? (old >= 0 ? px[(int64_t)c * x0_cs] : 0.0) : vb[c];
        }
#pragma unroll
        for (int c = 0; c < D; ++c) { b[r + (int64_t)c * ld] = vb[c]; x[r + (int64_t)c * ld] = vx[c]; }
    } else {
        for (int c = 0; c < d; ++c) {
            const double vb = old >= 0 ? pb[(int64_t)c * rhs_cs] : 0.0;
            const double vx = X0 ? (old >= 0 ? px[(int64_t)c * x0_cs] : 0.0) : vb;
            b[r + (int64_t)c * ld] = vb;
            x[r + (int64_t)c * ld] = vx;
        }
    }
}

// ... 290 lines not shown
```

### include/gravomg_hip.h

```cpp
#ifndef GRAVOMG_HIP_H
#define GRAVOMG_HIP_H

#include <stdint.h>

#ifdef __cplusplus
extern "C" {
#endif

typedef struct gmg_solver_s* gmg_handle;
typedef struct gmg_hierarchy_s* gmg_hierarchy;

typedef enum {
    GMG_OK = 0,
    GMG_ERR_INVALID = -1,
    GMG_ERR_NO_DEVICE = -2,
    GMG_ERR_HIP = -3,
    GMG_ERR_STATE = -4,
    GMG_ERR_NUMERIC = -5,
    GMG_ERR_UNSUPPORTED = -6,
    GMG_DIVERGED = 1
} gmg_status;

enum { GMG_SMOOTHER_MULTICOLOR_GS = 0, GMG_SMOOTHER_JACOBI = 1, GMG_SMOOTHER_CHEBYSHEV = 2 };
enum { GMG_COARSE_HOST_LDLT = 0, GMG_COARSE_DEVICE_INVERSE = 1, GMG_COARSE_AUTO = 2, GMG_COARSE_DEVICE_TRIANGLE = 3 };

typedef struct {
    int device;
    int smoother;
    double jacobi_omega;
    int pre_iters;
    int post_iters;
    int coarse_mode;
    int use_graph;
    int sigma;
    int row_align;
    int block_rows;
    int block_lanes;
    int block_from_level;
    int device_setup;
    int device_rap;
    int reorder_fine;
    int inner_precision;
    int block_csr;
    int host_threads;
    int verbose;
    double gs_omega;
    int restrict_sigma;
    int block_ep;
    int dist_shard_levels;
    int block_fine;
    int fine_col16;
    int stream_gate;
    int dist_exchange;
    int prepare_structure;
    int fuse_restrict_sweep;
    int speculate_head;
    int uniform_slices;
    int color_ahead;
    int accelerate;
} gmg_config;

int gmg_config_default(gmg_config* cfg);
int gmg_config_size(void);
int gmg_create(const gmg_config* cfg, gmg_handle* out);
void gmg_destroy(gmg_handle h);
const char* gmg_last_error(gmg_handle h);
int gmg_host_threads(void);
int gmg_device_count(void);

int gmg_set_num_levels(gmg_handle h, int L);
int gmg_set_prolongation(gmg_handle h, int k, int n_fine, int n_coarse, const int* colptr, const int* rowidx, const double* val);
int gmg_set_mass(gmg_handle h, int n, const double* mass_diag);
int gmg_set_system(gmg_handle h, int n, const int* colptr, const int* rowidx, const double* val);
int gmg_set_system_values_device(gmg_handle h, const double* d_val, int64_t nnz);

int gmg_num_levels(gmg_handle h);
int gmg_level_info(gmg_handle h, int k, int* n, int64_t* nnz, int* n_colors, int* n_pad);
int gmg_get_level_operator(gmg_handle h, int k, int* colptr, int* rowidx, double* val);
int gmg_get_level_ordering(gmg_handle h, int k, int* new2old, int* color_begin);
int gmg_get_level_blocks(gmg_handle h, int k, int* n_blocks, int* blk_begin, unsigned char* row_color);
int gmg_get_timing(gmg_handle h, const char* key, double* out);

int gmg_smooth(gmg_handle h, int k, const double* b, double* x, int d, int iters);
int gmg_smooth_residual(gmg_handle h, int k, const double* b, double* x, int d, int iters, int from_zero, double* r);
int gmg_residual(gmg_handle h, int k, const double* b, const double* x, int d, double* r);
int gmg_spmv(gmg_handle h, int k, const double* x, int d, double* y);
int gmg_restrict(gmg_handle h, int k, const double* r, int d, double* rc);
int gmg_prolong_add(gmg_handle h, int k, const double* e, int d, double* x);
int gmg_coarse_solve(gmg_handle h, const double* rc, int d, double* e);
int gmg_residual_norm(gmg_handle h, const double* b, const double* x, int d, int type, double* out);

int gmg_vcycle(gmg_handle h, const double* b, double* x, int d);
int gmg_solve(gmg_handle h, const double* rhs, double* x, int d, double tol, int stop_type, int max_iter,
              int* iters_out, double* residue_out, double* conv);
int gmg_solve_x0_rhs(gmg_handle h, const double* rhs, double* x, int d, double tol, int stop_type, int max_iter,
                     int* iters_out, double* residue_out, double* conv);
typedef struct {
    const double* rhs;  int64_t rhs_row_stride, rhs_col_stride;
    const double* x0;   int64_t x0_row_stride,  x0_col_stride;
    double*       x;    int64_t x_row_stride,   x_col_stride;
} gmg_device_vectors;
int gmg_solve_device(gmg_handle h, const gmg_device_vectors* v, int d, double tol, int stop_type, int max_iter,
                     int* iters_out, double* residue_out, double* conv);

int gmg_load_problem(gmg_handle h, const double* b, const double* x0, int d);
int gmg_run_cycles(gmg_handle h, int n_cycles, int stop_type, double* residues);
int gmg_fetch_solution(gmg_handle h, double* x);

int gmg_set_stream(gmg_handle h, void* hip_stream);
int gmg_dist_setup(gmg_handle h, int rank, int world);
int gmg_dist_partition(gmg_handle h, int rank, int world);
int gmg_dist_bind(gmg_handle h, double* x0, double* b0, double* r0, int d);
int gmg_dist_smooth_color(gmg_handle h, int c);
int gmg_dist_residual_own(gmg_handle h);
int gmg_dist_coarse_cycle(gmg_handle h);
int gmg_dist_prolong_own(gmg_handle h);
int gmg_dist_norm_partial(gmg_handle h, int type, double* sums);
int gmg_dist_all_rows(gmg_handle h, int on);
int gmg_dist_gather(gmg_handle h, const double* src, const int64_t* idx, int64_t n, double* dst);
int gmg_dist_scatter(gmg_handle h, const double* src, const int64_t* pos, const int64_t* idx, int64_t n, double* dst);

int gmg_p2p_blob_bytes(void);
int gmg_p2p_prepare(gmg_handle h, int rank, int world, int d);
int gmg_p2p_export(gmg_handle h, void* blob_out);
int gmg_p2p_connect(gmg_handle h, const void* blobs);
int gmg_p2p_rccl_unique_id(void* id_out_128_bytes);
int gmg_p2p_connect_rccl(gmg_handle h, const void* id_128_bytes);
int gmg_p2p_load(gmg_handle h, const double* b, const double* x0);
int gmg_p2p_cycles(gmg_handle h, int n_cycles, int stop_type, double* residues);
int gmg_p2p_fetch(gmg_handle h, double* x);
int gmg_p2p_solve(gmg_handle h, const double* b, double* x, double tol, int stop_type, int max_iter, int* iters_out, double* residue_out);
int gmg_p2p_stat(gmg_handle h, const char* key, double* out);
int gmg_p2p_set_smoother(gmg_handle h, int mode);
int gmg_p2p_set_fences(gmg_handle h, int fenced);

typedef struct {
    double ratio;
    int lower_bound;
    int check_voronoi;
    int nested;
    int sampling;
// ... 32 lines not shown
```

### include/gravomg_hip_internal.h

```cpp
#ifndef GRAVOMG_HIP_INTERNAL_H
#define GRAVOMG_HIP_INTERNAL_H

#include "gravomg_hip.h"

#ifdef __cplusplus
extern "C" {
#endif

int gmg_debug_sell_info(gmg_handle h, int k, int which, int64_t* info);
int gmg_debug_sell_copy(gmg_handle h, int k, int which, int64_t* slice_ptr, int* col, double* val, int* row_of, double* diag);
int gmg_debug_col16_copy(gmg_handle h, int which, int64_t* info, unsigned* col16, int* win_base);

int gmg_debug_set(gmg_handle h, const char* key, double value);

int gmg_debug_select_parents(int nf, int nc, int Kc, int ntri, int weighting, int nested, const double* P, const double* Pc, const int* nearest,
                             const int* sample, const int* cadj_ptr, const int* cadj, const int* tris, const int* tof_ptr, const int* tof,
                             const int* NBc, int mode, unsigned char* cnt, unsigned char* kind, int* col, double* w);
int gmg_hierarchy_debug_row_kinds(gmg_hierarchy hh, int k, int* out);

int gmg_host_galerkin(int n, const int* a_colptr, const int* a_rowidx, const double* a_val,
                      int n_coarse, const int* u_colptr, const int* u_rowidx, const double* u_val,
                      int* c_colptr, int* c_rowidx, double* c_val);

int gmg_debug_device_galerkin(gmg_handle h, int n, const int* a_colptr, const int* a_rowidx, const double* a_val, const double* a_val2, int n_coarse,
                              const int* u_colptr, const int* u_rowidx, const double* u_val, int64_t cap, int* c_colptr, int* c_rowidx, double* c_val,
                              double* c_val2, int* status);

int gmg_host_plan_level(int n, const int* colptr, const int* rowidx, const double* val, int mode, int block_rows, int sigma,
                        int64_t* info, int* new2old, int* color_begin, int* blk_begin, unsigned char* row_color);

int gmg_host_fine_block_rule(int n, const int* colptr, const int* rowidx, const double* val, int* blocked, int* reason);

int gmg_bench_kernel(gmg_handle h, int kind, int k, int d, int reps, double* ms_avg, int* launches_out);
int gmg_profile_cycle(gmg_handle h, int stop_type, int reps, double* ms_out, int n_out);
int gmg_algorithmic_bytes(gmg_handle h, int kind, int k, int d, double* bytes_out);

int gmg_p2p_bench_kind(gmg_handle h, const char* kind, int reps, double* ms_avg);

int gmg_p2p_debug_collective_roundtrip(gmg_handle h, double* max_abs_diff, long long* doubles);

int gmg_host_ldlt_probe(int n, const int* colptr, const int* rowidx, const double* val, const double* b, int reps, char* report, int cap);

#ifdef __cplusplus
}
#endif
#endif
```

Baseline: 0.5773.

## Reorder fine-level workgroups spatially across colors for cache locality

Adds a host-built permutation table that remaps workgroup indices on the finest level so blocks from different color ranges with the same relative position run close together in time. The table also spreads blocks round-robin across the 8 XCDs. It is used by the full-residual SpMV and the residual-norm kernels by default (mask 3), and can be enabled for prolongation (bit 4). The aim is better L2/MALL reuse of x entries shared by spatially nearby rows from different colors. The cost is an extra indirect load per workgroup and more setup work.

Result: no change. 0.5762, median of 3 (-0.2%).

```diff
diff --git a/gravo_mg_amd/cabi.py b/gravo_mg_amd/cabi.py
--- a/gravo_mg_amd/cabi.py
+++ b/gravo_mg_amd/cabi.py
@@ -34,7 +34,7 @@
         ("row_align", C.c_int), ("block_rows", C.c_int), ("block_lanes", C.c_int), ("block_from_level", C.c_int),
         ("device_setup", C.c_int), ("device_rap", C.c_int), ("reorder_fine", C.c_int), ("inner_precision", C.c_int), ("block_csr", C.c_int), ("host_threads", C.c_int),
         ("verbose", C.c_int), ("gs_omega", C.c_double), ("restrict_sigma", C.c_int), ("block_ep", C.c_int), ("dist_shard_levels", C.c_int), ("block_fine", C.c_int), ("fine_col16", C.c_int), ("stream_gate", C.c_int), ("dist_exchange", C.c_int), ("prepare_structure", C.c_int), ("fuse_restrict_sweep", C.c_int), ("speculate_head", C.c_int), ("uniform_slices", C.c_int), ("color_ahead", C.c_int),
-        ("accelerate", C.c_int),
+        ("spatial_order", C.c_int), ("accelerate", C.c_int),
     ]
 
 
@@ -146,6 +146,7 @@
     "gmg_debug_device_galerkin": (C.c_int, [_vp, C.c_int, _ip, _ip, _dp, _dp, C.c_int, _ip, _ip, _dp, C.c_int64, _ip, _ip, _dp, _dp, _ip]),
     "gmg_host_plan_level": (C.c_int, [C.c_int, _ip, _ip, _dp, C.c_int, C.c_int, C.c_int, C.POINTER(C.c_int64), _ip, _ip, _ip,
                                       C.POINTER(C.c_ubyte)]),
+    "gmg_host_spatial_order": (C.c_int, [_ip, C.c_int, C.c_int, C.c_int, _ip]),
     "gmg_host_fine_block_rule": (C.c_int, [C.c_int, _ip, _ip, _dp, _ip, _ip]),
     "gmg_debug_set": (C.c_int, [_vp, C.c_char_p, C.c_double]),
     "gmg_bench_kernel": (C.c_int, [_vp, C.c_int, C.c_int, C.c_int, C.c_int, _dp, _ip]),
@@ -319,7 +320,7 @@
 
     def __init__(self, smoother=SMOOTHER_MULTICOLOR_GS, pre_iters=2, post_iters=2, jacobi_omega=0.67,
                  coarse_mode=COARSE_AUTO, use_graph=False, sigma=0, row_align=64, block_rows=64, block_from_level=1, block_lanes=0,
-                 device_setup=True, device_rap=True, reorder_fine=2, inner_precision=0, block_csr=True, device=0, verbose=False, gs_omega=None, block_ep=None, restrict_sigma=None, dist_shard_levels=None, block_fine=None, fine_col16=None, stream_gate=None, prepare_structure=None, dist_exchange=None, fuse_restrict_sweep=None, speculate_head=None, uniform_slices=None, color_ahead=None, accelerate=0):
+                 device_setup=True, device_rap=True, reorder_fine=2, inner_precision=0, block_csr=True, device=0, verbose=False, gs_omega=None, block_ep=None, restrict_sigma=None, dist_shard_levels=None, block_fine=None, fine_col16=None, stream_gate=None, prepare_structure=None, dist_exchange=None, fuse_restrict_sweep=None, speculate_head=None, uniform_slices=None, color_ahead=None, accelerate=0, spatial_order=None):
         l = lib()
         cfg = GmgConfig()
         l.gmg_config_default(C.byref(cfg))
@@ -356,6 +357,8 @@
         if dist_exchange is not None:
             cfg.dist_exchange = int(dist_exchange)
         cfg.accelerate = int(accelerate)
+        if spatial_order is not None:
+            cfg.spatial_order = int(bool(spatial_order))
         self._h = _vp()
         rc = l.gmg_create(C.byref(cfg), C.byref(self._h))
         if rc:
@@ -839,6 +842,15 @@
     return {"n_pad": int(info[0]), "n_colors": int(info[1]), "colored_ahead": bool(info[5]), "new2old": new2old, "color_begin": color_begin}
 
 
+def host_spatial_order(color_begin, n_slices: int, slices_per_wg: int) -> np.ndarray:
+    cb = np.ascontiguousarray(color_begin, np.int32)
+    order = np.empty((int(n_slices) + int(slices_per_wg) - 1) // int(slices_per_wg), np.int32)
+    rc = lib().gmg_host_spatial_order(_pi(cb), len(cb) - 1, int(n_slices), int(slices_per_wg), _pi(order))
+    if rc:
+        raise GmgError(rc, "gmg_host_spatial_order")
+    return order
+
+
 def host_fine_block_rule(A):
     a = _csc(A)
     blocked, reason = C.c_int(0), C.c_int(0)
diff --git a/gravo_mg_amd/csrc/bindings.cpp b/gravo_mg_amd/csrc/bindings.cpp
--- a/gravo_mg_amd/csrc/bindings.cpp
+++ b/gravo_mg_amd/csrc/bindings.cpp
@@ -308,6 +308,7 @@
         else if (key == "dist_exchange") c.dist_exchange = (int)value;
         else if (key == "inner_precision") c.inner_precision = (int)value;
         else if (key == "accelerate") c.accelerate = (int)value;
+        else if (key == "spatial_order") c.spatial_order = (int)value;
         else throw std::invalid_argument("unknown engine option: " + key);
     }
 
diff --git a/gravo_mg_amd/csrc/engine.hip b/gravo_mg_amd/csrc/engine.hip
--- a/gravo_mg_amd/csrc/engine.hip
+++ b/gravo_mg_amd/csrc/engine.hip
@@ -121,6 +121,7 @@
     cfg->restrict_sigma = 64;
     cfg->gs_omega = 1.35;
     cfg->accelerate = 0;
+    cfg->spatial_order = 1;
     return GMG_OK;
 } GMG_CATCH_0
 
@@ -1435,6 +1436,14 @@
     return GMG_OK;
 } GMG_CATCH_0
 
+int gmg_host_spatial_order(const int* color_begin, int n_colors, int n_slices, int slices_per_wg, int* order) try {
+    if (!color_begin || !order || n_colors < 1 || n_slices < 1 || slices_per_wg < 1) return GMG_ERR_INVALID;
+    for (int c = 0; c < n_colors; ++c) if (color_begin[c] < 0 || color_begin[c + 1] < color_begin[c]) return GMG_ERR_INVALID;
+    const std::vector<int> o = spatial_block_order(color_begin, n_colors, n_slices, slices_per_wg);
+    std::memcpy(order, o.data(), sizeof(int) * o.size());
+    return GMG_OK;
+} GMG_CATCH_0
+
 int gmg_debug_set(gmg_handle h, const char* key, double value) try {
     if (!h || !key) return GMG_ERR_INVALID;
     if (std::string(key) == "col16_uncovered") { h->dbg_col16_uncovered = (int)value; return GMG_OK; }
@@ -1443,6 +1452,11 @@
         h->dbg_cheby_ratio = value;
         if (h->has_device) drop_graphs(h);
         if (h->timing.count("cheby_ratio")) h->timing["cheby_ratio"] = cheby_ratio(h);
+        return GMG_OK;
+    }
+    if (std::string(key) == "spatial_mask") {
+        h->dbg_spatial_mask = value < 0 ? -1 : ((int)value & 7);
+        if (h->has_device) drop_graphs(h);
         return GMG_OK;
     }
     return fail(h, GMG_ERR_INVALID, std::string("unknown debug key: ") + key);
diff --git a/gravo_mg_amd/csrc/engine_cycle.hip.hpp b/gravo_mg_amd/csrc/engine_cycle.hip.hpp
--- a/gravo_mg_amd/csrc/engine_cycle.hip.hpp
+++ b/gravo_mg_amd/csrc/engine_cycle.hip.hpp
@@ -101,6 +101,20 @@
 
 inline bool polled(gmg_handle h);
 
+constexpr int kSpatialOrderMask = 3;
+inline int spatial_mask(gmg_handle h) {
+    if (h->dbg_spatial_mask >= 0) return h->dbg_spatial_mask;
+    const int env = EnvSwitches::get().spatial_mask;
+    return env >= 0 ? env : kSpatialOrderMask;
+}
+inline const int* order_table(gmg_handle h, const Level& l, int sb, int se, int spw, int bit) {
+    if (&l != &h->lv[0] || sb != 0 || se <= 0 || !l.wg_all4 || !(spatial_mask(h) & bit)) return nullptr;
+    const bool norm = spw == gmgk::kNormWaves;
+    if (se == l.Aoff.n_slices) return norm ? l.wg_all16.get() : l.wg_all4.get();
+    if (se == l.wg_head_slices) return norm ? l.wg_head16.get() : l.wg_head4.get();
+    return nullptr;
+}
+
 template <class T>
 T level_omega(gmg_handle h, const Level& l) { return &l == &h->lv[0] ? (T)h->cfg.gs_omega : (T)1.0; }
 
@@ -295,12 +309,13 @@
 void launch_spmv_lpr(gmg_handle h, Level& l, int d, int mode, const T* b, const T* x, T* y, int sb, int se, bool y_il = false) {
     const int ld = l.n_pad;
     const bool il = y_il && mode == 1 && LPR == 1 && d > 1 && d <= 4;
+    const int* wg_order = LPR == 1 ? order_table(h, l, sb, se, gmgk::kWavesPerBlock, 1) : nullptr;
     for_col_chunks(d, [&](int c0, int dc) {
         DISPATCH_D(dc, DISPATCH_C16(l.Aoff.c16_sel(), DISPATCH_FLAG(RES, mode == 1, DISPATCH_FLAG(YI, il,
                        hipLaunchKernelGGL((gmgk::spmv_full<T, D, (RES ? 1 : 0), LPR, (LPR == 1 ? C16 : 0), (YI && RES && LPR == 1 && D > 1)>), dim3(grid_for(se - sb)),
                                           dim3(gmgk::kBlock), 0, h->stream, l.Aoff.slice_ptr, l.Aoff.col, Prec<T>::val(l.Aoff), Prec<T>::diag(l),
                                           (RES ? b + (size_t)c0 * ld : nullptr), x + (size_t)c0 * ld, y + (size_t)c0 * ld, ld, sb, se, 1, l.Aoff.col16,
-                                          l.Aoff.win_base, l.Aoff.c16_arg())))));
+                                          l.Aoff.win_base, l.Aoff.c16_arg(), wg_order)))));
     });
 }
 template <class T>
@@ -375,10 +390,11 @@
     const bool il = src_il && d > 1 && d <= 4;
     if (se < 0) se = fine.P.n_slices;
     if (c16 < 0) c16 = fine.P.c16_sel();
+    const int* wg_order = (se == fine.P.n_slices && fine.P.n_slices == fine.Aoff.n_slices) ? order_table(h, fine, sb, se, gmgk::kWavesPerBlock, 4) : nullptr;
     for_col_chunks(d, [&](int c0, int dc) {
         DISPATCH_D(dc, DISPATCH_C16(c16, DISPATCH_FLAG(XI, il, hipLaunchKernelGGL((gmgk::transfer<T, D, 1, 1, C16, (XI && D > 1)>), dim3(grid_for(se - sb)), dim3(gmgk::kBlock), 0,
                                           h->stream, fine.P.slice_ptr, fine.P.col, Prec<T>::val(fine.P), (const int*)nullptr, src + (size_t)c0 * coarse.n_pad, coarse.n_pad,
-                                          dst + (size_t)c0 * fine.n_pad, fine.n_pad, sb, se, 1, fine.P.col16, fine.P.win_base, fine.P.c16_arg()))));
+                                          dst + (size_t)c0 * fine.n_pad, fine.n_pad, sb, se, 1, fine.P.col16, fine.P.win_base, fine.P.c16_arg(), wg_order))));
     });
 }
 template <class T>
@@ -440,10 +456,11 @@
     const int n_slices = folded ? l.ord.color_begin[l.ord.n_colors - 1] / 64 : l.Aoff.n_slices;
     const int nblk = norm_grid(n_slices);
     const bool poll = polled(h);
+    const int* wg_order = order_table(h, l, 0, n_slices, gmgk::kNormWaves, 2);
     for_col_chunks(d, [&](int c0, int dc) {
         DISPATCH_D(dc, DISPATCH_C16(l.Aoff.c16_sel(), hipLaunchKernelGGL((gmgk::residual_norm_slices<D, 0, C16>), dim3(nblk), dim3(gmgk::kNormWaves * 64), 0, h->stream,
                                           l.Aoff.slice_ptr, l.Aoff.col, l.Aoff.val, l.diag, l.b + (size_t)c0 * l.n_pad, l.x + (size_t)c0 * l.n_pad, w,
-                                          l.n_pad, n_slices, (float*)nullptr, h->d_partials, l.Aoff.col16, l.Aoff.win_base, l.Aoff.c16_arg())));
+                                          l.n_pad, n_slices, (float*)nullptr, h->d_partials, l.Aoff.col16, l.Aoff.win_base, l.Aoff.c16_arg(), wg_order)));
         launch_reduce(h, nblk + folded, dc, c0, c0 + 4 >= d, nullptr, decide);
     });
     if (!poll) HIPCHK(hipMemcpyAsync(h->h_norm, h->d_norm, sizeof(double) * 2 * d, hipMemcpyDeviceToHost, h->stream));
@@ -857,10 +874,11 @@
     Level& l = h->lv[0];
     const double* w = type == 1 ? h->d_minv : (type == 2 ? h->d_mass : nullptr);
     const int nblk = norm_grid(l.Aoff.n_slices);
+    const int* wg_order = order_table(h, l, 0, l.Aoff.n_slices, gmgk::kNormWaves, 2);
     for_col_chunks(d, [&](int c0, int dc) {
         DISPATCH_D(dc, DISPATCH_C16(l.Aoff.c16_sel(), hipLaunchKernelGGL((gmgk::residual_norm_slices<D, 1, C16>), dim3(nblk), dim3(gmgk::kNormWaves * 64), 0, h->stream,
                                           l.Aoff.slice_ptr, l.Aoff.col, l.Aoff.val, l.diag, l.b + (size_t)c0 * l.n_pad, l.x + (size_t)c0 * l.n_pad, w, l.n_pad,
-                                          l.Aoff.n_slices, l.b32 + (size_t)c0 * l.n_pad, h->d_partials, l.Aoff.col16, l.Aoff.win_base, l.Aoff.c16_arg())));
+                                          l.Aoff.n_slices, l.b32 + (size_t)c0 * l.n_pad, h->d_partials, l.Aoff.col16, l.Aoff.win_base, l.Aoff.c16_arg(), wg_order)));
         launch_reduce(h, nblk, dc, c0, c0 + 4 >= d);
     });
     if (!polled(h)) HIPCHK(hipMemcpyAsync(h->h_norm, h->d_norm, sizeof(double) * 2 * d, hipMemcpyDeviceToHost, h->stream));
diff --git a/gravo_mg_amd/csrc/engine_state.hip.hpp b/gravo_mg_amd/csrc/engine_state.hip.hpp
--- a/gravo_mg_amd/csrc/engine_state.hip.hpp
+++ b/gravo_mg_amd/csrc/engine_state.hip.hpp
@@ -126,6 +126,8 @@
     DevBuf<int> d_new2old;
     DevBuf<int> d_old2new;
     DevBuf<int> d_blk_of_row;
+    DevBuf<int> wg_all4, wg_head4, wg_all16, wg_head16;
+    int wg_head_slices = 0;
     DevBuf<double> x, b, r, tmp;
     DevBuf<float> diag32, x32, b32, r32, tmp32;
 };
@@ -161,6 +163,7 @@
     DevPool pool;
     DistP2P* p2p = nullptr;
     double dbg_cheby_ratio = 0.0;
+    int dbg_spatial_mask = -1;
     int dbg_col16_uncovered = 0;
     gmg_config cfg;
     std::string err;
diff --git a/gravo_mg_amd/csrc/engine_system.hip.hpp b/gravo_mg_amd/csrc/engine_system.hip.hpp
--- a/gravo_mg_amd/csrc/engine_system.hip.hpp
+++ b/gravo_mg_amd/csrc/engine_system.hip.hpp
@@ -427,6 +427,29 @@
     return rc;
 }
 
+int build_order_tables(gmg_handle h, bool part) {
+    Level& l = h->lv[0];
+    l.wg_all4 = {}; l.wg_head4 = {}; l.wg_all16 = {}; l.wg_head16 = {};
+    l.wg_head_slices = 0;
+    const LevelOrdering& o = l.ord;
+    const bool wanted = h->cfg.spatial_order && !part && !o.blocked && o.n_colors >= 2 && l.Aoff.lpr == 1 && l.Aoff.n_slices > 0 &&
+                        (int)o.color_begin.size() == o.n_colors + 1;
+    h->timing["spatial_order"] = wanted ? 1.0 : 0.0;
+    if (!wanted) return GMG_OK;
+    const int n_all = l.Aoff.n_slices, n_head = std::min(n_all, o.color_begin[o.n_colors - 1] / 64);
+    auto table = [&](int n_slices, int spw) { return n_slices > 0 ? spatial_block_order(o.color_begin.data(), o.n_colors, n_slices, spw) : std::vector<int>(); };
+    const std::vector<int> all4 = table(n_all, gmgk::kWavesPerBlock), all16 = table(n_all, gmgk::kNormWaves),
+                           head4 = table(n_head, gmgk::kWavesPerBlock), head16 = table(n_head, gmgk::kNormWaves);
+    int rc;
+    if ((rc = upload(h, l.wg_all4, all4)) || (rc = upload(h, l.wg_all16, all16))) return rc;
+    if (n_head > 0) {
+        if ((rc = upload(h, l.wg_head4, head4)) || (rc = upload(h, l.wg_head16, head16))) return rc;
+        l.wg_head_slices = n_head;
+    }
+    HIPCHK(hipStreamSynchronize(h->stream));
+    return GMG_OK;
+}
+
 void stash_orderings(gmg_handle h) {
     h->ord_cache.resize(h->L + 1);
     for (int k = 0; k <= h->L; ++k) h->ord_cache[k] = std::move(h->lv[k].ord);
@@ -485,6 +508,7 @@
         (void)hipStreamSynchronize(h->stream);
         if (rc_all != GMG_OK) return err_all.empty() ? rc_all : fail(h, rc_all, err_all);
         if (!factor_ok) return fail(h, GMG_ERR_NUMERIC, "coarsest operator is singular (LDL^T hit a zero pivot)");
+        if ((rc = build_order_tables(h, part))) return rc;
         h->coarse_work.assign((size_t)h->lv[L].A.n_outer * 4, 0.0);
         h->timing["setup_ordering"] = 0.0; h->timing["setup_sell"] = 0.0;
         for (int k = 0; k <= L; ++k) h->timing["setup_ordering_l" + std::to_string(k)] = stage[k].ms_order;
diff --git a/gravo_mg_amd/csrc/host_plan.hpp b/gravo_mg_amd/csrc/host_plan.hpp
--- a/gravo_mg_amd/csrc/host_plan.hpp
+++ b/gravo_mg_amd/csrc/host_plan.hpp
@@ -705,6 +705,35 @@
     for (int i = 0; i < n; ++i) { o.new2old[i] = i; o.old2new[i] = i; }
     return o;
 }
+
+inline std::vector<int> spatial_block_order(const int* color_begin, int n_colors, int n_slices, int S) {
+    const int nwg = (n_slices + S - 1) / S;
+    struct Key { int64_t num, den; int c, g; };
+    std::vector<Key> key((size_t)std::max(nwg, 0));
+    int c = 0, cb = 0, ce = 0, next = 0;
+    for (int g = 0; g < nwg; ++g) {
+        const int s = g * S;
+        for (; s >= ce && next < n_colors; ++next)
+            if (color_begin[next + 1] / kSlice > color_begin[next] / kSlice) { c = next; cb = color_begin[next] / kSlice; ce = color_begin[next + 1] / kSlice; }
+        key[g] = Key{2 * (int64_t)(s - cb) + S, 2 * (int64_t)std::max(ce - cb, 1), c, g};
+    }
+    std::vector<int> seq((size_t)std::max(nwg, 0));
+    std::iota(seq.begin(), seq.end(), 0);
+    std::sort(seq.begin(), seq.end(), [&](int a, int b) {
+        const Key &ka = key[a], &kb = key[b];
+        const int64_t l = ka.num * kb.den, r = kb.num * ka.den;
+        if (l != r) return l < r;
+        if (ka.c != kb.c) return ka.c < kb.c;
+        return ka.g < kb.g;
+    });
+    std::vector<int> order(seq.size());
+    for (int e = 0, start = 0; e < 8 && e < nwg; ++e) {
+        const int run = (nwg - e + 7) / 8;
+        for (int t = 0; t < run; ++t) order[e + 8 * t] = seq[start + t];
+        start += run;
+    }
+    return order;
+}
 struct RowStage {
     std::vector<int64_t> ptr;
     RawVec<int> idx;
diff --git a/gravo_mg_amd/csrc/host_sparse.hpp b/gravo_mg_amd/csrc/host_sparse.hpp
--- a/gravo_mg_amd/csrc/host_sparse.hpp
+++ b/gravo_mg_amd/csrc/host_sparse.hpp
@@ -75,6 +75,7 @@
     bool symv_v2 = true;
     bool tri_nt = false;
     double cheby_ratio = 0.0;
+    int spatial_mask = -1;
     static const EnvSwitches& get() {
         static const EnvSwitches v = [] {
             EnvSwitches e;
@@ -94,6 +95,7 @@
             e.symv_strides = std::max(0, (int)num("GMG_SYMV_STRIDES"));
             e.symv_v2 = (int)num("GMG_SYMV_V2") != 0;
             e.tri_nt = (int)num("GMG_TRI_NT") > 0;
+            if (std::getenv("GMG_SPATIAL_ORDER")) e.spatial_mask = std::max(0, (int)num("GMG_SPATIAL_ORDER")) & 7;
             if (const char* t = std::getenv("GMG_CHEBY_RATIO")) {
                 const double r = std::atof(t);
                 if (r > 1.0 && r <= 1e6) e.cheby_ratio = r;
diff --git a/gravo_mg_amd/csrc/kernels.hip.hpp b/gravo_mg_amd/csrc/kernels.hip.hpp
--- a/gravo_mg_amd/csrc/kernels.hip.hpp
+++ b/gravo_mg_amd/csrc/kernels.hip.hpp
@@ -16,6 +16,16 @@
     int w = b * kWavesPerBlock + (threadIdx.x >> 6);
     (void)n_slices_total;
     return __builtin_amdgcn_readfirstlane(w);
+}
+
+__device__ __forceinline__ int ordered_block(int n_slices_total, int spw, const int* __restrict__ wg_order) {
+    int b = blockIdx.x;
+    if (b < (n_slices_total + spw - 1) / spw) b = wg_order[b];
+    return __builtin_amdgcn_readfirstlane(b);
+}
+__device__ __forceinline__ int wave_slice(int n_slices_total, int xcd_swizzle, const int* __restrict__ wg_order) {
+    if (wg_order == nullptr) return wave_slice(n_slices_total, xcd_swizzle);
+    return __builtin_amdgcn_readfirstlane(ordered_block(n_slices_total, kWavesPerBlock, wg_order) * kWavesPerBlock + (int)(threadIdx.x >> 6));
 }
 
 template <int D, int XI> __device__ __forceinline__ int64_t x_at(int c, int d, int ld) { return XI ? (int64_t)c * D + d : c + (int64_t)d * ld; }
@@ -974,8 +984,9 @@
                                                     const T* __restrict__ val, const T* __restrict__ diag,
                                                     const T* __restrict__ b, const T* __restrict__ x,
                                                     T* __restrict__ y, int ld, int slice_begin, int slice_end,
-                                                    int xcd_swizzle, const unsigned* __restrict__ col16 = nullptr, const int* __restrict__ win_base = nullptr, int c16_arg = 0) {
-    const int s = slice_begin + wave_slice(slice_end - slice_begin, xcd_swizzle);
+                                                    int xcd_swizzle, const unsigned* __restrict__ col16 = nullptr, const int* __restrict__ win_base = nullptr, int c16_arg = 0,
+                                                    const int* __restrict__ wg_order = nullptr) {
+    const int s = slice_begin + wave_slice(slice_end - slice_begin, xcd_swizzle, wg_order);
     if (s >= slice_end) return;
     spmv_full_slice<T, D, MODE, LPR, C16, YI>(slice_ptr, col, val, diag, b, x, y, ld, s, col16, win_base, c16_arg);
 }
@@ -1011,8 +1022,8 @@
                                                    const T* __restrict__ val, const int* __restrict__ row_of,
                                                    const T* __restrict__ x, int ldx, T* __restrict__ y, int ldy,
                                                    int slice_begin, int slice_end, int xcd_swizzle, const unsigned* __restrict__ col16 = nullptr,
-                                                   const int* __restrict__ win_base = nullptr, int c16_arg = 0) {
-    const int s = slice_begin + wave_slice(slice_end - slice_begin, xcd_swizzle);
+                                                   const int* __restrict__ win_base = nullptr, int c16_arg = 0, const int* __restrict__ wg_order = nullptr) {
+    const int s = slice_begin + wave_slice(slice_end - slice_begin, xcd_swizzle, wg_order);
     if (s >= slice_end) return;
     transfer_slice<T, D, ADD, LPR, C16, XI>(slice_ptr, col, val, row_of, x, ldx, y, ldy, s, col16, win_base, c16_arg);
 }
@@ -1426,11 +1437,13 @@
                                                                const double* __restrict__ b, const double* __restrict__ x,
                                                                const double* __restrict__ weight, int ld, int n_slices,
                                                                float* __restrict__ r32, double* __restrict__ partials,
-                                                               const unsigned* __restrict__ col16 = nullptr, const int* __restrict__ win_base = nullptr, int c16_arg = 0) {
+                                                               const unsigned* __restrict__ col16 = nullptr, const int* __restrict__ win_base = nullptr, int c16_arg = 0,
+                                                               const int* __restrict__ wg_order = nullptr) {
     __shared__ double red[kNormWaves][2 * D];
     const int wave = threadIdx.x >> 6, lane = threadIdx.x & 63;
     int nblk = gridDim.x, bb = blockIdx.x;
-    if ((nblk & 7) == 0) bb = (bb & 7) * (nblk >> 3) + (bb >> 3);
+    if (wg_order != nullptr) bb = ordered_block(n_slices, kNormWaves, wg_order);
+    else if ((nblk & 7) == 0) bb = (bb & 7) * (nblk >> 3) + (bb >> 3);
     const int s = __builtin_amdgcn_readfirstlane(bb * kNormWaves + wave);
     double sums[2 * D];
 #pragma unroll
diff --git a/include/gravomg_hip.h b/include/gravomg_hip.h
--- a/include/gravomg_hip.h
+++ b/include/gravomg_hip.h
@@ -57,6 +57,7 @@
     int speculate_head;
     int uniform_slices;
     int color_ahead;
+    int spatial_order;
     int accelerate;
 } gmg_config;
 
diff --git a/include/gravomg_hip_internal.h b/include/gravomg_hip_internal.h
--- a/include/gravomg_hip_internal.h
+++ b/include/gravomg_hip_internal.h
@@ -29,6 +29,8 @@
 int gmg_host_plan_level(int n, const int* colptr, const int* rowidx, const double* val, int mode, int block_rows, int sigma,
                         int64_t* info, int* new2old, int* color_begin, int* blk_begin, unsigned char* row_color);
 
+int gmg_host_spatial_order(const int* color_begin, int n_colors, int n_slices, int slices_per_wg, int* order);
+
 int gmg_host_fine_block_rule(int n, const int* colptr, const int* rowidx, const double* val, int* blocked, int* reason);
 
 int gmg_bench_kernel(gmg_handle h, int kind, int k, int d, int reps, double* ms_avg, int* launches_out);
```
